# Jisu-Linnea-Han/ClimateMachine.jl

Hardware: AMD Instinct MI355X
Metric: DG RHS DOF-updates/sec (higher is better)
Workload: dtype f64; 1 GPU; Held-Suarez dry GCM (BASELINE configs[2]), stacked cubed sphere 6x30x30x8 elements, N=4, LSRK54 explicit, hyperdiffusion (DryBiharmonic, horizontal), Rusanov, fp64; elements=43200, nodes_per_element=125, states=5, parallelism=element partition (Hilbert, whole columns), 1 rank(s), RCCL p2p halo

## Files before the change

### climatemachine.jl_amd/_lib.py

```python
import ctypes as C
import os

_HERE = os.path.dirname(os.path.abspath(__file__))
LIB_PATH = os.environ.get("CMDG_LIB", os.path.join(_HERE, "libcmdg.so"))

CMDG_K = dict(GRADIENTS=0, DIVGRAD=1, GRADLAP=2, TENDENCY=3, PACK=4, UNPACK=5, UPDATE_AUX=6,
              FILTER=7, STACK_INTEGRAL=8, TRANSPORT=9, HALO_EXPOSED=10, GRADIENTS_EXT=11,
              DIVGRAD_EXT=12, GRADLAP_EXT=13, TENDENCY_EXT=14, FV_GRADIENTS=15, FV_TENDENCY=16,
              ESDG_TENDENCY=17)
STACK_MAXOUT = 8
OPT_KEEP_GRADFLUX = 1
OPT_STACK_HEIGHT = 2
OPT_REFERENCE_HALO = 3
OPT_HALO_PIPELINE = 4
OPT_STEP_GRAPH = 5
OPT_STREAM_PRIORITY = 6
OPT_TENDENCY_PAIRS = 7
OPT_ASYNC_RUN = 8
OPT_TENDENCY_FOUR_WAVES = 9
OPT_GRADARG_HANDOFF = 10
CMDG_Q = dict(GRADFLUX_LIVE=1, LAW_NEEDS_GRADFLUX=2, NDERIVED=3, NUPDATED_AUX=4, FUSED_UPDATE_AUX=5,
              DIRECT_SEND=6, DIRECT_RECV=7, TENDENCY_ELEMS_PER_GROUP=8, HALO_PIPELINE=9, HOST_POST_NS=10, HOST_POST_COUNT=11, GRAPH_STEPS=12, TENDENCY_PAIRS=13,
              GRADARG_HANDOFF=14, GRADARG_REFRESHES=15,
              STATE_READ=16, AUX_READ=20)


class CmdgStackIntegralDesc(C.Structure):
    _fields_ = [
        ("nout", C.c_int32),
        ("src_is_state", C.c_int32 * STACK_MAXOUT), ("src_col", C.c_int32 * STACK_MAXOUT),
        ("scale", C.c_double * STACK_MAXOUT), ("dst_col", C.c_int32 * STACK_MAXOUT),
        ("rsrc_col", C.c_int32 * STACK_MAXOUT), ("rdst_col", C.c_int32 * STACK_MAXOUT),
    ]


class CmdgDesc(C.Structure):
    _fields_ = [
        ("dim", C.c_int32), ("N", C.c_int32 * 3),
        ("nreal", C.c_int64), ("nghost", C.c_int64),
        ("nvgeo", C.c_int32), ("physics_id", C.c_int32),
        ("iparam", C.c_int32 * 16), ("dparam", C.c_double * 64),
        ("nf_first", C.c_int32), ("direction", C.c_int32),
        ("diffusion_direction", C.c_int32), ("stacked", C.c_int32),
        ("vgeo", C.c_void_p), ("sgeo", C.c_void_p),
        ("vmapM", C.c_void_p), ("vmapP", C.c_void_p), ("elemtobndy", C.c_void_p),
        ("interiorelems", C.c_void_p), ("ninterior", C.c_int64),
        ("exteriorelems", C.c_void_p), ("nexterior", C.c_int64),
        ("activedofs", C.c_void_p), ("D", C.c_void_p),
        ("vmapsend", C.c_void_p), ("nvmapsend", C.c_int64),
        ("vmaprecv", C.c_void_p), ("nvmaprecv", C.c_int64),
        ("nnabr", C.c_int32), ("nabrtorank", C.c_void_p),
        ("nabrtovmapsend", C.c_void_p), ("nabrtovmaprecv", C.c_void_p),
        ("state_auxiliary", C.c_void_p), ("state_gradient_flux", C.c_void_p),
        ("Qhypervisc_grad", C.c_void_p), ("Qhypervisc_div", C.c_void_p),
        ("Dv", C.c_void_p),
    ]


MAX_HOOK_OPS = 4


class CmdgRhsHooks(C.Structure):
    _fields_ = [
        ("npre", C.c_int32), ("pre_filter", C.c_void_p * MAX_HOOK_OPS),
        ("ncopy", C.c_int32),
        ("copy_gf_col", C.c_int32 * MAX_HOOK_OPS), ("copy_aux_col", C.c_int32 * MAX_HOOK_OPS),
        ("copy_scale", C.c_double * MAX_HOOK_OPS),
        ("has_integral", C.c_int32), ("has_reverse_integral", C.c_int32),
        ("integral", CmdgStackIntegralDesc), ("reverse_integral", CmdgStackIntegralDesc),
        ("nsurf", C.c_int32),
        ("surf_src_col", C.c_int32 * MAX_HOOK_OPS), ("surf_dst_col", C.c_int32 * MAX_HOOK_OPS),
        ("nvertelem", C.c_int32), ("Imat", C.c_void_p),
        ("has_flow_deviation", C.c_int32), ("flow_u_col", C.c_int32), ("flow_ud_col", C.c_int32),
        ("flow_H", C.c_double),
        ("ops_before_gradients", C.c_int32), ("pre_rhs_handle", C.c_void_p),
        ("pre_rhs_src_col", C.c_int32), ("pre_rhs_dst_aux_col", C.c_int32),
    ]


class CmdgOcean01Desc(C.Structure):
    _fields_ = [("nvertelem", C.c_int32), ("H", C.c_double), ("Imat", C.c_void_p),
                ("add_fast_substeps", C.c_int32), ("nstages_fast", C.c_int32),
                ("rka_fast", C.c_void_p), ("rkb_fast", C.c_void_p), ("rkc_fast", C.c_void_p)]


class CmdgOceanCouplingDesc(C.Structure):
    _fields_ = [
        ("nvertelem", C.c_int32), ("H", C.c_double), ("Imat", C.c_void_p),
        ("slow_u_col", C.c_int32), ("slow_eta_col", C.c_int32), ("slow_dGu_col", C.c_int32),
        ("fast_eta_col", C.c_int32), ("fast_U_col", C.c_int32),
        ("fast_GU_col", C.c_int32), ("fast_du_col", C.c_int32),
    ]


MRI_MAXR, MRI_MAXGAMMA = 6, 4
MRIGARK_EXPLICIT, MRIGARK_DECOUPLED_IMPLICIT = 0, 1


class CmdgMrigarkDesc(C.Structure):
    _fields_ = [("kind", C.c_int32), ("nstages", C.c_int32), ("ngamma", C.c_int32),
                ("gamma", C.c_void_p), ("dc", C.c_void_p), ("fast_nstages", C.c_int32),
                ("fast_rka", C.c_void_p), ("fast_rkb", C.c_void_p), ("fast_rkc", C.c_void_p),
                ("fast_dt", C.c_double), ("lu_adjustable", C.c_int32)]


GMRES_MAX_M = 64


class CmdgGmresInfo(C.Structure):
    _fields_ = [("iterations", C.c_int64), ("converged", C.c_int32), ("residual_norm", C.c_double),
                ("threshold", C.c_double)]


RED_WEIGHTEDSUM, RED_SUM, RED_DOT, RED_DISTANCE, RED_NORM, RED_MAX, RED_MIN = range(7)


class CmdgReduceDesc(C.Structure):
    _fields_ = [("op", C.c_int32), ("p", C.c_double), ("weighted", C.c_int32),
                ("per_state", C.c_int32), ("nstate", C.c_int32), ("states", C.c_void_p),
                ("nstates", C.c_int32)]


class CmdgFvDesc(C.Structure):
    _fields_ = [("reconstruction", C.c_int32), ("width", C.c_int32), ("limiter", C.c_int32),
                ("nvertelem", C.c_int32), ("periodicstack", C.c_int32)]


FV_CONSTANT, FV_LINEAR = 0, 1


class CmdgEsdgDesc(C.Structure):
    _fields_ = [("volume_flux", C.c_int32), ("surface_flux", C.c_int32), ("Mcut", C.c_double),
                ("low_mach", C.c_int32), ("kinetic_energy_preserving", C.c_int32)]


(ESDG_FLUX_NONE, ESDG_FLUX_ENTROPY_CONSERVATIVE, ESDG_FLUX_CENTRAL, ESDG_FLUX_KG, ESDG_FLUX_RUSANOV,
 ESDG_FLUX_ENTROPY_CONSERVATIVE_PENALTY, ESDG_FLUX_MATRIX) = range(7)
FV_VANLEER, FV_NOLIMITER = 0, 1


_vp, _i32, _i64, _d = C.c_void_p, C.c_int32, C.c_int64, C.c_double
SYMBOLS = [
    ("cmdg_version", C.c_char_p, []),
    ("cmdg_status_string", C.c_char_p, [C.c_int]),
    ("cmdg_physics_counts", C.c_int, [_i32, _vp, _vp]),
    ("cmdg_atmos_host_constants", C.c_int, [_vp, _vp, _vp]),
    ("cmdg_create", C.c_int, [C.POINTER(CmdgDesc), C.POINTER(_vp)]),
    ("cmdg_create_dgfv", C.c_int, [C.POINTER(CmdgDesc), C.POINTER(CmdgFvDesc), C.POINTER(_vp)]),
    ("cmdg_create_esdg", C.c_int, [C.POINTER(CmdgDesc), C.POINTER(CmdgEsdgDesc), C.POINTER(_vp)]),
    ("cmdg_esdg_entropy", C.c_int, [_vp, _vp, _vp, _vp]),
    ("cmdg_destroy", C.c_int, [_vp]),
    ("cmdg_last_error", C.c_char_p, [_vp]),
    ("cmdg_rhs", C.c_int, [_vp, _vp, _vp, _d, _d, _d]),
    ("cmdg_rhs_async", C.c_int, [_vp, _vp, _vp, _d, _d, _d]),
    ("cmdg_lsrk_step", C.c_int, [_vp, _vp, _vp, _d, _d, _i32, _vp, _vp, _vp]),
    ("cmdg_lsrk_run", C.c_int, [_vp, _vp, _vp, _d, _d, _i64, _i32, _vp, _vp, _vp]),
    ("cmdg_synchronize", C.c_int, [_vp]),
    ("cmdg_set_option", C.c_int, [_vp, _i32, _i32]),
    ("cmdg_query", C.c_int, [_vp, _i32, _vp]),
    ("cmdg_export_hypervisc_grad", C.c_int, [_vp, _vp]),
    ("cmdg_export_gradient_flux", C.c_int, [_vp, _vp]),
    ("cmdg_halo_begin", C.c_int, [_vp, _vp, _i32]),
    ("cmdg_halo_end", C.c_int, [_vp, _vp, _i32]),
    ("cmdg_fillsendbuf", C.c_int, [_vp, _vp, _vp, _i64, _i32, _i32]),
    ("cmdg_transferrecvbuf", C.c_int, [_vp, _vp, _vp, _i64, _i32, _i32]),
    ("cmdg_comm_unique_id", C.c_int, [_vp]),
    ("cmdg_comm_init_rccl", C.c_int, [_vp, _vp, _i32, _i32]),
    ("cmdg_comm_selftest", C.c_int, [_vp, _i64]),
    ("cmdg_comm_connect_local", C.c_int, [_vp, _i32]),
    ("cmdg_group_rhs", C.c_int, [_vp, _i32, _vp, _vp, _d, _d, _d]),
    ("cmdg_group_halo", C.c_int, [_vp, _i32, _vp, _i32]),
    ("cmdg_group_lsrk_run", C.c_int, [_vp, _i32, _vp, _vp, _d, _d, _i64, _i32, _vp, _vp, _vp]),
    ("cmdg_norm2_local", C.c_int, [_vp, _vp, _i32, _i32, _vp]),
    ("cmdg_distance2_local", C.c_int, [_vp, _vp, _vp, _i32, _vp]),
    ("cmdg_reduce_local", C.c_int, [_vp, _vp, _vp, _vp, _vp]),
    ("cmdg_reduce_combine", C.c_int, [_vp, _vp, _i32, _vp]),
    ("cmdg_reduce", C.c_int, [_vp, _vp, _vp, _vp, _vp]),
    ("cmdg_group_reduce", C.c_int, [_vp, _i32, _vp, _vp, _vp, _vp]),
    ("cmdg_courant", C.c_int, [_vp, _i32, _vp, _d, _d, _i32, _vp]),
    ("cmdg_min_node_distance", C.c_int, [_vp, _i32, _vp]),
    ("cmdg_indefinite_stack_integral", C.c_int, [_vp, _vp, _i32, _vp, _i32, _i32, _vp, _vp]),
    ("cmdg_reverse_indefinite_stack_integral", C.c_int, [_vp, _vp, _i32, _i32, _vp]),
    ("cmdg_filter_create", C.c_int, [_vp, _vp, C.POINTER(_vp)]),
    ("cmdg_filter_destroy", C.c_int, [_vp, _vp]),
    ("cmdg_filter_apply", C.c_int, [_vp, _vp, _vp, _i32]),
    ("cmdg_set_filters", C.c_int, [_vp, _vp, _vp, _vp]),
    ("cmdg_set_rhs_hooks", C.c_int, [_vp, _vp]),
    ("cmdg_ocean_initialize_states", C.c_int, [_vp, _vp, _vp]),
    ("cmdg_ocean_tendency_from_slow_to_fast", C.c_int, [_vp, _vp, _vp, _vp]),
    ("cmdg_ocean_reconcile_from_fast_to_slow", C.c_int, [_vp, _vp, _vp, _vp, _vp]),
    ("cmdg_split_explicit01_step", C.c_int,
     [_vp, _vp, _vp, _vp, _vp, _vp, _vp, _vp, _d, _d, _d, _i32, _vp, _vp, _vp]),
    ("cmdg_group_split_explicit01_step", C.c_int,
     [_vp, _vp, _i32, _vp, _vp, _vp, _vp, _vp, _vp, _d, _d, _d, _i32, _vp, _vp, _vp]),
    ("cmdg_load_plugin", C.c_int, [C.c_char_p]),
    ("cmdg_lsrk_update", C.c_int, [_vp, _vp, _vp, _d, _d]),
    ("cmdg_ls3n_step", C.c_int, [_vp, _vp, _vp, _vp, _d, _d, _i32, _vp, _vp, _vp]),
    ("cmdg_ssprk_step", C.c_int, [_vp, _vp, _vp, _vp, _d, _d, _i32, _vp, _vp, _vp]),
    ("cmdg_group_split_explicit_step", C.c_int,
     [_vp, _vp, _i32, _vp, _i32, _vp, _vp, _vp, _vp, _vp, _d, _d, _d, _i32, _vp, _vp, _vp]),
    ("cmdg_split_explicit_step", C.c_int,
     [_vp, _vp, _vp, _i32, _vp, _vp, _vp, _vp, _vp, _d, _d, _d, _i32, _vp, _vp, _vp]),
    ("cmdg_profile_enable", C.c_int, [_vp, _i32]),
    ("cmdg_profile_get", C.c_int, [_vp, _i32, _vp, _vp]),
    ("cmdg_profile_reset", C.c_int, [_vp]),
    ("cmdg_columnlu_create", C.c_int, [_vp, _i32, _d, C.POINTER(_vp)]),
    ("cmdg_columnlu_update", C.c_int, [_vp, _d]),
    ("cmdg_columnlu_assemble", C.c_int, [_vp, _d]),
    ("cmdg_columnlu_solve", C.c_int, [_vp, _vp, _vp]),
    ("cmdg_columnlu_info", C.c_int, [_vp, _vp]),
    ("cmdg_columnlu_alpha", C.c_int, [_vp, _vp]),
    ("cmdg_columnlu_export_band", C.c_int, [_vp, _i64, _vp]),
    ("cmdg_columnlu_destroy", C.c_int, [_vp]),
    ("cmdg_ark_step", C.c_int, [_vp, _vp, _vp, _vp, _d, _d, _i32, _vp, _vp, _vp, _vp, _i32]),
    ("cmdg_mri_lsrk_update", C.c_int, [_vp, _vp, _vp, _d, _d, _i32, _vp, _vp]),
    ("cmdg_mri_qhat", C.c_int, [_vp, _vp, _vp, _i32, _vp, _vp]),
    ("cmdg_mrigark_step", C.c_int, [_vp, _vp, _vp, _vp, _vp, _vp, _vp, _vp, _d, _d]),
    ("cmdg_gmres_create", C.c_int, [_vp, _i32, _d, _d, C.POINTER(_vp)]),
    ("cmdg_gmres_fits", C.c_int, [_vp, _i32, _i64, _vp]),
    ("cmdg_gmres_prepare", C.c_int, [_vp, _d]),
    ("cmdg_gmres_solve", C.c_int, [_vp, _d, _vp, _vp, _d, _i64, C.POINTER(CmdgGmresInfo)]),
    ("cmdg_gmres_step_info", C.c_int, [_vp, _i32, _vp, _vp]),
    ("cmdg_gmres_destroy", C.c_int, [_vp]),
    ("cmdg_ark_step_gmres", C.c_int, [_vp, _vp, _vp, _vp, _d, _d, _i32, _vp, _vp, _vp, _vp, _i32]),
    ("cmdg_mrigark_step_gmres", C.c_int, [_vp, _vp, _vp, _vp, _vp, _vp, _vp, _vp, _d, _d]),
    ("cmdg_interp_create", C.c_int, [_vp, _vp, C.POINTER(_vp)]),
    ("cmdg_interp_destroy", C.c_int, [_vp, _vp]),
    ("cmdg_interp_apply", C.c_int, [_vp, _vp, _vp, _i32, _i64, _vp]),
    ("cmdg_interp_project", C.c_int, [_vp, _vp, _vp, _i32, _vp]),
    ("cmdg_interp_scatter", C.c_int, [_vp, _vp, _i32, _vp, _i32, _vp]),
    ("cmdg_dss_create", C.c_int, [_vp, _vp, C.POINTER(_vp)]),
    ("cmdg_dss_destroy", C.c_int, [_vp, _vp]),
    ("cmdg_dss_info", C.c_int, [_vp, _vp]),
    ("cmdg_dss_apply", C.c_int, [_vp, _vp, _vp, _i32]),
    ("cmdg_dss", C.c_int, [_vp, _vp, _vp, _i32]),
    ("cmdg_group_dss", C.c_int, [_vp, _i32, _vp, _vp, _i32]),
]

_LIB = None


class CmdgError(RuntimeError):
    pass


def lib():
    global _LIB
    if _LIB is None:
        if not os.path.exists(LIB_PATH):
            raise CmdgError(
                "libcmdg.so is not built (%s); run `python -c 'import __graft_entry__ as g; "
                "g.build()'` -- there is no CPU fallback" % LIB_PATH)
        try:
            import torch
            rccl = os.path.join(os.path.dirname(torch.__file__), "lib", "librccl.so")
            if os.path.exists(rccl):
                os.environ.setdefault("CMDG_RCCL_LIB", rccl)
        except Exception:
            pass
        L = C.CDLL(LIB_PATH)
        for name, res, args in SYMBOLS:
            f = getattr(L, name)
            f.restype = res
            f.argtypes = args
        _LIB = L
    return _LIB


def check(status, handle=None):
    if status != 0:
        L = lib()
        msg = L.cmdg_last_error(handle).decode()
        raise CmdgError("libcmdg: %s (%d): %s" % (
            L.cmdg_status_string(status).decode(), status, msg))
```

### climatemachine.jl_amd/csrc/cmdg.hip

```cpp
#include <dlfcn.h>

#include <algorithm>
#include <new>
#include <tuple>

#include "rccl.h"
#include "stepping.h"

namespace cmdg {

namespace {
typedef int (*roctx_push_t)(const char *);
typedef int (*roctx_pop_t)();
roctx_push_t g_roctx_push = nullptr;
roctx_pop_t g_roctx_pop = nullptr;
int g_roctx_state = 0;
void roctx_resolve()
{
    g_roctx_state = -1;
    const char *names[] = {"librocprofiler-sdk-roctx.so.1", "librocprofiler-sdk-roctx.so", "libroctx64.so.4",
                           "libroctx64.so", nullptr};
    const char *want = getenv("CMDG_ROCTX");
    void *lib = nullptr;
    for (int i = 0; names[i] && !lib; ++i) lib = dlopen(names[i], RTLD_NOW | RTLD_NOLOAD);
    if (!lib && want && *want && *want != '0')
        for (int i = 0; names[i] && !lib; ++i) lib = dlopen(names[i], RTLD_NOW | RTLD_GLOBAL);
    if (!lib) return;
    g_roctx_push = (roctx_push_t)dlsym(lib, "roctxRangePushA");
    g_roctx_pop = (roctx_pop_t)dlsym(lib, "roctxRangePop");
    if (g_roctx_push && g_roctx_pop) g_roctx_state = 1;
}
}
void roctx_push(const char *name)
{
    if (g_roctx_state == 0) roctx_resolve();
    if (g_roctx_state == 1) g_roctx_push(name);
}
void roctx_pop()
{
    if (g_roctx_state == 1) g_roctx_pop();
}

int dbg_sync()
{
    static const int v = [] {
        const char *p = getenv("CMDG_DBG_SYNC");
        return p ? atoi(p) : 0;
    }();
    return v;
}

hipError_t ev_record(hipEvent_t e, hipStream_t s) { return hipEventRecord(e, s); }

int EngineBase::launch_status(const char *what)
{
    hipError_t e = hipGetLastError();
    if (e != hipSuccess) return fail(CMDG_ERR_HIP, std::string(what) + ": " + hipGetErrorString(e));
    return CMDG_OK;
}

int EngineBase::order(hipStream_t earlier, hipStream_t later)
{
    if (earlier == later) return CMDG_OK;
    if (dbg_sync() & 1) (void)hipStreamSynchronize(earlier);
    if (ev_record(ev_comp, earlier) != hipSuccess || hipStreamWaitEvent(later, ev_comp, 0) != hipSuccess)
        return fail(CMDG_ERR_HIP, "stream ordering failed");
    return CMDG_OK;
}

int EngineBase::ensure_Imat(const double *host)
{
    if (d_Imat) return CMDG_OK;
    if (!host) return fail(CMDG_ERR_INVALID, "Imat is NULL");
    if (d_Imat.alloc(NQ * NQ) != hipSuccess ||
        hipMemcpy(d_Imat, host, sizeof(double) * NQ * NQ, hipMemcpyHostToDevice) != hipSuccess)
        return fail(CMDG_ERR_HIP, "Imat upload failed");
    return CMDG_OK;
}

int set_err(cmdg_handle h, int code)
{
    if (h && h->eng && code != CMDG_OK) h->err = h->eng->err;
    return code;
}

GroupCall::GroupCall(cmdg_handle *h, cmdg_handle *h2, int n, bool pairs)
{
    if (!h || (pairs && !h2) || n < 1) return;
    for (int i = 0; i < n; ++i)
        if (!h[i] || (pairs && !h2[i])) return;
    for (int i = 0; i < n; ++i) {
        const std::string r = std::to_string(i);
        members.push_back({h[i], pairs ? "pair " + r + " (slow): " : "rank " + r + ": "});
        if (pairs) members.push_back({h2[i], "pair " + r + " (fast): "});
    }
    for (auto &m : members) {
        if (m.first->eng->worker) m.first->eng->worker->wait_idle();
        m.first->eng->err.clear();
    }
    dev.emplace(h[0]->eng);
}

GroupCall::GroupCall(const std::vector<std::pair<cmdg_handle, std::string>> &named)
{
    if (named.empty()) return;
    for (auto &m : named)
        if (!m.first) return;
    for (auto &m : named) {
        bool merged = false;
        for (auto &have : members)
            if (have.first == m.first) {
                have.second = have.second.substr(0, have.second.size() - 2) + " / " + m.second + ": ";
                merged = true;
            }
        if (!merged) members.push_back({m.first, m.second + ": "});
    }
    for (auto &m : members) {
        if (m.first->eng->worker) m.first->eng->worker->wait_idle();
        m.first->eng->err.clear();
    }
    dev.emplace(named[0].first->eng);
}

int GroupCall::finish(int rc)
{
    if (rc == CMDG_OK) return rc;
    std::string msg = cmdg_status_string(rc);
    for (auto &m : members)
        if (!m.first->eng->err.empty()) {
            msg = m.second + m.first->eng->err;
            break;
        }
    for (auto &m : members) m.first->err = msg;
    return rc;
}

EngineBase::~EngineBase()
{
    delete worker;
    worker = nullptr;
    if (s_comp) hipStreamSynchronize(s_comp);
    if (s_comm) hipStreamSynchronize(s_comm);
    prof_collect();
    if (graph_exec) hipGraphExecDestroy(graph_exec);
    if (nccl_comm && rccl::CommDestroy) rccl::CommDestroy(nccl_comm);
}

static __global__ void k_face_digest(const double *__restrict__ vgeo, int nvgeo,
                                     const double *__restrict__ sgeo,
                                     const int64_t *__restrict__ vmapM,
                                     const int64_t *__restrict__ vmapP,
                                     const int64_t *__restrict__ elemtobndy, int NQ, int NQV,
                                     int64_t nreal, int32_t *__restrict__ faceP,
                                     double *__restrict__ faceG, double *__restrict__ faceW,
                                     int32_t *__restrict__ facePr, int *__restrict__ bad)
{
    const int Np = NQ * NQ * NQV, Nfph = NQ * NQV, Nfpv = NQ * NQ;
    const int Nfp = Nfph > Nfpv ? Nfph : Nfpv, NFT = 4 * Nfph + 2 * Nfpv;
    const int64_t I = (int64_t)blockIdx.x * blockDim.x + threadIdx.x;
    if (I >= nreal * NFT) return;
    const int64_t e = I / NFT;
    const int t = (int)(I % NFT);
    int f, n;
    if (t < 4 * Nfph) {
        f = t / Nfph;
        n = t % Nfph;
    } else {
        f = 4 + (t - 4 * Nfph) / Nfpv;
        n = (t - 4 * Nfph) % Nfpv;
    }
    const int64_t o = n + (int64_t)Nfp * (f + 6 * e);
    const int a = n % NQ, b = n / NQ;
    int vid;
    switch (f) {
    case 0: vid = NQ * (a + NQ * b); break;
    case 1: vid = (NQ - 1) + NQ * (a + NQ * b); break;
    case 2: vid = a + NQ * NQ * b; break;
    case 3: vid = a + NQ * ((NQ - 1) + NQ * b); break;
    case 4: vid = n; break;
    default: vid = n + NQ * NQ * (NQV - 1); break;
    }
    int flags = 0;
    const int64_t idM = vmapM[o] - 1;
    if (idM != e * Np + vid) flags |= 1;
    int64_t idP = vmapP[o] - 1;
    if (elemtobndy[f + 6 * e] != 0) idP = e * Np + vid;
    if (idP < 0 || idP > 2147483647LL) flags |= 4;
    faceP[I] = (int32_t)idP;
    const int64_t eP = idP >= 0 ? idP / Np : 0;
    facePr[I] = (int32_t)(eP * Np + ring_slot_of(NQ, NQV, (int)(idP - eP * Np)));
    const double *sg = sgeo + 5 * o;
#pragma unroll
    for (int c = 0; c < 4; ++c) faceG[((int64_t)4 * e + c) * NFT + t] = sg[c];
    const double mi = vgeo[vid + (int64_t)Np * (VMI + (int64_t)nvgeo * e)];
    if (!(sg[SVMI] == mi)) flags |= 2;
    faceW[I] = mi * sg[SSM];
    if (flags) atomicOr(bad, flags);
}

int EngineBase::init(const cmdg_desc *d)
{
    Np = NQ * NQ * NQV;
    Nfp = NQ * (NQ > NQV ? NQ : NQV);
    if (d->N[0] != d->N[1] || d->N[0] != NQ - 1 || d->N[2] != NQV - 1)
        return fail(CMDG_ERR_INVALID, "cmdg_create: polynomial orders do not match the engine");
    if (NQV != NQ && !d->Dv)
        return fail(CMDG_ERR_INVALID, "cmdg_create: Dv is required when the vertical order differs");
    nreal = d->nreal;
    nghost = d->nghost;
    nelem = nreal + nghost;
    nf_first = d->nf_first;
    direction = d->direction;
    diffusion_direction = d->diffusion_direction;
    stacked = d->stacked;
    if (!d->vgeo || !d->sgeo || !d->vmapM || !d->vmapP || !d->elemtobndy || !d->D ||
        !d->state_auxiliary)
        return fail(CMDG_ERR_INVALID, "cmdg_create: a required grid/state pointer is NULL");
    if (d->nvgeo < 11) return fail(CMDG_ERR_INVALID, "cmdg_create: vgeo needs >= 11 columns");
    if (d->ninterior + d->nexterior != nreal)
        return fail(CMDG_ERR_INVALID, "cmdg_create: interior + exterior != nreal");
    if ((d->ninterior > 0 && !d->interiorelems) || (d->nexterior > 0 && !d->exteriorelems))
        return fail(CMDG_ERR_INVALID, "cmdg_create: element list pointer is NULL");
    if (direction < 0 || direction > 2 || diffusion_direction < 0 || diffusion_direction > 2)
        return fail(CMDG_ERR_INVALID, "cmdg_create: bad direction");
    g.vgeo = d->vgeo;
    g.sgeo = d->sgeo;
    g.vmapM = d->vmapM;
    g.vmapP = d->vmapP;
    g.elemtobndy = d->elemtobndy;
    g.nvgeo = d->nvgeo;
    d_interior = d_interior_user = d->interiorelems;
    ninterior = d->ninterior;
    d_exterior = d_exterior_user = d->exteriorelems;
    nexterior = d->nexterior;
    d_activedofs = d->activedofs;
    d_vmapsend = d->vmapsend;
    nvmapsend = d->nvmapsend;
    d_vmaprecv = d->vmaprecv;
    nvmaprecv = d->nvmaprecv;
    if (d->nnabr > 0) {
        if (!d->nabrtorank || !d->nabrtovmapsend || !d->nabrtovmaprecv || !d->vmapsend ||
            !d->vmaprecv)
            return fail(CMDG_ERR_INVALID, "cmdg_create: halo tables missing");
        nabrtorank.assign(d->nabrtorank, d->nabrtorank + d->nnabr);
        nabrsend.assign(d->nabrtovmapsend, d->nabrtovmapsend + 2 * d->nnabr);
        nabrrecv.assign(d->nabrtovmaprecv, d->nabrtovmaprecv + 2 * d->nnabr);
    }
    HIPCHK(hipGetDevice(&dev));
    HIPCHK(s_comp.create(hipStreamNonBlocking));
    {
        int lo = 0, hi = 0;
        const char *pv = getenv("CMDG_HALO_PRIORITY");
        if (communicate() && pv && *pv == '1' && hipDeviceGetStreamPriorityRange(&lo, &hi) == hipSuccess && hi < lo)
            HIPCHK(s_comm.create(hipStreamNonBlocking, hi));
        else
            HIPCHK(s_comm.create(hipStreamNonBlocking));
    }
    for (int i = 0; i < 2; ++i) {
        HIPCHK(ev_int[i].create(hipEventDisableTiming));
        HIPCHK(ev_ext[i].create(hipEventDisableTiming));
    }
    HIPCHK(gev_fork.create(hipEventDisableTiming));
    if (const char *v = getenv("CMDG_STEP_GRAPH")) step_graph = *v && *v != '0';
    HIPCHK(ev_comp.create(hipEventDisableTiming));
    HIPCHK(d_D.alloc(NQ * NQ));
    HIPCHK(hipMemcpy(d_D, d->D, sizeof(double) * NQ * NQ, hipMemcpyHostToDevice));
    g.D = d_D;
    g.Dv = d_D;
    if (NQV != NQ) {
        HIPCHK(d_Dv.alloc(NQV * NQV));
        HIPCHK(hipMemcpy(d_Dv, d->Dv, sizeof(double) * NQV * NQV, hipMemcpyHostToDevice));
        g.Dv = d_Dv;
    }
    {
        const int NFT = 4 * NQ * NQV + 2 * NQ * NQ;
        const int64_t nt = std::max<int64_t>(nreal, 1) * NFT;
        DevBuf<int> d_bad;
        int bad = 0;
        HIPCHK(d_faceP.alloc(nt));
        HIPCHK(d_faceG.alloc(4 * nt));
        HIPCHK(d_faceW.alloc(nt));
        HIPCHK(d_facePr.alloc(nt));
        HIPCHK(d_bad.alloc_zeroed(1, s_comp));
        if (nreal > 0)
            hipLaunchKernelGGL(k_face_digest, dim3((unsigned)((nreal * NFT + 255) / 256)), dim3(256), 0,
                               s_comp, g.vgeo, g.nvgeo, g.sgeo, g.vmapM, g.vmapP, g.elemtobndy, NQ,
                               NQV, nreal, d_faceP.get(), d_faceG.get(), d_faceW.get(), d_facePr.get(),
                               d_bad.get());
        hipError_t le = hipGetLastError();
        hipError_t ce = hipMemcpyAsync(&bad, d_bad, sizeof(int), hipMemcpyDeviceToHost, s_comp);
        hipError_t se = hipStreamSynchronize(s_comp);
        d_bad.reset();
        if (le != hipSuccess || ce != hipSuccess || se != hipSuccess)
            return fail(CMDG_ERR_HIP, "cmdg_create: digest of the face tables failed");
        if (bad & 1)
            return fail(CMDG_ERR_INVALID, "cmdg_create: vmapM is not the face numbering of Grids.jl:586-594");
        if (bad & 2)
            return fail(CMDG_ERR_INVALID, "cmdg_create: sgeo's vMI differs from vgeo's MI at the face nodes (Grids.jl:1097-1101)");
        if (bad & 4)
            return fail(CMDG_ERR_INVALID, "cmdg_create: too many elements for 32-bit face indices");
        g.faceP = d_faceP;
        g.faceG = d_faceG;
        g.faceW = d_faceW;
        g.facePr = d_facePr;
    }
    aux = d->state_auxiliary;
    const size_t nd = (size_t)Np * nelem;
    gf = gf_node_major() ? nullptr : d->state_gradient_flux;
    gf_user = gf_node_major() ? d->state_gradient_flux : nullptr;
    if (!gf) {
        HIPCHK(gf_own.alloc_zeroed(std::max<size_t>(nd * ngf, 1), s_comp));
        gf = gf_own;
    }
    hypgrad_user = ngl > 0 ? d->Qhypervisc_grad : nullptr;
    HIPCHK(hypgrad.alloc_zeroed(std::max<size_t>(nd * 3 * ngl, 1), s_comp));
    hypdiv = d->Qhypervisc_div;
    if (!hypdiv) {
        HIPCHK(hd_own.alloc_zeroed(std::max<size_t>(nd * nhyp, 1), s_comp));
        hypdiv = hd_own;
    }
    slot_nvar_max = std::max(std::max(ns, ngf), std::max(3 * ngl, nhyp));
    if (communicate()) {
        for (auto &s : slot) {
            HIPCHK(s.sendbuf.alloc(slot_nvar_max * std::max<int64_t>(nvmapsend, 1)));
            HIPCHK(s.recvbuf.alloc(slot_nvar_max * std::max<int64_t>(nvmaprecv, 1)));
            HIPCHK(s.ev_packed.create(hipEventDisableTiming));
            HIPCHK(s.ev_done.create(hipEventDisableTiming));
            HIPCHK(s.ev_pulled.create(hipEventDisableTiming));
        }
    }
    HIPCHK(d_partial.alloc(1024));
    if (communicate())
        if (int r = init_halo_tables()) return r;
    if (const char *v = getenv("CMDG_REFERENCE_HALO")) reference_halo = *v && *v != '0';
    if (const char *v = getenv("CMDG_HALO_PIPELINE")) no_pipeline = *v == '0';
    if (const char *v = getenv("CMDG_FUSED_COLUMNS")) fused_columns = atoi(v);
    if (int r = init_derived()) return r;
    HIPCHK(hipStreamSynchronize(s_comp));
    return CMDG_OK;
}

int EngineBase::ensure_work()
{
    for (int i = 0; i < 2; ++i)
        if (!W[i]) {
            const size_t n = (size_t)Np * ns * nelem;
            HIPCHK(W[i].alloc_zeroed(n, s_comp));
            HIPCHK(hipStreamSynchronize(s_comp));
        }
    return CMDG_OK;
}

int EngineBase::ensure_garg()
{
    if (!garg) {
        const size_t n = std::max<size_t>((size_t)Np * ngl * nelem, 1);
        HIPCHK(garg.alloc_zeroed(n, s_comp));
        HIPCHK(lapr.alloc_zeroed(n, s_comp));
        HIPCHK(hipStreamSynchronize(s_comp));
    }
    return CMDG_OK;
}

int EngineBase::synchronize()
{
    HIPCHK(hipStreamSynchronize(s_comp));
    HIPCHK(hipStreamSynchronize(s_comm));
    return CMDG_OK;
}

ProfRec &EngineBase::prof_pair(int kernel, bool clamp, Event e1)
{
    ProfRec r{kernel, Event(), std::move(e1), clamp};
    r.e0.create();
    if (!r.e1) r.e1.create();
    prof.push_back(std::move(r));
    return prof.back();
}
void EngineBase::prof_begin(int kernel, hipStream_t st)
{
    if (!profiling) return;
    hipEventRecord(prof_pair(kernel, false).e0, st);
}
void EngineBase::prof_end(hipStream_t st)
{
    if (!profiling) return;
    hipEventRecord(prof.back().e1, st);
}
static __global__ void k_export_node_major(double *__restrict__ dst, const double *__restrict__ src, int Np,
                                           int ncol, int64_t nelem)
{
    const int64_t I = (int64_t)blockIdx.x * blockDim.x + threadIdx.x;
    if (I >= (int64_t)Np * ncol * nelem) return;
    const int64_t e = I / ((int64_t)Np * ncol);
    const int r = (int)(I - e * Np * ncol), s = r / Np, n = r - s * Np;
    dst[I] = src[s + (int64_t)ncol * (n + (int64_t)Np * e)];
}
static __global__ void k_import_node_major(double *__restrict__ dst, const double *__restrict__ src, int Np,
                                           int ncol, int64_t nelem)
{
    const int64_t I = (int64_t)blockIdx.x * blockDim.x + threadIdx.x;
    if (I >= (int64_t)Np * ncol * nelem) return;
    const int64_t e = I / ((int64_t)Np * ncol);
    const int r = (int)(I - e * Np * ncol), n = r / ncol, s = r - n * ncol;
    dst[I] = src[n + (int64_t)Np * (s + (int64_t)ncol * e)];
}

int EngineBase::export_hypgrad(double *dst)
{
    if (!dst) dst = hypgrad_user;
    if (ngl == 0) return CMDG_OK;
    if (!dst) return fail(CMDG_ERR_INVALID, "cmdg_export_hypervisc_grad: no destination (cmdg_desc.Qhypervisc_grad was NULL)");
    const int64_t n = (int64_t)Np * 3 * ngl * nelem;
    hipLaunchKernelGGL(k_export_node_major, dim3((unsigned)((n + 255) / 256)), dim3(256), 0, s_comp, dst, hypgrad, Np,
                       3 * ngl, nelem);
    HIPCHK(hipStreamSynchronize(s_comp));
    return CMDG_OK;
}
int EngineBase::export_gradflux(double *dst)
{
    if (!dst) dst = gf_node_major() ? gf_user : gf;
    if (ngf == 0) return CMDG_OK;
    if (!dst) return fail(CMDG_ERR_INVALID, "cmdg_export_gradient_flux: no destination (cmdg_desc.state_gradient_flux was NULL)");
    const int64_t n = (int64_t)Np * ngf * nelem;
    if (gf_node_major()) {
        hipLaunchKernelGGL(k_export_node_major, dim3((unsigned)((n + 255) / 256)), dim3(256), 0, s_comp, dst, gf, Np,
                           ngf, nelem);
    } else if (dst != gf) {
        HIPCHK(hipMemcpyAsync(dst, gf, sizeof(double) * n, hipMemcpyDeviceToDevice, s_comp));
    }
    HIPCHK(hipStreamSynchronize(s_comp));
    return CMDG_OK;
}
void EngineBase::prof_collect()
{
    for (auto &r : prof) {
        hipEventSynchronize(r.e1);
        float ms = 0;
        if (hipEventElapsedTime(&ms, r.e0, r.e1) == hipSuccess) {
            prof_ms[r.kernel] += r.clamp && ms < 0 ? 0.0f : ms;
            prof_n[r.kernel] += 1;
        }
    }
    prof.clear();
}

int EngineBase::set_stack_height(int nv)
{
    constexpr int TILE_C = 32, TILE_L = 4, MIN_HEIGHT = 17;
    if (nv < 0 || (nv > 0 && (!stacked || nreal % nv != 0)))
        return fail(CMDG_ERR_INVALID, "stack height: not a stacked topology or nreal is not a multiple of it");
    if (fv) return CMDG_OK;
    HIPCHK(hipStreamSynchronize(s_comp));
    d_interior = d_interior_user;
    d_exterior = d_exterior_user;
    if (nv < MIN_HEIGHT) return CMDG_OK;
    for (int which = 0; which < 2; ++which) {
        const int64_t n = which ? nexterior : ninterior;
        if (n == 0) continue;
        std::vector<int64_t> h((size_t)n);
        HIPCHK(hipMemcpy(h.data(), which ? d_exterior_user : d_interior_user, sizeof(int64_t) * n,
                         hipMemcpyDeviceToHost));
        auto key = [&](int64_t e1) {
            const int64_t e = e1 - 1, col = e / nv, lev = e % nv;
            return std::make_tuple(col / TILE_C, lev / TILE_L, col % TILE_C, lev % TILE_L);
        };
        std::stable_sort(h.begin(), h.end(), [&](int64_t x, int64_t y) { return key(x) < key(y); });
        DevBuf<int64_t> &own = which ? d_exterior_tiled : d_interior_tiled;
        if (!own) HIPCHK(own.alloc(n));
        HIPCHK(hipMemcpy(own, h.data(), sizeof(int64_t) * n, hipMemcpyHostToDevice));
        (which ? d_exterior : d_interior) = own;
    }
    return CMDG_OK;
}

int EngineBase::set_stream_priority(int level)
{
    int lo = 0, hi = 0;
    HIPCHK(hipDeviceGetStreamPriorityRange(&lo, &hi));
    if (level < -1 || level > 1) return fail(CMDG_ERR_INVALID, "stream priority: 0 (default), 1 (highest) or -1 (lowest)");
    if (int r = synchronize()) return r;
    drop_graph();
    Stream nc, nm;
    const int prio = level > 0 ? hi : (level < 0 ? lo : 0);
    HIPCHK(nc.create(hipStreamNonBlocking, prio));
    HIPCHK(nm.create(hipStreamNonBlocking, prio));
    s_comp = std::move(nc);
    s_comm = std::move(nm);
    stream_priority = level;
    return CMDG_OK;
}

int EngineBase::rhs_segment(int seg, const RhsCtx &c)
{
    const bool comm = exchanges();
    const bool gfl = gf_live();
    const bool grad = gfl || nhyp > 0;
    const bool hyper = nhyp > 0;
    const bool dsend = comm && direct_send(), unpack = !(comm && direct_recv());
    const bool pipe = pipelined() && !has_hooks;
    hipStream_t s_ext = pipe ? s_comm : s_comp;
    const int nhd = ngl;
    int r;
#define TRY(x) \
    if ((r = (x)) != CMDG_OK) return r
    const Event *const EI = capturing ? gev_int : ev_int, *const EE = capturing ? gev_ext : ev_ext;
    auto evi = [&](int64_t q) { return capturing ? (int)((cap_pass + (q - pass_seq)) % NGEV) : (int)(q & 1); };
    auto interior_begin = [&]() -> int {
        ++pass_seq;
        if (capturing) ++cap_pass;
        if (!pipe) return CMDG_OK;
        if (capturing && cap_interior++ == 0) return CMDG_OK;
        if (profiling && prof_ext_done) {
            hipEventRecord(prof_pair(CMDG_K_HALO_EXPOSED, true, std::move(prof_ext_done)).e0, s_comp);
        }
        if (dbg_sync() & 64) HIPCHK(hipStreamSynchronize(s_comm));
        HIPCHK(hipStreamWaitEvent(s_comp, EE[evi(pass_seq - 1)], 0));
        return CMDG_OK;
    };
    auto interior_end = [&]() -> int {
        if (pipe) HIPCHK(ev_record(EI[evi(pass_seq)], s_comp));
        return CMDG_OK;
    };
    auto exterior_begin = [&]() -> int {
        if (pipe && !(capturing && cap_exterior++ == 0)) {
            if (dbg_sync() & 64) HIPCHK(hipStreamSynchronize(s_comp));
            HIPCHK(hipStreamWaitEvent(s_comm, EI[evi(pass_seq - 1)], 0));
        }
        return CMDG_OK;
    };
    auto exterior_end = [&]() -> int {
        if (pipe) HIPCHK(ev_record(EE[evi(pass_seq)], s_comm));
        if (pipe && profiling) {
            prof_ext_done.create();
            hipEventRecord(prof_ext_done, s_comm);
        }
        return CMDG_OK;
    };
    switch (seg) {
    case 0:
        if (has_hooks) {
            if (!c.pre_done) TRY(run_pre_hooks(c));
            slot[SLOT_Q].fresh_for = nullptr;
        }
        if (!(grad && fused_update_aux())) launch_update_aux(c, 0, nreal);
        if (comm) TRY(halo_begin(SLOT_Q, c.Qin, ns, 0, pipe));
        if (grad) {
            TRY(interior_begin());
            launch_gradients(c, d_interior, ninterior, false, s_comp);
            TRY(interior_end());
        }
        break;
    case 1:
        if (!grad) break;
        if (comm) {
            TRY(halo_end(SLOT_Q, c.Qin, ns, unpack, pipe));
            if (unpack) launch_update_aux(c, nreal, nelem);
            if (has_hooks && hooks.has_flow_deviation)
                TRY(flow_deviation(c.Qin, nreal / hooks.nvertelem, nghost / hooks.nvertelem));
            if (has_hooks && hooks.ops_before_gradients) TRY(run_column_ops(c, nreal, nelem));
        }
        if (dsend && gfl) TRY(before_direct_send(SLOT_GF, s_ext));
        if (dsend && hyper) TRY(before_direct_send(SLOT_HG, s_ext));
        TRY(exterior_begin());
        launch_gradients(c, d_exterior, nexterior, comm, s_ext);
        TRY(exterior_end());
        if (dsend && gfl && !gradient_filter) mark_fresh(SLOT_GF, gf, ngf);
        if (dsend && hyper) mark_fresh(SLOT_HG, hypgrad, 3 * ngl);
        if (gradient_filter && gfl) {
            if (gf_node_major()) {
                const int64_t n = (int64_t)Np * ngf * nelem;
                const unsigned nb = (unsigned)((n + 255) / 256);
                if (!gf_scratch) HIPCHK(gf_scratch.alloc(n));
                hipLaunchKernelGGL(k_export_node_major, dim3(nb), dim3(256), 0, s_comp, gf_scratch, gf, Np, ngf, nelem);
                TRY(filter_apply(gradient_filter, gf_scratch, ngf));
                hipLaunchKernelGGL(k_import_node_major, dim3(nb), dim3(256), 0, s_comp, gf, gf_scratch, Np, ngf, nelem);
            } else {
                TRY(filter_apply(gradient_filter, gf, ngf));
            }
        }
        if (comm) {
            int slots[2], ns_ = 0;
            if (gfl) {
                TRY(halo_pack(SLOT_GF, gf, ngf, 0, pipe));
                slots[ns_++] = SLOT_GF;
            }
            if (hyper) {
                TRY(halo_pack(SLOT_HG, hypgrad, 3 * ngl, 0, pipe));
                slots[ns_++] = SLOT_HG;
            }
            if (ns_) TRY(halo_post(slots, ns_));
        }
        if (has_hooks && gfl) TRY(run_gradient_hooks(c, 0, nreal));
        if (hyper) {
            TRY(interior_begin());
            launch_divgrad(c, d_interior, ninterior, false, s_comp);
            TRY(interior_end());
        }
        break;
    case 2:
        if (!hyper) break;
        if (comm) TRY(halo_end(SLOT_HG, hypgrad, 3 * ngl, unpack, pipe));
        if (dsend) TRY(before_direct_send(SLOT_HD, s_ext));
        TRY(exterior_begin());
        launch_divgrad(c, d_exterior, nexterior, comm, s_ext);
        TRY(exterior_end());
        if (dsend) mark_fresh(SLOT_HD, hypdiv, nhd);
        if (comm) TRY(halo_begin(SLOT_HD, hypdiv, nhd, nhyp, pipe));
        TRY(interior_begin());
        launch_gradlap(c, d_interior, ninterior, false, s_comp);
        TRY(interior_end());
        break;
    case 3:
        if (hyper) {
            if (comm) TRY(halo_end(SLOT_HD, hypdiv, nhd, unpack, pipe));
            if (dsend) TRY(before_direct_send(SLOT_HG, s_ext));
            TRY(exterior_begin());
            launch_gradlap(c, d_exterior, nexterior, comm, s_ext);
            TRY(exterior_end());
            if (dsend) mark_fresh(SLOT_HG, hypgrad, 3 * ngl);
            if (comm) TRY(halo_begin(SLOT_HG, hypgrad, 3 * ngl, 0, pipe));
        }
        TRY(interior_begin());
        launch_tendency(c, d_interior, ninterior, false, s_comp);
        TRY(interior_end());
        break;
    case 4:
        if (comm) {
            if (grad) {
                if (gfl) {
                    TRY(halo_end(SLOT_GF, gf, ngf, unpack, pipe));
                    if (has_hooks) TRY(run_gradient_hooks(c, nreal, nelem));
                }
                if (hyper) TRY(halo_end(SLOT_HG, hypgrad, 3 * ngl, unpack, pipe));
            } else {
                TRY(halo_end(SLOT_Q, c.Qin, ns, unpack, pipe));
                if (unpack) launch_update_aux(c, nreal, nelem);
            }
        }
        break;
    case 5:
        if (dsend && c.lsrk) TRY(before_direct_send(SLOT_Q, s_ext));
        TRY(exterior_begin());
        launch_tendency(c, d_exterior, nexterior, comm, s_ext);
        TRY(exterior_end());
        if (dsend && c.lsrk) mark_fresh(SLOT_Q, c.Qout, ns);
        if (pipe && (dbg_sync() & 128)) HIPCHK(hipStreamSynchronize(s_comm));
        if (pipe) HIPCHK(hipStreamWaitEvent(s_comp, EE[evi(pass_seq)], 0));
        if (tendency_filter) TRY(filter_apply(tendency_filter, c.tendency, ns));
        if (c.update_after) {
            const int64_t n = (int64_t)Np * ns * nreal;
            lsrk_update(s_comp, c.tendency, c.Qin, c.rka_next, c.rkb_dt, n);
        }
        break;
    default: break;
    }
#undef TRY
    if (dbg_sync() & 512) HIPCHK(hipDeviceSynchronize());
    return launch_status("kernel launch");
}

int EngineBase::rhs_async(const RhsCtx &c)
{
    if (transport == TRANSPORT_LOCAL && communicate())
        return fail(CMDG_ERR_INVALID, "handles connected locally must be driven by the cmdg_group_* calls");
    invalidate_sends();
    for (int s = 0; s < NSEG; ++s)
        if (int r = rhs_segment(s, c)) {
            abort_exchanges();
            return r;
        }
    return CMDG_OK;
}

int group_rhs(std::vector<EngineBase *> &g, std::vector<RhsCtx> &c, bool keep_fresh)
{
    if (!keep_fresh)
        for (auto *e : g) e->invalidate_sends();
    for (auto &x : c) x.pre_done = false;
    if (dbg_sync() & 256) (void)hipDeviceSynchronize();
    bool nested = false;
    for (auto *e : g) nested = nested || (e->has_hooks && e->hooks.pre_rhs_handle);
    if (nested && g.size() > 1) {
        std::vector<EngineBase *> ch;
        std::vector<RhsCtx> cc(g.size());
        for (size_t i = 0; i < g.size(); ++i) {
            if (!(g[i]->has_hooks && g[i]->hooks.pre_rhs_handle))
                return g[i]->fail(CMDG_ERR_INVALID, "local group: every rank needs the nested operator");
            if (int r = g[i]->run_pre_hooks_a(c[i], cc[i])) return r;
            ch.push_back(g[i]->hooks.pre_rhs_handle->eng);
        }
        for (auto *e : ch) e->err.clear();
        if (int r = group_rhs(ch, cc)) {
            for (size_t i = 0; i < ch.size(); ++i)
                if (!ch[i]->err.empty()) return g[i]->fail(r, "nested operator: " + ch[i]->err);
            return r;
        }
        for (size_t i = 0; i < g.size(); ++i) {
            if (int r = g[i]->run_pre_hooks_b(c[i])) return r;
            c[i].pre_done = true;
        }
    }
    for (int s = 0; s < EngineBase::NSEG; ++s)
        for (size_t i = 0; i < g.size(); ++i)
            if (int r = g[i]->rhs_segment(s, c[i])) {
                for (auto *e : g) e->abort_exchanges();
                return r;
            }
    return CMDG_OK;
}

static __global__ void k_extremum(const double *__restrict__ v, int64_t n, int is_min,
                                  double *__restrict__ out)
{
    __shared__ double s[1024];
    double a = is_min ? INFINITY : -INFINITY;
    for (int64_t i = threadIdx.x; i < n; i += blockDim.x) a = is_min ? fmin(a, v[i]) : fmax(a, v[i]);
    s[threadIdx.x] = a;
    __syncthreads();
    for (int h = blockDim.x / 2; h > 0; h >>= 1) {
        if ((int)threadIdx.x < h)
            s[threadIdx.x] = is_min ? fmin(s[threadIdx.x], s[threadIdx.x + h])
                                    : fmax(s[threadIdx.x], s[threadIdx.x + h]);
        __syncthreads();
    }
    if (threadIdx.x == 0) out[0] = s[0];
}

int EngineBase::courant(int mode, int kind, const double *Q, double dt, double t, int dir,
                        double *out)
{
    if (dir < 0 || dir > 2 || kind < 0 || kind > 3) return fail(CMDG_ERR_INVALID, "courant: bad argument");
    if (g.nvgeo < 15) return fail(CMDG_ERR_INVALID, "courant: vgeo lacks the coordinate columns");
    if (nreal == 0) {
        *out = mode == 0 ? INFINITY : -INFINITY;
        return CMDG_OK;
    }
    if (!d_elemred) HIPCHK(d_elemred.alloc(nreal + 1));
    if (int r = launch_courant(mode, kind, Q, dt, t, dir, d_elemred)) return r;
    hipLaunchKernelGGL(k_extremum, dim3(1), dim3(1024), 0, s_comp, d_elemred, nreal, mode == 0,
                       d_elemred + nreal);
    HIPCHK(hipMemcpyAsync(out, d_elemred + nreal, sizeof(double), hipMemcpyDeviceToHost, s_comp));
    HIPCHK(hipStreamSynchronize(s_comp));
    return CMDG_OK;
}

static __global__ void k_wsum2(const double *__restrict__ A, const double *__restrict__ B,
                        const double *__restrict__ vgeo, int nvgeo, int Np, int nvar,
                        int64_t nreal, int weighted, double *__restrict__ partial)
{
    __shared__ double sh[256];
    const int64_t total = (int64_t)Np * nvar * nreal;
    double acc = 0.0;
    for (int64_t I = (int64_t)blockIdx.x * blockDim.x + threadIdx.x; I < total;
         I += (int64_t)gridDim.x * blockDim.x) {
        const int64_t e = I / ((int64_t)Np * nvar);
        const int n = (int)(I % Np);
        double d = A[I];
        if (B) d -= B[I];
        const double w = weighted ? vgeo[n + (int64_t)Np * (VM + (int64_t)nvgeo * e)] : 1.0;
        acc += w * d * d;
    }
    sh[threadIdx.x] = acc;
    __syncthreads();
    for (int s = 128; s > 0; s >>= 1) {
        if ((int)threadIdx.x < s) sh[threadIdx.x] += sh[threadIdx.x + s];
        __syncthreads();
    }
    if (threadIdx.x == 0) partial[blockIdx.x] = sh[0];
}

int EngineBase::wsum2(const double *A, const double *B, int nvar, int weighted, double *out)
{
    const int nb = 512;
    hipLaunchKernelGGL(k_wsum2, dim3(nb), dim3(256), 0, s_comp, A, B, g.vgeo, g.nvgeo, Np, nvar,
                       nreal, weighted, d_partial);
    double h[nb];
    HIPCHK(hipMemcpyAsync(h, d_partial, sizeof(double) * nb, hipMemcpyDeviceToHost, s_comp));
    HIPCHK(hipStreamSynchronize(s_comp));
    double acc = 0;
    for (int i = 0; i < nb; ++i) acc += h[i];
    *out = acc;
    return CMDG_OK;
}

}

using namespace cmdg;

extern "C" {

const char *cmdg_version(void) { return "cmdg 0.1 (gfx950)"; }

const char *cmdg_status_string(int status)
{
    switch (status) {
    case CMDG_OK: return "ok";
    case CMDG_ERR_INVALID: return "invalid argument";
    case CMDG_ERR_HIP: return "HIP runtime error";
    case CMDG_ERR_NO_DEVICE: return "no gfx950 device";
    case CMDG_ERR_COMM: return "communication error";
    case CMDG_ERR_UNSUPPORTED: return "unsupported physics / polynomial order";
    default: return "unknown status";
    }
}

int cmdg_esdg_entropy(cmdg_handle h, const double *Q, double *beta, double *eta)
{
    if (!h || !Q) return CMDG_ERR_INVALID;
    DevGuard guard_(h->eng);
    return set_err(h, h->eng->launch_entropy(Q, beta, eta));
}

int cmdg_rhs_async(cmdg_handle h, double *tendency, double *Q, double t, double alpha, double beta)
{
    if (!h || !tendency || !Q) return CMDG_ERR_INVALID;
    DevGuard guard_(h->eng);
    RhsCtx c;
    c.tendency = tendency;
    c.Qin = Q;
    c.t = t;
    c.alpha = alpha;
    c.beta = beta;
    return set_err(h, h->eng->rhs_async(c));
}

int cmdg_rhs(cmdg_handle h, double *tendency, double *Q, double t, double alpha, double beta)
{
    int r = cmdg_rhs_async(h, tendency, Q, t, alpha, beta);
    if (r) return r;
    DevGuard guard_(h->eng);
    return set_err(h, h->eng->synchronize());
}

int cmdg_synchronize(cmdg_handle h)
{
    if (!h) return CMDG_ERR_INVALID;
    DevGuard guard_(h->eng);
    if (h->eng->worker) {
        std::lock_guard<std::mutex> lk(h->eng->worker->m);
        if (const int r = h->eng->worker->deferred_rc) {
            h->eng->err = h->eng->worker->deferred_err;
            h->eng->worker->deferred_rc = 0;
            h->eng->worker->deferred_err.clear();
            return set_err(h, r);
        }
    }
    return set_err(h, h->eng->synchronize());
}

int cmdg_set_option(cmdg_handle h, int32_t option, int32_t value)
{
    if (!h) return CMDG_ERR_INVALID;
    DevGuard guard_(h->eng);
    EngineBase *e = h->eng;
    switch (option) {
    case CMDG_OPT_KEEP_GRADFLUX:
        e->drop_graph();
        e->keep_gradflux = value != 0;
        return CMDG_OK;
    case CMDG_OPT_STACK_HEIGHT:
        e->drop_graph();
        return set_err(h, e->set_stack_height(value));
    case CMDG_OPT_REFERENCE_HALO:
        if (int r = e->synchronize()) return set_err(h, r);
        e->drop_graph();
        e->reference_halo = value != 0 || e->fv || e->esdg;
        e->invalidate_sends();
        return CMDG_OK;
    case CMDG_OPT_STEP_GRAPH:
        if (int r = e->synchronize()) return set_err(h, r);
        e->drop_graph();
        e->step_graph = value != 0;
        e->graph_failed = false;
        return CMDG_OK;
    case CMDG_OPT_STREAM_PRIORITY: return set_err(h, e->set_stream_priority(value));
    case CMDG_OPT_ASYNC_RUN:
        if (value && !e->worker) {
            e->worker = new (std::nothrow) RunWorker();
            if (!e->worker) return set_err(h, e->fail(CMDG_ERR_INVALID, "async run: out of memory"));
            e->worker->start();
        } else if (!value && e->worker) {
            delete e->worker;
            e->worker = nullptr;
        }
        return CMDG_OK;
    case CMDG_OPT_TENDENCY_PAIRS:
    case CMDG_OPT_TENDENCY_FOUR_WAVES: return CMDG_OK;
    case CMDG_OPT_GRADARG_HANDOFF: e->gradarg_handoff = value != 0; return CMDG_OK;
    case CMDG_OPT_HALO_PIPELINE:
        if (int r = e->synchronize()) return set_err(h, r);
        e->drop_graph();
        e->no_pipeline = value == 0;
        e->invalidate_sends();
        return CMDG_OK;
    default: return set_err(h, e->fail(CMDG_ERR_INVALID, "cmdg_set_option: unknown option"));
    }
}

int cmdg_query(cmdg_handle h, int32_t what, int64_t *out)
{
    if (!h || !out) return CMDG_ERR_INVALID;
    const EngineBase *e = h->eng;
    switch (what) {
    case CMDG_Q_GRADFLUX_LIVE: *out = e->gf_live(); return CMDG_OK;
    case CMDG_Q_LAW_NEEDS_GRADFLUX: *out = e->law_needs_gradflux(); return CMDG_OK;
    case CMDG_Q_NDERIVED: *out = e->law_nder(); return CMDG_OK;
    case CMDG_Q_NUPDATED_AUX: *out = e->has_update_aux() ? e->law_nupd() : 0; return CMDG_OK;
    case CMDG_Q_FUSED_UPDATE_AUX: *out = e->has_update_aux() && e->fused_update_aux(); return CMDG_OK;
    case CMDG_Q_DIRECT_SEND: *out = e->communicate() && e->direct_send(); return CMDG_OK;
    case CMDG_Q_DIRECT_RECV: *out = e->communicate() && e->direct_recv(); return CMDG_OK;
    case CMDG_Q_TENDENCY_ELEMS_PER_GROUP: *out = e->tendency_epb(); return CMDG_OK;
    case CMDG_Q_GRAPH_STEPS: *out = e->graph_steps; return CMDG_OK;
    case CMDG_Q_TENDENCY_PAIRS: *out = -1; return CMDG_OK;
    case CMDG_Q_GRADARG_HANDOFF: *out = e->handoff_used; return CMDG_OK;
    case CMDG_Q_GRADARG_REFRESHES: *out = e->handoff_refreshes; return CMDG_OK;
    case CMDG_Q_HOST_POST_NS: *out = e->host_post_ns; return CMDG_OK;
    case CMDG_Q_HOST_POST_COUNT: *out = e->host_post_n; return CMDG_OK;
    case CMDG_Q_HALO_PIPELINE: *out = e->pipelined() && !e->has_hooks; return CMDG_OK;
    default:
        if (what >= CMDG_Q_STATE_READ && what < CMDG_Q_STATE_READ + 4) {
            *out = e->law_state_read(what - CMDG_Q_STATE_READ);
            return CMDG_OK;
        }
        if (what >= CMDG_Q_AUX_READ && what < CMDG_Q_AUX_READ + 4) {
            *out = e->law_aux_read(what - CMDG_Q_AUX_READ);
            return CMDG_OK;
        }
        return set_err(h, h->eng->fail(CMDG_ERR_INVALID, "cmdg_query: unknown item"));
    }
}

int cmdg_export_hypervisc_grad(cmdg_handle h, double *dst)
{
    if (!h) return CMDG_ERR_INVALID;
    DevGuard guard_(h->eng);
    return set_err(h, h->eng->export_hypgrad(dst));
}

int cmdg_export_gradient_flux(cmdg_handle h, double *dst)
{
    if (!h) return CMDG_ERR_INVALID;
    DevGuard guard_(h->eng);
    return set_err(h, h->eng->export_gradflux(dst));
}

int cmdg_group_rhs(cmdg_handle *handles, int32_t n, double **tendency, double **Q, double t,
                   double alpha, double beta)
{
    if (!tendency || !Q) return CMDG_ERR_INVALID;
    for (int i = 0; i < n; ++i)
        if (!tendency[i] || !Q[i]) return CMDG_ERR_INVALID;
    GroupCall gc(handles, n);
    if (!gc.ok()) return CMDG_ERR_INVALID;
    std::vector<EngineBase *> g;
    std::vector<RhsCtx> c(n);
    for (int i = 0; i < n; ++i) {
        g.push_back(handles[i]->eng);
        c[i].tendency = tendency[i];
        c[i].Qin = Q[i];
        c[i].t = t;
        c[i].alpha = alpha;
        c[i].beta = beta;
    }
    return gc.finish(group_rhs(g, c));
}

int cmdg_norm2_local(cmdg_handle h, const double *A, int32_t nstate, int32_t weighted,
                     double *out_host)
{
    if (!h || !A || !out_host) return CMDG_ERR_INVALID;
    DevGuard guard_(h->eng);
    return set_err(h, h->eng->wsum2(A, nullptr, nstate, weighted, out_host));
}
int cmdg_distance2_local(cmdg_handle h, const double *A, const double *B, int32_t nstate,
                         double *out_host)
{
    if (!h || !A || !B || !out_host) return CMDG_ERR_INVALID;
    DevGuard guard_(h->eng);
    return set_err(h, h->eng->wsum2(A, B, nstate, 1, out_host));
}

int cmdg_courant(cmdg_handle h, int32_t kind, const double *Q, double dt, double simtime,
                 int32_t direction, double *out_host)
{
    if (!h || !Q || !out_host) return CMDG_ERR_INVALID;
    DevGuard guard_(h->eng);
    if (h->eng->fv)
        return set_err(h, h->eng->fail(CMDG_ERR_UNSUPPORTED, "courant: the device Courant number is not defined "
                                                             "for a finite-volume vertical (DGFVModel handle)"));
    return set_err(h, h->eng->courant(1, kind, Q, dt, simtime, direction, out_host));
}

int cmdg_min_node_distance(cmdg_handle h, int32_t direction, double *out_host)
{
    if (!h || !out_host) return CMDG_ERR_INVALID;
    DevGuard guard_(h->eng);
    if (h->eng->fv)
        return set_err(h, h->eng->fail(CMDG_ERR_UNSUPPORTED, "min_node_distance: on a DGFVModel handle the vertical "
                                                             "distance is the cell height 2 JcV; use the host grid's"));
    return set_err(h, h->eng->courant(0, 0, nullptr, 0.0, 0.0, direction, out_host));
}

int cmdg_profile_enable(cmdg_handle h, int32_t on)
{
    if (!h) return CMDG_ERR_INVALID;
    DevGuard guard_(h->eng);
    h->eng->drop_graph();
    h->eng->profiling = on != 0;
    return CMDG_OK;
}
int cmdg_profile_get(cmdg_handle h, int32_t kernel, double *total_ms, int64_t *launches)
{
    if (!h || kernel < 0 || kernel >= CMDG_K_COUNT) return CMDG_ERR_INVALID;
    DevGuard guard_(h->eng);
    h->eng->synchronize();
    h->eng->prof_collect();
    if (total_ms) *total_ms = h->eng->prof_ms[kernel];
    if (launches) *launches = h->eng->prof_n[kernel];
    return CMDG_OK;
}
int cmdg_profile_reset(cmdg_handle h)
{
    if (!h) return CMDG_ERR_INVALID;
    DevGuard guard_(h->eng);
    h->eng->synchronize();
    h->eng->prof_collect();
    for (int i = 0; i < CMDG_K_COUNT; ++i) {
        h->eng->prof_ms[i] = 0;
        h->eng->prof_n[i] = 0;
    }
    return CMDG_OK;
}

}
```

### climatemachine.jl_amd/csrc/engine.h

```cpp
#pragma once
#include "engine_base.h"
#include "kernels.h"

namespace cmdg {

template <class P, int NQ_, int NQV_ = NQ_>
struct EngineT : EngineBase {
    typename P::Params prm;
    PassArgs<P> make_args(const RhsCtx &c, const int64_t *elems, int64_t n, int dir, bool exterior, double *send0,
                          double *send1) const
    {
        PassArgs<P> a;
        a.prm = prm;
        a.g = g;
        a.elems = elems;
        a.nelems = n;
        a.Q = c.Qin;
        a.aux = aux;
        a.aux_rw = aux;
        a.derived = derived;
        a.gf = gf;
        a.hypgrad = hypgrad;
        a.hypdiv = hypdiv;
        a.tendency = c.tendency;
        a.Qout = c.Qout;
        a.garg = garg;
        a.lapr = lapr;
        a.hypdiv_out = c.hypdiv_out;
        a.t = c.t;
        a.tptr = c.tptr;
        a.alpha = c.alpha;
        a.beta = c.beta;
        a.rkb_dt = c.rkb_dt;
        a.rka_next = c.rka_next;
        a.direction = dir;
        a.model_dir = direction;
        a.nf_first = nf_first;
        a.h = halo_dev(exterior, send0, send1);
        return a;
    }
    using Kernel = void (*)(PassArgs<P>);
    static constexpr bool HO = GradArgHandoff<P, NQ_, NQV_>::value;
    static constexpr bool ELIDE = GradArgHandoff<P, NQ_, NQV_>::elide_refresh;
    struct Pass {
        const char *range, *range_ext;
        int prof, prof_ext;
    };
    static constexpr Pass GRADIENTS{"cmdg:gradients", "cmdg:gradients:exterior", CMDG_K_GRADIENTS, CMDG_K_GRADIENTS_EXT};
    static constexpr Pass DIVGRAD{"cmdg:divgrad", "cmdg:divgrad:exterior", CMDG_K_DIVGRAD, CMDG_K_DIVGRAD_EXT};
    static constexpr Pass GRADLAP{"cmdg:gradlap", "cmdg:gradlap:exterior", CMDG_K_GRADLAP, CMDG_K_GRADLAP_EXT};
    static constexpr Pass TENDENCY{"cmdg:tendency", "cmdg:tendency:exterior", CMDG_K_TENDENCY, CMDG_K_TENDENCY_EXT};
    template <class Enqueue>
    void in_pass(const Pass &p, int64_t n, bool exterior, hipStream_t st, Enqueue enqueue)
    {
        if (n <= 0) return;
        Range range_(exterior ? p.range_ext : p.range);
        prof_begin(exterior ? p.prof_ext : p.prof, st);
        enqueue();
        prof_end(st);
    }
    static Kernel pick_gradients(bool gf_live, bool garg_in)
    {
        if constexpr (HO)
            if (garg_in) return k_gradients<P, NQ_, NQV_, false, true>;
        return gf_live ? k_gradients<P, NQ_, NQV_, true> : k_gradients<P, NQ_, NQV_, false>;
    }
    template <bool LSRK, bool GF>
    static Kernel tendency_recv(bool recv)
    {
        return recv ? k_tendency<P, NQ_, NQV_, LSRK, GF, true> : k_tendency<P, NQ_, NQV_, LSRK, GF, false>;
    }
    static Kernel pick_tendency(bool lsrk, bool gf, bool recv, GargOut out)
    {
        if constexpr (HO)
            if (out != GargOut::none) {
                if constexpr (ELIDE)
                    if (out == GargOut::records) return k_tendency<P, NQ_, NQV_, true, false, false, true, false>;
                return k_tendency<P, NQ_, NQV_, true, false, false, true>;
            }
        if (lsrk) return gf ? tendency_recv<true, true>(recv) : tendency_recv<true, false>(recv);
        return gf ? tendency_recv<false, true>(recv) : tendency_recv<false, false>(recv);
    }
    static Kernel pick_divgrad(bool ring)
    {
        if constexpr (HO)
            if (ring) return k_divgrad<P, NQ_, NQV_, true>;
        return k_divgrad<P, NQ_, NQV_>;
    }
    static Kernel pick_gradlap(bool ring)
    {
        if constexpr (HO)
            if (ring) return k_gradlap<P, NQ_, NQV_, true>;
        return k_gradlap<P, NQ_, NQV_>;
    }
    void launch_gradients(const RhsCtx &c, const int64_t *elems, int64_t n, bool exterior, hipStream_t st) override
    {
        in_pass(GRADIENTS, n, exterior, st, [&] {
            const PassArgs<P> args = make_args(c, elems, n, diffusion_direction, exterior,
                                               gf_live() ? slot[SLOT_GF].sendbuf : nullptr,
                                               ngl > 0 ? slot[SLOT_HG].sendbuf : nullptr);
            hipLaunchKernelGGL(pick_gradients(gf_live(), c.garg_in), dim3((unsigned)n), dim3(KDims<NQ_, NQV_>::NT), 0,
                               st, args);
        });
    }
    void launch_divgrad(const RhsCtx &c, const int64_t *elems, int64_t n, bool exterior, hipStream_t st) override
    {
        in_pass(DIVGRAD, n, exterior, st, [&] {
            const PassArgs<P> args = make_args(c, elems, n, diffusion_direction, exterior, slot[SLOT_HD].sendbuf, nullptr);
            hipLaunchKernelGGL(pick_divgrad(c.garg_in), dim3((unsigned)n), dim3(KDims<NQ_, NQV_>::NT), 0, st, args);
        });
    }
    void launch_gradlap(const RhsCtx &c, const int64_t *elems, int64_t n, bool exterior, hipStream_t st) override
    {
        in_pass(GRADLAP, n, exterior, st, [&] {
            PassArgs<P> args = make_args(c, elems, n, diffusion_direction, exterior, slot[SLOT_HG].sendbuf, nullptr);
            if (c.garg_in) args.g.faceP = g.facePr;
            hipLaunchKernelGGL(pick_gradlap(c.garg_in), dim3((unsigned)n), dim3(KDims<NQ_, NQV_>::NT), 0, st, args);
        });
    }
    void launch_tendency(const RhsCtx &c, const int64_t *elems, int64_t n, bool exterior, hipStream_t st) override
    {
        in_pass(TENDENCY, n, exterior, st, [&] {
            using SH = TendencyShape<P, NQ_, NQV_>;
            PassArgs<P> args = make_args(c, elems, n, direction, exterior, c.lsrk ? slot[SLOT_Q].sendbuf : nullptr, nullptr);
            const bool recv = args.h.ghostslot != nullptr && exterior;
            if (!recv) args.h.ghostslot = nullptr;
            hipLaunchKernelGGL(pick_tendency(c.lsrk, P::needs_gradflux(prm), recv, c.garg_out),
                               dim3((unsigned)SH::blocks(n)), dim3(SH::NT), 0, st, args);
        });
    }
    void launch_update_aux(const RhsCtx &c, int64_t e0, int64_t e1) override
    {
        if constexpr (P::HAS_UPDATE_AUX) {
            if (e1 <= e0 || !P::update_aux_active(prm)) return;
            const int64_t n = (e1 - e0) * KDims<NQ_, NQV_>::Np;
            prof_begin(CMDG_K_UPDATE_AUX, s_comp);
            hipLaunchKernelGGL((k_update_aux<P, NQ_, NQV_>), dim3((unsigned)((n + 255) / 256)), dim3(256),
                               0, s_comp, prm, c.Qin, aux, d_activedofs, c.t, e0, e1);
            prof_end(s_comp);
        }
    }
    int launch_courant(int mode, int kind, const double *Q, double dt, double t, int dir,
                       double *out_elem) override
    {
        constexpr int NT = KDims<NQ_, NQV_>::Np <= 128 ? 128 : 256;
        if (mode == 1 && !P::HAS_COURANT)
            return fail(CMDG_ERR_UNSUPPORTED, "this balance law defines no local Courant number");
        if (mode == 0)
            hipLaunchKernelGGL((k_courant<P, NQ_, NQV_, 0>), dim3((unsigned)nreal), dim3(NT), 0, s_comp, prm,
                               g.vgeo, g.nvgeo, Q, aux, gf, kind, dt, t, dir, out_elem);
        else
            hipLaunchKernelGGL((k_courant<P, NQ_, NQV_, 1>), dim3((unsigned)nreal), dim3(NT), 0, s_comp, prm,
                               g.vgeo, g.nvgeo, Q, aux, gf, kind, dt, t, dir, out_elem);
        return CMDG_OK;
    }
    bool has_update_aux() const override { return P::HAS_UPDATE_AUX && P::update_aux_active(prm); }
    bool law_needs_gradflux() const override { return P::needs_gradflux(prm); }
    bool gf_node_major() const override { return cmdg::gf_node_major<P>::value; }
    bool fused_update_aux() const override { return P::HAS_UPDATE_AUX && P::FUSE_UPDATE_AUX; }
    bool garg_capable() const override { return HO && !P::needs_gradflux(prm); }
    bool refresh_elidable() const override { return ELIDE; }
    int law_nder() const override { return P::HAS_SOURCE ? P::NDER : 0; }
    int law_nupd() const override { return P::HAS_UPDATE_AUX ? P::NUPD : 0; }
    int tendency_epb() const override { return TendencyShape<P, NQ_, NQV_>::EPB; }
    int law_state_read(int pass) const override { return law_reads<P>::state(pass); }
    int law_aux_read(int pass) const override { return law_reads<P>::aux(pass); }
    int init_derived() override
    {
        if constexpr (P::NDER > 0) {
            const int64_t n = nelem * KDims<NQ_, NQV_>::Np;
            if (derived.alloc((size_t)n * P::NDER) != hipSuccess)
                return fail(CMDG_ERR_HIP, "hipMalloc(derived) failed");
            hipLaunchKernelGGL((k_init_derived<P, NQ_, NQV_>), dim3((unsigned)((n + 255) / 256)), dim3(256),
                               0, s_comp, prm, aux, derived, nelem);
            if (hipStreamSynchronize(s_comp) != hipSuccess)
                return fail(CMDG_ERR_HIP, "k_init_derived failed");
        }
        return CMDG_OK;
    }
};

template <class P, int NQ_, int NQV_ = NQ_>
EngineBase *make_engine(const cmdg_desc *d)
{
    auto *e = new EngineT<P, NQ_, NQV_>();
    e->NQ = NQ_;
    e->NQV = NQV_;
    e->ns = P::NS;
    e->naux = P::NAUX;
    e->ngrad = P::NGRAD;
    e->ngf = P::NGF;
    e->ngl = P::NGL;
    e->nhyp = P::NHYP;
    P::make_params(e->prm, d->iparam, d->dparam);
    return e;
}


}
```

### climatemachine.jl_amd/csrc/engine_base.h

```cpp
#pragma once
#include <hip/hip_runtime.h>
#include <stdint.h>

#include <algorithm>
#include <condition_variable>
#include <deque>
#include <functional>
#include <mutex>
#include <optional>
#include <string>
#include <thread>
#include <vector>

#include "../../include/cmdg.h"
#include "cmdg_common.h"
#include "owned.h"

namespace cmdg {

enum { SLOT_Q = 0, SLOT_GF = 1, SLOT_HG = 2, SLOT_HD = 3, NSLOT = 4 };
enum { TRANSPORT_NONE = 0, TRANSPORT_LOCAL = 1, TRANSPORT_RCCL = 2 };

struct HaloSlot {
    DevBuf<double> sendbuf, recvbuf;
    Event ev_packed, ev_done, ev_pulled;
    bool active = false;
    int nvar = 0;
    int ncol = 0;
    double *array = nullptr;
    const double *fresh_for = nullptr;
    int fresh_nvar = 0;
};

struct StepInRun {
    bool first_step, last_step;
};

enum class GargOut { none, records, records_refresh };

struct RhsCtx {
    double *tendency = nullptr;
    double *Qin = nullptr;
    double *Qout = nullptr;
    double t = 0, alpha = 1, beta = 0;
    const double *tptr = nullptr;
    bool lsrk = false;
    bool update_after = false;
    bool garg_in = false;
    bool hypdiv_out = true;
    GargOut garg_out = GargOut::none;
    double rkb_dt = 0, rka_next = 0;
    bool pre_done = false;
};

struct FilterObj {
    int kind = 0, target = 0, direction = 0;
    int nindices = 0;
    int indices[CMDG_MAX_FILTER_STATES] = {0};
    int aux_ref_rho = 0, aux_ref_rhoe = 0;
    DevBuf<double> d_Fh, d_Fv;
};

void roctx_push(const char *name);
void roctx_pop();
int dbg_sync();
hipError_t ev_record(hipEvent_t e, hipStream_t s);
inline unsigned nblocks(int64_t n) { return (unsigned)std::min<int64_t>((n + 255) / 256, 65535); }
struct Range {
    explicit Range(const char *name) { roctx_push(name); }
    ~Range() { roctx_pop(); }
    Range(const Range &) = delete;
    Range &operator=(const Range &) = delete;
};

struct ProfRec {
    int kernel;
    Event e0, e1;
    bool clamp;
};

struct RunWorker {
    std::thread th;
    std::mutex m;
    std::condition_variable cv;
    std::deque<std::function<int()>> jobs;
    bool stop = false, busy = false;
    int deferred_rc = 0;
    std::string deferred_err;
    std::thread::id tid;
    void start()
    {
        th = std::thread([this] {
            std::unique_lock<std::mutex> lk(m);
            for (;;) {
                cv.wait(lk, [this] { return stop || !jobs.empty(); });
                if (jobs.empty()) return;
                auto job = std::move(jobs.front());
                jobs.pop_front();
                busy = true;
                lk.unlock();
                const int r = job();
                lk.lock();
                busy = false;
                if (r && !deferred_rc) deferred_rc = r;
                cv.notify_all();
            }
        });
        tid = th.get_id();
    }
    void submit(std::function<int()> f)
    {
        {
            std::lock_guard<std::mutex> lk(m);
            jobs.push_back(std::move(f));
        }
        cv.notify_all();
    }
    void wait_idle()
    {
        if (std::this_thread::get_id() == tid) return;
        std::unique_lock<std::mutex> lk(m);
        cv.wait(lk, [this] { return jobs.empty() && !busy; });
    }
    ~RunWorker()
    {
        if (th.joinable()) {
            {
                std::lock_guard<std::mutex> lk(m);
                stop = true;
            }
            cv.notify_all();
            th.join();
        }
    }
};

#define HIPCHK(call)                                                                     \
    do {                                                                                 \
        hipError_t e_ = (call);                                                          \
        if (e_ != hipSuccess)                                                            \
            return fail(CMDG_ERR_HIP, std::string(#call) + ": " + hipGetErrorString(e_)); \
    } while (0)

struct EngineBase {
    Stream s_comp, s_comm;
    RunWorker *worker = nullptr;
    int NQ = 0, NQV = 0, Np = 0, Nfp = 0;
    int64_t nreal = 0, nghost = 0, nelem = 0;
    int ns = 0, naux = 0, ngrad = 0, ngf = 0, ngl = 0, nhyp = 0;
    int nf_first = 0, direction = 0, diffusion_direction = 0, stacked = 0;
    GridDev g{};
    const int64_t *d_interior = nullptr, *d_exterior = nullptr;
    const int64_t *d_interior_user = nullptr, *d_exterior_user = nullptr;
    DevBuf<int64_t> d_interior_tiled, d_exterior_tiled;
    int set_stack_height(int nv);
    int set_stream_priority(int level);
    int stream_priority = 0;
    int64_t ninterior = 0, nexterior = 0;
    const uint8_t *d_activedofs = nullptr;
    DevBuf<double> d_D;
    DevBuf<int32_t> d_faceP;
    DevBuf<double> d_faceG;
    DevBuf<double> d_faceW;
    DevBuf<int32_t> d_facePr;
    const int64_t *d_vmapsend = nullptr, *d_vmaprecv = nullptr;
    int64_t nvmapsend = 0, nvmaprecv = 0;
    std::vector<int> nabrtorank;
    std::vector<int64_t> nabrsend, nabrrecv;
    double *aux = nullptr, *gf = nullptr, *hypdiv = nullptr;
    DevBuf<double> hypgrad;
    DevBuf<double> derived;
    DevBuf<double> gf_own, hd_own;
    double *hypgrad_user = nullptr, *gf_user = nullptr;
    DevBuf<double> gf_scratch;
    bool node_major(const double *array) const
    {
        return array == hypgrad || (array == gf && gf_node_major());
    }
    int dev = 0;
    Event ev_comp;
    HaloSlot slot[NSLOT];
    int slot_nvar_max = 0;
    DevBuf<double> W[2];
    DevBuf<double> garg;
    DevBuf<double> lapr;
    bool gradarg_handoff = true;
    bool handoff_used = false;
    int64_t handoff_refreshes = 0;
    virtual bool garg_capable() const = 0;
    virtual bool refresh_elidable() const = 0;
    bool handoff_eligible() const
    {
        return gradarg_handoff && garg_capable() && !gf_live() && ngl > 0 && has_update_aux() &&
               fused_update_aux() && !has_hooks && !step_filter && !tendency_filter && !gradient_filter &&
               !step_graph && nghost == 0 && !communicate();
    }
    int ensure_garg();
    DevBuf<double> d_partial;
    int transport = TRANSPORT_NONE;
    int rank = 0, nranks = 1;
    std::vector<EngineBase *> group;
    void *nccl_comm = nullptr;
    const FilterObj *gradient_filter = nullptr, *tendency_filter = nullptr,
                    *step_filter = nullptr;
    bool profiling = false;
    std::vector<ProfRec> prof;
    double prof_ms[CMDG_K_COUNT] = {0};
    int64_t prof_n[CMDG_K_COUNT] = {0};
    std::string err;

    virtual ~EngineBase();
    int init(const cmdg_desc *d);
    int fail(int code, const std::string &msg)
    {
        err = msg;
        return code;
    }
    int launch_status(const char *what);
    int order(hipStream_t earlier, hipStream_t later);
    bool communicate() const { return !nabrtorank.empty(); }
    bool fv = false;
    int fv_nvert = 0;
    bool esdg = false;
    bool fused_lsrk() const { return tendency_filter == nullptr && !fv && !esdg; }
    int init_fv();
    bool column_orders() const { return NQ >= 2 && NQ <= 8 && NQV == NQ; }
    bool exchanges() const { return communicate() && !(stacked && direction == DIR_VERTICAL); }

    virtual void launch_gradients(const RhsCtx &c, const int64_t *elems, int64_t n, bool exterior, hipStream_t st) = 0;
    virtual void launch_divgrad(const RhsCtx &c, const int64_t *elems, int64_t n, bool exterior, hipStream_t st) = 0;
    virtual void launch_gradlap(const RhsCtx &c, const int64_t *elems, int64_t n, bool exterior, hipStream_t st) = 0;
    virtual void launch_tendency(const RhsCtx &c, const int64_t *elems, int64_t n, bool exterior, hipStream_t st) = 0;
    virtual void launch_update_aux(const RhsCtx &c, int64_t e0, int64_t e1) = 0;
    virtual bool has_update_aux() const = 0;
    virtual bool law_needs_gradflux() const = 0;
    virtual bool gf_node_major() const = 0;
    bool keep_gradflux = false;
    bool gf_live() const
    {
        return ngf > 0 && (keep_gradflux || law_needs_gradflux() || has_hooks || gradient_filter);
    }
    virtual bool fused_update_aux() const = 0;
    virtual int law_nder() const = 0;
    virtual int law_nupd() const = 0;
    virtual int tendency_epb() const = 0;
    virtual int law_state_read(int pass) const = 0;
    virtual int law_aux_read(int pass) const = 0;
    virtual int init_derived() = 0;
    virtual int launch_courant(int mode, int kind, const double *Q, double dt, double t, int dir,
                               double *out_elem) = 0;
    virtual int launch_entropy(const double *, double *, double *)
    {
        return fail(CMDG_ERR_UNSUPPORTED, "cmdg_esdg_entropy: not an ESDGModel handle (cmdg_create_esdg)");
    }

    DevBuf<int32_t> d_sendoff, d_ghostslot;
    DevBuf<SendEnt> d_sendent;
    bool direct_send_ok = false, direct_recv_ok = false;
    bool reference_halo = false;
    int init_halo_tables();
    bool direct_send() const { return direct_send_ok && !reference_halo; }
    bool direct_recv() const
    {
        return direct_recv_ok && !reference_halo && !has_hooks && !(has_update_aux() && !fused_update_aux());
    }
    HaloDev halo_dev(bool exterior, double *send0, double *send1) const
    {
        HaloDev h{};
        h.nreal = nreal;
        if (!communicate()) return h;
        if (exterior && direct_send()) {
            h.sendoff = d_sendoff;
            h.sendent = d_sendent;
            h.send[0] = send0;
            h.send[1] = send1;
        }
        if (direct_recv()) {
            h.ghostslot = d_ghostslot;
            h.recvQ = slot[SLOT_Q].recvbuf;
            h.recvGF = slot[SLOT_GF].recvbuf;
            h.recvHG = slot[SLOT_HG].recvbuf;
            h.recvHD = slot[SLOT_HD].recvbuf;
        }
        return h;
    }
    int before_direct_send(int s, hipStream_t st);
    Event ev_int[2], ev_ext[2];
    int64_t pass_seq = 0;
    int64_t host_post_ns = 0, host_post_n = 0;
    Event prof_ext_done;
    bool no_pipeline = false;
    bool pipelined() const
    {
        return exchanges() && !no_pipeline && direct_send() && direct_recv() && !gradient_filter &&
               !tendency_filter && (!has_update_aux() || fused_update_aux());
    }
    void invalidate_sends()
    {
        for (auto &h : slot) h.fresh_for = nullptr;
    }
    void mark_fresh(int s, const double *array, int nvar)
    {
        slot[s].fresh_for = array;
        slot[s].fresh_nvar = nvar;
    }

    bool step_graph = false;
    bool capturing = false;
    int cap_interior = 0, cap_exterior = 0;
    static constexpr int NGEV = 64;
    Event gev_int[NGEV], gev_ext[NGEV], gev_fork;
    int cap_pass = 0;
    hipGraphExec_t graph_exec = nullptr;
    struct GraphKey {
        const double *Q = nullptr, *dQ = nullptr;
        double dt = 0;
        int nstages = 0;
        double coef[48] = {0};
        bool pipe = false, comm = false;
        bool operator==(const GraphKey &o) const
        {
            if (Q != o.Q || dQ != o.dQ || dt != o.dt || nstages != o.nstages || pipe != o.pipe || comm != o.comm)
                return false;
            for (int i = 0; i < 48; ++i)
                if (coef[i] != o.coef[i]) return false;
            return true;
        }
    } graph_key;
    DevBuf<double> d_gtime;
    int64_t graph_steps = 0;
    bool graph_failed = false;
    bool graph_eligible() const;
    void drop_graph()
    {
        if (graph_exec) {
            hipStreamSynchronize(s_comp);
            hipGraphExecDestroy(graph_exec);
            graph_exec = nullptr;
        }
    }
    int capture_step(double *Q, double *dQ, double dt, int nstages, const double *rka,
                     const double *rkb, const double *rkc);
    int run_steps(double *Q, double *dQ, double t, double dt, int64_t nsteps, int nstages,
                  const double *rka, const double *rkb, const double *rkc);

    static constexpr int NSEG = 6;
    int rhs_segment(int seg, const RhsCtx &c);
    int rhs_async(const RhsCtx &c);
    int lsrk_step(double *Q, double *dQ, double t, double dt, int nstages, const double *rka,
                  const double *rkb, const double *rkc, bool continued = false,
                  const StepInRun *handoff = nullptr);
    int export_hypgrad(double *dst);
    int export_gradflux(double *dst);
    int halo_begin(int s, double *array, int nvar, int ncol = 0, bool on_halo_stream = false);
    int halo_pack(int s, double *array, int nvar, int ncol = 0, bool on_halo_stream = false);
    int halo_post(const int *slots, int nslots);
    int halo_end(int s, double *array, int nvar, bool unpack = true, bool on_halo_stream = false);
    void abort_exchanges();
    int ensure_work();
    int synchronize();
    int wsum2(const double *A, const double *B, int nvar, int weighted, double *out);
    int courant(int mode, int kind, const double *Q, double dt, double t, int dir, double *out);
    DevBuf<double> d_elemred;
    int stack_integral(bool reverse, const double *Q, int nstate, double *aux_arr, int naux_arr,
                       int nvert, const double *Imat_host, const cmdg_stack_integral_desc *d,
                       int64_t h0 = 0, int64_t nh = -1);
    bool has_hooks = false;
    bool hooks_orphaned = false;
    cmdg_rhs_hooks hooks{};
    std::vector<EngineBase *> nested_in;
    int set_hooks(const cmdg_rhs_hooks *hk);
    int run_pre_hooks(const RhsCtx &c);
    int run_pre_hooks_a(const RhsCtx &c, RhsCtx &nested);
    int run_pre_hooks_b(const RhsCtx &c);
    int integrate_velocity(const double *X, int nstate, int col, int nvert, int64_t h0 = 0,
                           int64_t nh = -1);
    int flow_deviation(double *Q, int64_t h0, int64_t nh);
    DevBuf<double> d_flowint;
    DevBuf<double> d_preT;
    int run_column_ops(const RhsCtx &c, int64_t e0, int64_t e1);
    int fused_columns = 2;
    bool column_chain(const RhsCtx &c, int64_t e0, int64_t e1, bool with_copies);
    bool filter_pair(double *Q);
    int run_gradient_hooks(const RhsCtx &c, int64_t e0, int64_t e1);
    DevBuf<double> d_Imat;
    int ensure_Imat(const double *host);
    DevBuf<double> d_Dv;
    int filter_create(const cmdg_filter_desc *d, FilterObj **out);
    int filter_apply(const FilterObj *f, double *Q, int nstate);

    ProfRec &prof_pair(int kernel, bool clamp, Event e1 = Event());
    void prof_begin(int kernel, hipStream_t st);
    void prof_end(hipStream_t st);
    void prof_collect();
};

}

struct cmdg_context {
    cmdg::EngineBase *eng = nullptr;
    std::string err;
};

namespace cmdg {
struct DevGuard {
    int prev = -1;
    bool changed = false;
    explicit DevGuard(const EngineBase *e)
    {
        if (e->worker) e->worker->wait_idle();
        if (hipGetDevice(&prev) == hipSuccess && prev != e->dev)
            changed = hipSetDevice(e->dev) == hipSuccess;
    }
    ~DevGuard()
    {
        if (changed) (void)hipSetDevice(prev);
    }
    DevGuard(const DevGuard &) = delete;
    DevGuard &operator=(const DevGuard &) = delete;
};

struct GroupCall {
    GroupCall(cmdg_handle *handles, int n) : GroupCall(handles, nullptr, n, false) {}
    GroupCall(cmdg_handle *slow, cmdg_handle *fast, int n) : GroupCall(slow, fast, n, true) {}
    explicit GroupCall(const std::vector<std::pair<cmdg_handle, std::string>> &named);
    bool ok() const { return !members.empty(); }
    int finish(int rc);

  private:
    GroupCall(cmdg_handle *h, cmdg_handle *h2, int n, bool pairs);
    std::vector<std::pair<cmdg_handle, std::string>> members;
    std::optional<DevGuard> dev;
};

int set_err(cmdg_handle h, int code);
void set_create_err(const std::string &msg);

struct ObjectDevice {
    int prev = -1;
    bool changed = false;
    explicit ObjectDevice(int dev)
    {
        if (hipGetDevice(&prev) == hipSuccess && prev != dev) changed = hipSetDevice(dev) == hipSuccess;
    }
    ~ObjectDevice()
    {
        if (changed) (void)hipSetDevice(prev);
    }
    ObjectDevice(const ObjectDevice &) = delete;
    ObjectDevice &operator=(const ObjectDevice &) = delete;
};
inline int object_call_done(cmdg_handle h, int r, const std::string &err)
{
    if (r == CMDG_OK) return r;
    if (h) return set_err(h, h->eng->fail(r, err));
    set_create_err(err);
    return r;
}

inline unsigned long engine_abi_stamp()
{
    return (unsigned long)sizeof(EngineBase) * 1000003ul + (unsigned long)sizeof(cmdg_desc) * 10007ul +
           (unsigned long)sizeof(RhsCtx) * 101ul + (unsigned long)sizeof(cmdg_rhs_hooks);
}

}
```

### climatemachine.jl_amd/csrc/kernels.h

```cpp
#pragma once
#include <type_traits>

#include "cmdg_common.h"

#ifndef CMDG_TEND_MINW
#define CMDG_TEND_MINW 1
#endif
#ifndef CMDG_TEND_EPB_LARGE
#define CMDG_TEND_EPB_LARGE 2
#endif
#ifndef CMDG_TEND_EPB_SMALL
#define CMDG_TEND_EPB_SMALL 1
#endif
#ifndef CMDG_GRAD_MINW
#define CMDG_GRAD_MINW 4
#endif
#ifndef CMDG_GRAD_BOUND_LARGE
#define CMDG_GRAD_BOUND_LARGE 1024
#endif
#ifndef CMDG_LAP_MINW
#define CMDG_LAP_MINW 1
#endif

namespace cmdg {

template <class P>
struct PassArgs {
    typename P::Params prm;
    GridDev g;
    const int64_t *elems;
    int64_t nelems;
    const double *Q;
    const double *aux;
    double *aux_rw;
    const double *derived;
    double *gf;
    double *hypgrad;
    double *hypdiv;
    double *tendency;
    double *Qout;
    double *garg;
    double *lapr;
    int hypdiv_out;
    double t, alpha, beta;
    const double *tptr;
    double rkb_dt, rka_next;
    int direction;
    int model_dir;
    int nf_first;
    HaloDev h;
};

struct FacePt {
    double n[3], sM, vMI;
    double w;
    int64_t eP;
    int vidM, vidP, bctag;
};

template <int NQ, int NQV = NQ>
__host__ __device__ __forceinline__ constexpr int face_vid(int f, int n)
{
    const int a = n % NQ, b = n / NQ;
    switch (f) {
    case 0: return NQ * (a + NQ * b);
    case 1: return (NQ - 1) + NQ * (a + NQ * b);
    case 2: return a + NQ * NQ * b;
    case 3: return a + NQ * ((NQ - 1) + NQ * b);
    case 4: return n;
    default: return n + NQ * NQ * (NQV - 1);
    }
}

template <int NQ, int NQV = NQ>
__device__ __forceinline__ void face_index(const GridDev &g, int64_t e, int t, int f, int32_t &idP,
                                           int &bctag)
{
    idP = g.faceP[(int64_t)KDims<NQ, NQV>::NFT * e + t];
    bctag = (int)g.elemtobndy[f + 6 * e];
}
template <int NQ, int NQV = NQ, bool LIFTW = false>
__device__ __forceinline__ void face_geometry(const GridDev &g, int64_t e, int t, int f, int n,
                                              int32_t idP, int bctag, FacePt &fp)
{
    constexpr int Np = KDims<NQ, NQV>::Np, NFT = KDims<NQ, NQV>::NFT;
    const double *sg = g.faceG + (int64_t)4 * NFT * e + t;
    fp.n[0] = sg[0];
    fp.n[1] = sg[NFT];
    fp.n[2] = sg[2 * NFT];
    fp.vidM = face_vid<NQ, NQV>(f, n);
    if constexpr (LIFTW) {
        fp.w = g.faceW[(int64_t)NFT * e + t];
    } else {
        fp.sM = sg[3 * NFT];
        fp.vMI = g.vgeo[fp.vidM + (int64_t)Np * (VMI + (int64_t)g.nvgeo * e)];
    }
    fp.bctag = bctag;
    fp.eP = idP / Np;
    fp.vidP = idP - (int)fp.eP * Np;
}
template <int NQ, int NQV = NQ, bool LIFTW = false>
__device__ __forceinline__ void face_setup(const GridDev &g, int64_t e, int t, int f, int n,
                                           FacePt &fp)
{
    int32_t idP;
    int bctag;
    face_index<NQ, NQV>(g, e, t, f, idP, bctag);
    face_geometry<NQ, NQV, LIFTW>(g, e, t, f, n, idP, bctag, fp);
}

template <class P, class = void>
struct has_flux_wavespeed : std::false_type {
};
template <class P>
struct has_flux_wavespeed<P, std::void_t<decltype(P::HAS_FLUX_WAVESPEED)>> : std::true_type {
};

template <class P, class = void>
struct gf_node_major : std::false_type {
};
template <class P>
struct gf_node_major<P, std::void_t<decltype(P::GF_NODE_MAJOR)>>
    : std::integral_constant<bool, P::GF_NODE_MAJOR && (P::NGF > 0)> {
};
template <class P, int Np>
__device__ __forceinline__ int64_t gf_at(int n, int s, int64_t e)
{
    return col_at<gf_node_major<P>::value, P::NGF, Np>(n, s, e);
}
template <class P, int Np>
__device__ __forceinline__ void load_gf(Vec<P::NGF> &dst, const double *__restrict__ arr, int n, int64_t e)
{
#pragma unroll
    for (int s = 0; s < P::NGF; ++s) dst[s] = arr[gf_at<P, Np>(n, s, e)];
}
template <class P, int Np>
__device__ __forceinline__ void load_plus_gf(Vec<P::NGF> &dst, const double *__restrict__ arr,
                                             const double *__restrict__ recv, int gslot, int vidP, int64_t eP)
{
    if (gslot >= 0) {
#pragma unroll
        for (int s = 0; s < P::NGF; ++s) dst[s] = recv[s + (int64_t)P::NGF * gslot];
    } else {
        load_gf<P, Np>(dst, arr, vidP, eP);
    }
}

template <class P, class = void>
struct node_cache_size : std::integral_constant<int, 0> {
};
template <class P>
struct node_cache_size<P, std::void_t<decltype(P::NCACHE)>> : std::integral_constant<int, P::NCACHE> {
};

template <class P, class = void>
struct law_reads {
    static constexpr int state(int) { return P::NS; }
    static constexpr int aux(int) { return P::NAUX; }
};
template <class P>
struct law_reads<P, std::void_t<decltype(P::aux_read(0))>> {
    static constexpr int state(int pass) { return P::state_read(pass); }
    static constexpr int aux(int pass) { return P::aux_read(pass); }
};

template <class P, class = void>
struct has_law_nf : std::false_type {
};
template <class P>
struct has_law_nf<P, std::void_t<decltype(P::LAW_NF)>> : std::integral_constant<bool, P::LAW_NF> {
};

template <class P>
__device__ __forceinline__ void nf_first_order(const typename P::Params &prm, int nf,
                                               Vec<P::NS> &fluxn, const double *n,
                                               const double *QM, const double *auxM,
                                               const double *QP, const double *auxP, double t,
                                               int facedir, const double *cacheM = nullptr)
{
    constexpr int NS = P::NS;
    if constexpr (has_law_nf<P>::value) {
        if (nf >= NF_ROE) {
            P::numerical_flux_law(prm, nf, fluxn, n, QM, auxM, QP, auxP, t, facedir);
            return;
        }
    }
    Vec<3 * NS> FM, FP;
    Vec<NS> wM, wP;
    FM.negzero();
    FP.negzero();
    if constexpr (has_flux_wavespeed<P>::value) {
        if (nf == NF_RUSANOV) {
            if constexpr (node_cache_size<P>::value > 0) {
                if (cacheM)
                    P::flux_wavespeed_cached(prm, FM, wM, n, QM, auxM, cacheM);
                else
                    P::flux_wavespeed(prm, FM, wM, n, QM, auxM, t, facedir);
            } else {
                P::flux_wavespeed(prm, FM, wM, n, QM, auxM, t, facedir);
            }
            P::flux_wavespeed(prm, FP, wP, n, QP, auxP, t, facedir);
        } else {
            P::flux_first_order(prm, FM, QM, auxM, t, facedir);
            P::flux_first_order(prm, FP, QP, auxP, t, facedir);
        }
    } else {
        P::flux_first_order(prm, FM, QM, auxM, t, facedir);
        P::flux_first_order(prm, FP, QP, auxP, t, facedir);
    }
    const double nh0 = n[0] / 2, nh1 = n[1] / 2, nh2 = n[2] / 2;
#pragma unroll
    for (int s = 0; s < NS; ++s)
        fluxn[s] += (FM[3 * s] + FP[3 * s]) * nh0 + (FM[3 * s + 1] + FP[3 * s + 1]) * nh1 +
                    (FM[3 * s + 2] + FP[3 * s + 2]) * nh2;
    if (nf == NF_RUSANOV) {
        if constexpr (!has_flux_wavespeed<P>::value) {
            P::wavespeed(prm, wM, n, QM, auxM, t, facedir);
            P::wavespeed(prm, wP, n, QP, auxP, t, facedir);
        }
        Vec<NS> pen;
#pragma unroll
        for (int s = 0; s < NS; ++s) {
            const double mw = wM[s] > wP[s] ? wM[s] : wP[s];
            pen[s] = mw * (QM[s] - QP[s]);
        }
        if constexpr (P::HAS_PENALTY) P::update_penalty(prm, pen, n, QM, QP);
#pragma unroll
        for (int s = 0; s < NS; ++s) fluxn[s] += pen[s] / 2;
    }
}

template <int NQ, int NQV = NQ>
__device__ __forceinline__ int surf_index(int ijk)
{
    constexpr int NI = NQ - 2, NIV = NQV > 2 ? NQV - 2 : 0;
    const int i = ijk % NQ, j = (ijk / NQ) % NQ, k = ijk / (NQ * NQ);
    const bool ii = i >= 1 && i <= NI, jj = j >= 1 && j <= NI, kk = k >= 1 && k <= NIV;
    if (ii && jj && kk) return -1;
    auto clampi = [](int v, int hi) { return v < 0 ? 0 : (v > hi ? hi : v); };
    int before = NI * NI * clampi(k - 1, NIV);
    if (kk) {
        before += NI * clampi(j - 1, NI);
        if (jj) before += clampi(i - 1, NI);
    }
    return ijk - before;
}
template <int NQ, int NQV = NQ>
struct SurfDims {
    static constexpr int NSURF =
        NQ * NQ * NQV - (NQ - 2) * (NQ - 2) * (NQV > 2 ? NQV - 2 : 0);
};

template <class P, class = void>
struct has_gradient_flux_g : std::false_type {
};
template <class P>
struct has_gradient_flux_g<P, std::void_t<decltype(&P::gradient_flux_g)>> : std::true_type {
};
template <class P>
__device__ __forceinline__ void law_gradient_flux(const typename P::Params &prm, double *gf,
                                                  const double *g, const double *Q, const double *aux,
                                                  double t, const double *G)
{
    if constexpr (has_gradient_flux_g<P>::value)
        P::gradient_flux_g(prm, gf, g, Q, aux, t, G);
    else
        P::gradient_flux(prm, gf, g, Q, aux, t);
}

template <class P, class = void>
struct grad_min_waves : std::integral_constant<int, CMDG_GRAD_MINW> {
};
template <class P>
struct grad_min_waves<P, std::void_t<decltype(P::GRAD_MIN_WAVES)>> : std::integral_constant<int, P::GRAD_MIN_WAVES> {
};

template <class P, int NQ, int NQV>
struct TendencyShape {
    using KD = KDims<NQ, NQV>;
    static constexpr int EPB =
        node_cache_size<P>::value != 0 ? 1 : (KD::Np > 125 ? CMDG_TEND_EPB_LARGE : CMDG_TEND_EPB_SMALL);
    static constexpr bool STAGE_M = EPB == 1;
    static constexpr int NTE = EPB == 1 ? KD::NT : (KD::Np > KD::NFT ? KD::Np : KD::NFT);
    static constexpr int NT = EPB == 1 ? KD::NT : ((EPB * NTE + 63) / 64) * 64;
    static int64_t blocks(int64_t nelems) { return (nelems + EPB - 1) / EPB; }
};

template <class P, class = void>
struct law_gradarg_handoff : std::false_type {
};
template <class P>
struct law_gradarg_handoff<P, std::void_t<decltype(P::GRADARG_HANDOFF)>>
    : std::integral_constant<bool, P::GRADARG_HANDOFF && (P::NGL > 0) && P::HAS_UPDATE_AUX && P::FUSE_UPDATE_AUX> {
};
template <class P, class = void>
struct law_refresh_unread : std::false_type {
};
template <class P>
struct law_refresh_unread<P, std::void_t<decltype(P::GRADARG_REFRESH_UNREAD)>>
    : std::integral_constant<bool, P::GRADARG_REFRESH_UNREAD && law_gradarg_handoff<P>::value> {
};
template <class P, int NQ, int NQV>
struct GradArgHandoff {
    static constexpr bool value = law_gradarg_handoff<P>::value && TendencyShape<P, NQ, NQV>::EPB == 1;
    static constexpr bool elide_refresh = value && law_refresh_unread<P>::value;
};
template <int NGL, int Np>
__device__ __forceinline__ int64_t garg_at(int n, int64_t e)
{
    return (int64_t)NGL * (n + (int64_t)Np * e);
}

template <class P, int NQ, int NQV, bool LSRK, bool USE_GF, bool RECV = false, bool GARG_OUT = false,
          bool GARG_REFRESH = true>
__device__ __forceinline__ void tendency_body(const PassArgs<P> &a)
{
    static_assert(!GARG_OUT || (LSRK && !USE_GF && !RECV && TendencyShape<P, NQ, NQV>::EPB == 1),
                  "the hand-off rides in the fused update of single-rank handles");
    static_assert(GARG_REFRESH || (GARG_OUT && GradArgHandoff<P, NQ, NQV>::elide_refresh),
                  "only a hand-off launch of a law that opts in may leave the refresh out");
    using KD = KDims<NQ, NQV>;
    const double a_t = a.tptr ? *a.tptr : a.t;
    using SH = TendencyShape<P, NQ, NQV>;
    constexpr int EPB = SH::EPB;
    constexpr bool STAGE_M = SH::STAGE_M;
    constexpr int Np = KD::Np, NS = P::NS, NAUX = P::NAUX, NGF = P::NGF,
                  NHYP = P::NHYP, NHG = 3 * P::NGL, NFA = P::NFAUX,
                  NSURF = SurfDims<NQ, NQV>::NSURF, NGFS = USE_GF ? NGF : 0,
                  NCA = node_cache_size<P>::value,
                  NMF = (STAGE_M ? NFA + NGFS + NHYP : 0) + NCA, OCA = NMF - NCA;
    __shared__ double aD[NQ * NQ + (NQV == NQ ? 0 : NQV * NQV)], aF[EPB * 3 * NS * Np],
        aM[EPB * (NMF > 0 ? NMF : 1) * (NMF > 0 ? NSURF : 1)], aQ[EPB * NS * Np];
    double *sD = aD, *sF_ = aF, *sM_ = aM, *sQ_ = aQ;
    const double *const sDv = sD + (NQV == NQ ? 0 : NQ * NQ);
    const int sub = EPB == 1 ? 0 : (int)threadIdx.x / SH::NTE;
    const int tid = EPB == 1 ? (int)threadIdx.x : (int)threadIdx.x - sub * SH::NTE;
    const int64_t li = (int64_t)EPB * xcd_remap(blockIdx.x, gridDim.x) + sub;
    const bool live = EPB == 1 || (sub < EPB && li < a.nelems);
    const int64_t e = live ? a.elems[li] - 1 : 0;
    const int lsub = live ? sub : 0;
    double *const sF = sF_ + lsub * (3 * NS * Np);
    double *const sM = sM_ + lsub * ((NMF > 0 ? NMF : 1) * (NMF > 0 ? NSURF : 1));
    double *const sQ = sQ_ + lsub * (NS * Np);
    double *const sT = sF;
    if (threadIdx.x < NQ * NQ) sD[threadIdx.x] = a.g.D[threadIdx.x];
    if constexpr (NQV != NQ) {
        if (threadIdx.x < NQV * NQV) sD[NQ * NQ + threadIdx.x] = a.g.Dv[threadIdx.x];
    }
    const bool hz = a.direction != DIR_VERTICAL, vt = a.direction != DIR_HORIZONTAL;
    constexpr bool use_gf = NGF > 0 && USE_GF;
    constexpr bool HS_SHAPE = NHYP > 0 && !use_gf && Np <= 125 && NS >= 5;
    int32_t f_idP = 0;
    int f_bctag = 0, f_f = 0, f_n = 0;
    KD::face_task(tid, f_f, f_n);
    const bool face_on = live && tid < KD::NFT && (f_f < 4 ? hz : vt);
    if (face_on) face_index<NQ, NQV>(a.g, e, tid, f_f, f_idP, f_bctag);
    Vec<NS> S;
    double MI = 0;
    if (live && tid < Np) {
        const double *vg = a.g.vgeo + (int64_t)Np * a.g.nvgeo * e + tid;
        const double M = vg[VM * Np];
        MI = vg[VMI * Np];
        Vec<NS> lQ;
        Vec<NAUX> laux;
        Vec<NGF> lgf;
        Vec<NHYP> lhyp;
        double x11 = 0, x12 = 0, x13 = 0, x21 = 0, x22 = 0, x23 = 0, x31 = 0, x32 = 0, x33 = 0;
        constexpr bool METRICS_FIRST = !HS_SHAPE;
        if constexpr (METRICS_FIRST) {
            if (hz) {
                x11 = vg[XI1X1 * Np], x12 = vg[XI1X2 * Np], x13 = vg[XI1X3 * Np];
                x21 = vg[XI2X1 * Np], x22 = vg[XI2X2 * Np], x23 = vg[XI2X3 * Np];
            }
            if (vt) x31 = vg[XI3X1 * Np], x32 = vg[XI3X2 * Np], x33 = vg[XI3X3 * Np];
        }
        load_state<NS, Np>(lQ, a.Q, tid, e);
        load_state<NAUX, Np>(laux, a.aux, tid, e);
#pragma unroll
        for (int s = 0; s < NGF; ++s) lgf[s] = 0.0;
        if (use_gf) load_gf<P, Np>(lgf, a.gf, tid, e);
#pragma unroll
        for (int s = 0; s < NHYP; ++s)
            lhyp[s] = a.hypgrad[hg_at<NHG, Np>(tid, s, e)];
        if constexpr (METRICS_FIRST) __builtin_amdgcn_sched_barrier(0);
        const int sidx = surf_index<NQ, NQV>(tid);
#pragma unroll
        for (int s = 0; s < NS; ++s) sQ[s * Np + tid] = lQ[s];
        if (STAGE_M && sidx >= 0) {
#pragma unroll
            for (int s = 0; s < NFA; ++s) sM[s * NSURF + sidx] = laux[P::face_aux(s)];
            if (use_gf) {
#pragma unroll
                for (int s = 0; s < NGF; ++s) sM[(NFA + s) * NSURF + sidx] = lgf[s];
            }
#pragma unroll
            for (int s = 0; s < NHYP; ++s) sM[(NFA + NGFS + s) * NSURF + sidx] = lhyp[s];
        }
        Vec<3 * NS> F, F2;
        F.negzero();
        if constexpr (NCA > 0) {
            Vec<NCA> lc;
            P::node_cache(a.prm, lc, lQ, laux);
            P::flux_first_order_cached(a.prm, F, lQ, laux, lc);
            if (sidx >= 0) {
#pragma unroll
                for (int s = 0; s < NCA; ++s)
                    sM[(OCA + s) * NSURF + sidx] = lc[s];
            }
        } else {
            P::flux_first_order(a.prm, F, lQ, laux, a_t, a.model_dir);
        }
        F2.negzero();
        P::flux_second_order(a.prm, F2, lQ, lgf, lhyp, laux, a_t);
#pragma unroll
        for (int q = 0; q < 3 * NS; ++q) F[q] += F2[q];
        if (hz) {
            if constexpr (!METRICS_FIRST) {
                x11 = vg[XI1X1 * Np], x12 = vg[XI1X2 * Np], x13 = vg[XI1X3 * Np];
                x21 = vg[XI2X1 * Np], x22 = vg[XI2X2 * Np], x23 = vg[XI2X3 * Np];
            }
#pragma unroll
            for (int s = 0; s < NS; ++s) {
                const double F1 = F[3 * s], F2_ = F[3 * s + 1], F3 = F[3 * s + 2];
                sF[(0 * NS + s) * Np + tid] = M * (x11 * F1 + x12 * F2_ + x13 * F3);
                sF[(1 * NS + s) * Np + tid] = M * (x21 * F1 + x22 * F2_ + x23 * F3);
            }
        }
        if (vt) {
            if constexpr (!METRICS_FIRST) x31 = vg[XI3X1 * Np], x32 = vg[XI3X2 * Np], x33 = vg[XI3X3 * Np];
#pragma unroll
            for (int s = 0; s < NS; ++s) {
                const double F1 = F[3 * s], F2_ = F[3 * s + 1], F3 = F[3 * s + 2];
                sF[(2 * NS + s) * Np + tid] = M * (x31 * F1 + x32 * F2_ + x33 * F3);
            }
        }
        S.negzero();
        if constexpr (P::HAS_SOURCE) {
            Vec<P::NDER> lder;
            load_state<P::NDER, Np>(lder, a.derived, tid, e);
            P::source(a.prm, S, lQ, lgf, laux, lder, a_t, a.model_dir);
        }
    }
    __syncthreads();
    Vec<NS> Tv;
    if (live && tid < Np) {
        const int i = tid % NQ, j = (tid / NQ) % NQ, k = tid / (NQ * NQ);
        Vec<NS> Tprev;
#pragma unroll
        for (int s = 0; s < NS; ++s) Tprev[s] = 0.0;
        if (a.beta != 0) {
#pragma unroll
            for (int s = 0; s < NS; ++s) Tprev[s] = a.tendency[tid + (int64_t)Np * (s + (int64_t)NS * e)];
        }
        double mDi[NQ], mDj[NQ], mDk[NQV];
#pragma unroll
        for (int n = 0; n < NQ; ++n) mDi[n] = mDj[n] = 0.0;
#pragma unroll
        for (int kk = 0; kk < NQV; ++kk) mDk[kk] = 0.0;
        if constexpr (HS_SHAPE) {
            if (hz) {
#pragma unroll
                for (int n = 0; n < NQ; ++n) {
                    mDi[n] = MI * sD[n + NQ * i];
                    mDj[n] = MI * sD[n + NQ * j];
                }
            }
            if (vt) {
#pragma unroll
                for (int kk = 0; kk < NQV; ++kk) mDk[kk] = MI * sDv[kk + NQV * k];
            }
        }
#pragma unroll
        for (int s = 0; s < NS; ++s) {
            double T = 0.0;
            const double Told = Tprev[s];
            if (hz) {
                double lt = 0.0;
                if (a.direction == DIR_HORIZONTAL && P::HAS_SOURCE) lt += S[s];
#pragma unroll
                for (int n = 0; n < NQ; ++n) {
                    lt += (HS_SHAPE ? mDi[n] : MI * sD[n + NQ * i]) * sF[(0 * NS + s) * Np + n + NQ * (j + NQ * k)];
                    lt += (HS_SHAPE ? mDj[n] : MI * sD[n + NQ * j]) * sF[(1 * NS + s) * Np + i + NQ * (n + NQ * k)];
                }
                T = a.beta != 0 ? a.alpha * lt + a.beta * Told : a.alpha * lt;
            }
            if (vt) {
                double lt = 0.0;
#pragma unroll
                for (int kk = 0; kk < NQV; ++kk) {
                    lt += (HS_SHAPE ? mDk[kk] : MI * sDv[kk + NQV * k]) * sF[(2 * NS + s) * Np + i + NQ * (j + NQ * kk)];
                    if (kk == k && P::HAS_SOURCE) lt += S[s];
                }
                if (hz)
                    T = a.alpha * lt + T;
                else
                    T = a.beta != 0 ? a.alpha * lt + a.beta * Told : a.alpha * lt;
            }
            Tv[s] = T;
        }
    }
    __syncthreads();
    if (live && tid < Np) {
#pragma unroll
        for (int s = 0; s < NS; ++s) sT[s * Np + tid] = Tv[s];
    }
    Vec<NS> lift;
    int vidM = 0, fpair = -1;
    if (tid < KD::NFT) {
        int f, n;
        KD::face_task(tid, f, n);
        if (face_on) {
            const int facedir = f < 4 ? DIR_HORIZONTAL : DIR_VERTICAL;
            FacePt fp;
            face_geometry<NQ, NQV>(a.g, e, tid, f, n, f_idP, f_bctag, fp);
            Vec<NS> QM, QPn, QPd, flux;
            Vec<NAUX> auxM, auxPn, auxPd;
            Vec<NGF> gfM, gfP;
            Vec<NHYP> hypM, hypP;
            const int sidx = surf_index<NQ, NQV>(fp.vidM);
#pragma unroll
            for (int s = 0; s < NAUX; ++s) auxM[s] = 0;
#pragma unroll
            for (int s = 0; s < NS; ++s) QM[s] = sQ[s * Np + fp.vidM];
            Vec<NCA> cM;
#pragma unroll
            for (int s = 0; s < NCA; ++s) cM[s] = sM[(OCA + s) * NSURF + sidx];
#pragma unroll
            for (int s = 0; s < NFA; ++s)
                auxM[P::face_aux(s)] =
                    STAGE_M ? sM[s * NSURF + sidx]
                            : a.aux[fp.vidM + (int64_t)Np * (P::face_aux(s) + (int64_t)NAUX * e)];
#pragma unroll
            for (int s = 0; s < NGF; ++s) gfM[s] = gfP[s] = 0.0;
            const int gslot = RECV ? ghost_slot<Np>(a.h, fp.eP, fp.vidP) : -1;
            if (use_gf) {
                if constexpr (STAGE_M) {
#pragma unroll
                    for (int s = 0; s < NGF; ++s) gfM[s] = sM[(NFA + s) * NSURF + sidx];
                } else {
                    load_gf<P, Np>(gfM, a.gf, fp.vidM, e);
                }
            }
#pragma unroll
            for (int s = 0; s < NHYP; ++s)
                hypM[s] = STAGE_M ? sM[(NFA + NGFS + s) * NSURF + sidx]
                                  : a.hypgrad[hg_at<NHG, Np>(fp.vidM, s, e)];
#pragma unroll
            for (int s = 0; s < NAUX; ++s) auxPn[s] = 0;
            if (use_gf) load_plus_gf<P, Np>(gfP, a.gf, a.h.recvGF, gslot, fp.vidP, fp.eP);
            load_plus<NS, Np, NS>(QPn, a.Q, a.h.recvQ, gslot, fp.vidP, fp.eP);
#pragma unroll
            for (int s = 0; s < NFA; ++s)
                auxPn[P::face_aux(s)] = a.aux[fp.vidP + (int64_t)Np * (P::face_aux(s) + (int64_t)NAUX * fp.eP)];
            load_plus_hg<NHG, Np, NHYP>(hypP, a.hypgrad, a.h.recvHG, gslot, fp.vidP, fp.eP);
#pragma unroll
            for (int s = 0; s < NS; ++s) QPd[s] = QPn[s];
#pragma unroll
            for (int s = 0; s < NAUX; ++s) auxPd[s] = auxPn[s];
            flux.negzero();
            if (fp.bctag == 0) {
                nf_first_order<P>(a.prm, a.nf_first, flux, fp.n, QM, auxM, QPn, auxPn, a_t,
                                  facedir, NCA > 0 ? (const double *)cM : nullptr);
                Vec<3 * NS> FM, FP;
                FM.negzero();
                P::flux_second_order(a.prm, FM, QM, gfM, hypM, auxM, a_t);
                FP.negzero();
                P::flux_second_order(a.prm, FP, QPd, gfP, hypP, auxPd, a_t);
                const double nh0 = fp.n[0] / 2, nh1 = fp.n[1] / 2, nh2 = fp.n[2] / 2;
#pragma unroll
                for (int s = 0; s < NS; ++s)
                    flux[s] += (FM[3 * s] + FP[3 * s]) * nh0 +
                               (FM[3 * s + 1] + FP[3 * s + 1]) * nh1 +
                               (FM[3 * s + 2] + FP[3 * s + 2]) * nh2;
            } else {
                load_state<NAUX, Np>(auxM, a.aux, fp.vidM, e);
#pragma unroll
                for (int s = 0; s < NAUX; ++s) auxPn[s] = auxPd[s] = auxM[s];
                Vec<NS> Q1;
                Vec<NAUX> aux1;
                Vec<NGF> gf1;
                for (int s = 0; s < NS; ++s) Q1[s] = 0;
                for (int s = 0; s < NAUX; ++s) aux1[s] = 0;
                for (int s = 0; s < NGF; ++s) gf1[s] = 0;
                if (f == 4) {
                    load_state<NS, Np>(Q1, a.Q, n + NQ * NQ, e);
                    load_state<NAUX, Np>(aux1, a.aux, n + NQ * NQ, e);
                    if (use_gf) load_gf<P, Np>(gf1, a.gf, n + NQ * NQ, e);
                }
                P::boundary_state(a.prm, BS_FIRST, fp.bctag, QPn, auxPn, fp.n, QM, auxM, a_t, Q1,
                                  aux1);
                nf_first_order<P>(a.prm, a.nf_first, flux, fp.n, QM, auxM, QPn, auxPn, a_t,
                                  facedir, NCA > 0 ? (const double *)cM : nullptr);
                Vec<3 * NS> FP;
                FP.negzero();
                P::boundary_flux_second_order(a.prm, fp.bctag, FP, QPd, gfP, hypP, auxPd, fp.n, QM,
                                              gfM, hypM, auxM, a_t, Q1, gf1, aux1);
#pragma unroll
                for (int s = 0; s < NS; ++s)
                    flux[s] +=
                        FP[3 * s] * fp.n[0] + FP[3 * s + 1] * fp.n[1] + FP[3 * s + 2] * fp.n[2];
            }
#pragma unroll
            for (int s = 0; s < NS; ++s) lift[s] = a.alpha * fp.vMI * fp.sM * flux[s];
            vidM = fp.vidM;
            fpair = f / 2;
        }
    }
    Vec<NAUX> gaux;
    if constexpr (GARG_OUT) {
        if (live && tid < Np) load_state<NAUX, Np>(gaux, a.aux, tid, e);
    }
    __syncthreads();
#pragma unroll
    for (int p = 0; p < 3; ++p) {
        if (fpair == p) {
#pragma unroll
            for (int s = 0; s < NS; ++s) sT[s * Np + vidM] -= lift[s];
        }
        __syncthreads();
    }
    if (live && tid < Np) {
        Vec<NS> Qn;
#pragma unroll
        for (int s = 0; s < NS; ++s) {
            const int64_t o = tid + (int64_t)Np * (s + (int64_t)NS * e);
            const double T = sT[s * Np + tid];
            if constexpr (LSRK) {
                Qn[s] = sQ[s * Np + tid] + a.rkb_dt * T;
                a.Qout[o] = Qn[s];
                a.tendency[o] = T * a.rka_next;
            } else {
                a.tendency[o] = T;
            }
        }
        if constexpr (GARG_OUT) {
            Vec<P::NGRAD> G;
            G.negzero();
            P::gradient_argument(a.prm, G, Qn, gaux, a_t);
            double *rec = a.garg + garg_at<P::NGL, Np>(tid, e);
#pragma unroll
            for (int s = 0; s < P::NGL; ++s) rec[s] = G[P::hv_indexmap(s)];
            if constexpr (GARG_REFRESH) {
                P::update_aux(a.prm, Qn, gaux, a_t);
#pragma unroll
                for (int s = 0; s < P::NUPD; ++s)
                    a.aux_rw[tid + (int64_t)Np * (P::upd_aux(s) + (int64_t)NAUX * e)] = gaux[P::upd_aux(s)];
            }
        }
    }
    if constexpr (LSRK) {
        if (live)
            send_nodes<NS, NS>(a.h, 0, e, tid, EPB == 1 ? (int)SH::NT : (int)SH::NTE, [&](int s, int n) {
                return sQ[s * Np + n] + a.rkb_dt * sT[s * Np + n];
            });
    }
}
template <class P, int NQ, int NQV, bool LSRK, bool USE_GF, bool RECV = false, bool GARG_OUT = false,
          bool GARG_REFRESH = true>
__global__ void __launch_bounds__((TendencyShape<P, NQ, NQV>::NT), CMDG_TEND_MINW) k_tendency(const PassArgs<P> a)
{
    tendency_body<P, NQ, NQV, LSRK, USE_GF, RECV, GARG_OUT, GARG_REFRESH>(a);
}

template <class P, bool USE_GF>
__host__ __device__ constexpr unsigned gradient_argument_mask()
{
    if (USE_GF) return ~0u;
    unsigned m = 0;
    for (int s = 0; s < P::NGL; ++s) m |= 1u << P::hv_indexmap(s);
    return m;
}

template <class P, int NQ, int NQV = NQ, bool USE_GF = true, bool GARG_IN = false>
__global__ void __launch_bounds__((KDims<NQ, NQV>::Np > 125 ? CMDG_GRAD_BOUND_LARGE : KDims<NQ, NQV>::NT),
                                   (NQ == 5 && NQV == 5 ? grad_min_waves<P>::value : 1)) k_gradients(const PassArgs<P> a)
{
    using KD = KDims<NQ, NQV>;
    const double a_t = a.tptr ? *a.tptr : a.t;
    constexpr int Np = KD::Np, NS = P::NS, NAUX = P::NAUX, NGRAD = P::NGRAD,
                  NGF = USE_GF ? P::NGF : 0, NGL = P::NGL, NHG = 3 * NGL, NACC = NGF + NHG;
    constexpr unsigned GMASK = gradient_argument_mask<P, USE_GF>();
    static_assert(!GARG_IN || (!USE_GF && NGL > 0), "the hand-off feeds the USE_GF = false pass");
    __shared__ double sD[NQ * NQ + (NQV == NQ ? 0 : NQV * NQV)];
    const double *const sDv = sD + (NQV == NQ ? 0 : NQ * NQ);
    __shared__ double sG[(NGRAD > 0 ? NGRAD : 1) * Np];
    __shared__ double sA[(NACC > 0 ? NACC : 1) * Np];
    const int tid = threadIdx.x;
    const int64_t e = a.elems[xcd_remap(blockIdx.x, gridDim.x)] - 1;
    if (tid < NQ * NQ) sD[tid] = a.g.D[tid];
    if constexpr (NQV != NQ) {
        if (tid < NQV * NQV) sD[NQ * NQ + tid] = a.g.Dv[tid];
    }
    const bool hz = a.direction != DIR_VERTICAL, vt = a.direction != DIR_HORIZONTAL;
    Vec<NS> lQ;
    Vec<NAUX> laux;
    if constexpr (GARG_IN) {
        if (tid < Np) {
            const double *rec = a.garg + garg_at<NGL, Np>(tid, e);
#pragma unroll
            for (int s = 0; s < NGL; ++s) sG[P::hv_indexmap(s) * Np + tid] = rec[s];
        }
    } else if (tid < Np) {
        load_state<NS, Np>(lQ, a.Q, tid, e);
        load_state<NAUX, Np>(laux, a.aux, tid, e);
        if constexpr (P::HAS_UPDATE_AUX && P::FUSE_UPDATE_AUX) {
            P::update_aux(a.prm, lQ, laux, a_t);
#pragma unroll
            for (int s = 0; s < P::NUPD; ++s)
                a.aux_rw[tid + (int64_t)Np * (P::upd_aux(s) + (int64_t)NAUX * e)] =
                    laux[P::upd_aux(s)];
        }
        Vec<NGRAD> G;
        G.negzero();
        P::gradient_argument(a.prm, G, lQ, laux, a_t);
#pragma unroll
        for (int s = 0; s < NGRAD; ++s)
            if (GMASK >> s & 1) sG[s * Np + tid] = G[s];
    }
    __syncthreads();
    if (tid < Np) {
        const int i = tid % NQ, j = (tid / NQ) % NQ, k = tid / (NQ * NQ);
        const double *vg = a.g.vgeo + (int64_t)Np * a.g.nvgeo * e + tid;
        Vec<3 * NGRAD> gh, gv;
        gh.negzero();
        gv.negzero();
        if (hz) {
            const double x11 = vg[XI1X1 * Np], x12 = vg[XI1X2 * Np], x13 = vg[XI1X3 * Np];
            const double x21 = vg[XI2X1 * Np], x22 = vg[XI2X2 * Np], x23 = vg[XI2X3 * Np];
#pragma unroll
            for (int s = 0; s < NGRAD; ++s) {
                if (!(GMASK >> s & 1)) continue;
                double G1 = 0.0, G2 = 0.0;
#pragma unroll
                for (int n = 0; n < NQ; ++n) {
                    G1 += sD[i + NQ * n] * sG[s * Np + n + NQ * (j + NQ * k)];
                    G2 += sD[j + NQ * n] * sG[s * Np + i + NQ * (n + NQ * k)];
                }
                gh[3 * s + 0] += x11 * G1;
                gh[3 * s + 1] += x12 * G1;
                gh[3 * s + 2] += x13 * G1;
                gh[3 * s + 0] += x21 * G2;
                gh[3 * s + 1] += x22 * G2;
                gh[3 * s + 2] += x23 * G2;
            }
        }
        if (vt) {
            const double x31 = vg[XI3X1 * Np], x32 = vg[XI3X2 * Np], x33 = vg[XI3X3 * Np];
#pragma unroll
            for (int s = 0; s < NGRAD; ++s) {
                if (!(GMASK >> s & 1)) continue;
                double G3 = -0.0;
#pragma unroll
                for (int n = 0; n < NQV; ++n)
                    G3 += sDv[k + NQV * n] * sG[s * Np + i + NQ * (j + NQ * n)];
                gv[3 * s + 0] += x31 * G3;
                gv[3 * s + 1] += x32 * G3;
                gv[3 * s + 2] += x33 * G3;
            }
        }
#pragma unroll
        for (int s = 0; s < NGL; ++s)
#pragma unroll
            for (int d = 0; d < 3; ++d) {
                const int q = d + 3 * P::hv_indexmap(s);
                sA[(NGF + 3 * s + d) * Np + tid] = hz ? (vt ? gh[q] + gv[q] : gh[q]) : gv[q];
            }
        if constexpr (NGF > 0) {
            Vec<NGF> o1, o2;
            o1.negzero();
            o2.negzero();
            Vec<NGRAD> Gn;
#pragma unroll
            for (int s = 0; s < NGRAD; ++s) Gn[s] = (GMASK >> s & 1) ? sG[s * Np + tid] : 0.0;
            if (hz) law_gradient_flux<P>(a.prm, o1, gh, lQ, laux, a_t, Gn);
            if (vt) law_gradient_flux<P>(a.prm, o2, gv, lQ, laux, a_t, Gn);
#pragma unroll
            for (int s = 0; s < NGF; ++s)
                sA[s * Np + tid] = hz ? (vt ? o1[s] + o2[s] : o1[s]) : o2[s];
        }
    }
    __syncthreads();
    Vec<NACC> corr;
    int vidM = 0, fpair = -1;
    if (tid < KD::NFT) {
        int f, n;
        KD::face_task(tid, f, n);
        const bool on = f < 4 ? hz : vt;
        if (on) {
            FacePt fp;
            face_setup<NQ, NQV, true>(a.g, e, tid, f, n, fp);
            Vec<NS> QM, QP;
            Vec<NAUX> auxM, auxP;
            Vec<NGRAD> GM, GP;
            if constexpr (!GARG_IN) {
                load_state<NS, Np>(QM, a.Q, fp.vidM, e);
                load_state<NAUX, Np>(auxM, a.aux, fp.vidM, e);
            }
#pragma unroll
            for (int s = 0; s < NGRAD; ++s)
                GM[s] = (GMASK >> s & 1) ? sG[s * Np + fp.vidM] : 0.0;
            GP.negzero();
            Vec<NGF> lgf;
            lgf.negzero();
            Vec<3 * NGRAD> tg, nGM;
            if (fp.bctag == 0) {
                if constexpr (GARG_IN) {
                    const double *rec = a.garg + garg_at<NGL, Np>(fp.vidP, fp.eP);
#pragma unroll
                    for (int s = 0; s < NGL; ++s) GP[P::hv_indexmap(s)] = rec[s];
                } else {
                    load_plus<NS, Np, NS>(QP, a.Q, a.h.recvQ, ghost_slot<Np>(a.h, fp.eP, fp.vidP), fp.vidP,
                                          fp.eP);
                    load_state<NAUX, Np>(auxP, a.aux, fp.vidP, fp.eP);
                    P::gradient_argument(a.prm, GP, QP, auxP, a_t);
                }
#pragma unroll
                for (int s = 0; s < NGRAD; ++s)
#pragma unroll
                    for (int d = 0; d < 3; ++d) tg[d + 3 * s] = fp.n[d] * (GP[s] + GM[s]) / 2;
            } else {
                if constexpr (GARG_IN) {
                    load_state<NS, Np>(QM, a.Q, fp.vidM, e);
                    load_state<NAUX, Np>(auxM, a.aux, fp.vidM, e);
                }
#pragma unroll
                for (int s = 0; s < NS; ++s) QP[s] = QM[s];
#pragma unroll
                for (int s = 0; s < NAUX; ++s) auxP[s] = auxM[s];
                Vec<NS> Q1;
                Vec<NAUX> aux1;
                for (int s = 0; s < NS; ++s) Q1[s] = 0;
                for (int s = 0; s < NAUX; ++s) aux1[s] = 0;
                if (f == 4) {
                    load_state<NS, Np>(Q1, a.Q, n + NQ * NQ, e);
                    load_state<NAUX, Np>(aux1, a.aux, n + NQ * NQ, e);
                }
                P::boundary_state(a.prm, BS_GRADIENT, fp.bctag, QP, auxP, fp.n, QM, auxM, a_t, Q1,
                                  aux1);
                P::gradient_argument(a.prm, GP, QP, auxP, a_t);
#pragma unroll
                for (int s = 0; s < NGRAD; ++s)
#pragma unroll
                    for (int d = 0; d < 3; ++d) tg[d + 3 * s] = fp.n[d] * GP[s];
            }
            if constexpr (NGF > 0) law_gradient_flux<P>(a.prm, lgf, tg, QM, auxM, a_t, GM);
#pragma unroll
            for (int s = 0; s < NGRAD; ++s)
#pragma unroll
                for (int d = 0; d < 3; ++d) nGM[d + 3 * s] = fp.n[d] * GM[s];
#pragma unroll
            for (int s = 0; s < NGL; ++s)
#pragma unroll
                for (int d = 0; d < 3; ++d) {
                    const int q = d + 3 * P::hv_indexmap(s);
                    corr[NGF + 3 * s + d] = fp.w * (tg[q] - nGM[q]);
                }
            if constexpr (NGF > 0) {
                Vec<NGF> visc;
                for (int s = 0; s < NGF; ++s) visc[s] = 0;
                law_gradient_flux<P>(a.prm, visc, nGM, QM, auxM, a_t, GM);
#pragma unroll
                for (int s = 0; s < NGF; ++s) corr[s] = fp.w * (lgf[s] - visc[s]);
            }
            vidM = fp.vidM;
            fpair = f / 2;
        }
    }
#pragma unroll
    for (int p = 0; p < 3; ++p) {
        if (fpair == p) {
#pragma unroll
            for (int s = 0; s < NACC; ++s) sA[s * Np + vidM] += corr[s];
        }
        __syncthreads();
    }
    if (tid < Np) {
        if constexpr (!gf_node_major<P>::value) {
#pragma unroll
            for (int s = 0; s < NGF; ++s)
                a.gf[tid + (int64_t)Np * (s + (int64_t)P::NGF * e)] = sA[s * Np + tid];
        }
    }
    if constexpr (gf_node_major<P>::value && NGF > 0)
        store_node_major<P::NGF, Np, NGF>(a.gf, e, tid, (int)blockDim.x, sA);
    if constexpr (NHG > 0)
        store_node_major<NHG, Np, NHG>(a.hypgrad, e, tid, (int)blockDim.x, sA + NGF * Np);
    if constexpr (NGF > 0)
        send_nodes<P::NGF, NGF>(a.h, 0, e, tid, (int)blockDim.x, [&](int s, int n) { return sA[s * Np + n]; });
    if constexpr (NHG > 0)
        send_nodes<NHG, NHG>(a.h, 1, e, tid, (int)blockDim.x,
                             [&](int s, int n) { return sA[(NGF + s) * Np + n]; });
}

template <class P, int NQ, int NQV = NQ, bool RING = false>
__global__ void __launch_bounds__((KDims<NQ, NQV>::NT)) k_divgrad(const PassArgs<P> a)
{
    using KD = KDims<NQ, NQV>;
    const double a_t = a.tptr ? *a.tptr : a.t;
    constexpr int Np = KD::Np, NAUX = P::NAUX, NGL = P::NGL, NHG = 3 * NGL,
                  NHYP = P::NHYP, NG = NGL > 0 ? NGL : 1;
    __shared__ double sD[NQ * NQ + (NQV == NQ ? 0 : NQV * NQV)];
    const double *const sDv = sD + (NQV == NQ ? 0 : NQ * NQ);
    __shared__ double sC[3 * NG * Np];
    __shared__ double sA[NG * Np];
    constexpr int NSURF = SurfDims<NQ, NQV>::NSURF;
    __shared__ double sM[(NHG > 0 ? NHG : 1) * NSURF];
    const int tid = threadIdx.x;
    const int64_t e = a.elems[xcd_remap(blockIdx.x, gridDim.x)] - 1;
    if (tid < NQ * NQ) sD[tid] = a.g.D[tid];
    if constexpr (NQV != NQ) {
        if (tid < NQV * NQV) sD[NQ * NQ + tid] = a.g.Dv[tid];
    }
    const bool hz = a.direction != DIR_VERTICAL, vt = a.direction != DIR_HORIZONTAL;
    double MI = 0;
    if (tid < Np) {
        const double *vg = a.g.vgeo + (int64_t)Np * a.g.nvgeo * e + tid;
        const double M = vg[VM * Np];
        MI = vg[VMI * Np];
        double x11 = 0, x12 = 0, x13 = 0, x21 = 0, x22 = 0, x23 = 0, x31 = 0, x32 = 0, x33 = 0;
        if (hz) {
            x11 = vg[XI1X1 * Np], x12 = vg[XI1X2 * Np], x13 = vg[XI1X3 * Np];
            x21 = vg[XI2X1 * Np], x22 = vg[XI2X2 * Np], x23 = vg[XI2X3 * Np];
        }
        if (vt) x31 = vg[XI3X1 * Np], x32 = vg[XI3X2 * Np], x33 = vg[XI3X3 * Np];
        Vec<NHG> G;
#pragma unroll
        for (int q = 0; q < NHG; ++q) G[q] = a.hypgrad[hg_at<NHG, Np>(tid, q, e)];
#pragma unroll
        for (int s = 0; s < NGL; ++s) {
            const double G1 = G[3 * s + 0], G2 = G[3 * s + 1], G3 = G[3 * s + 2];
            if (hz) {
                sC[(0 * NG + s) * Np + tid] = M * (x11 * G1 + x12 * G2 + x13 * G3);
                sC[(1 * NG + s) * Np + tid] = M * (x21 * G1 + x22 * G2 + x23 * G3);
            }
            if (vt) sC[(2 * NG + s) * Np + tid] = M * (x31 * G1 + x32 * G2 + x33 * G3);
            const int sidx = surf_index<NQ, NQV>(tid);
            if (sidx >= 0) {
                sM[(3 * s + 0) * NSURF + sidx] = G1;
                sM[(3 * s + 1) * NSURF + sidx] = G2;
                sM[(3 * s + 2) * NSURF + sidx] = G3;
            }
        }
    }
    __syncthreads();
    if (tid < Np) {
        const int i = tid % NQ, j = (tid / NQ) % NQ, k = tid / (NQ * NQ);
#pragma unroll
        for (int s = 0; s < NGL; ++s) {
            double dh = 0.0, dv = 0.0;
            if (hz) {
#pragma unroll
                for (int n = 0; n < NQ; ++n) {
                    dh -= MI * sD[n + NQ * i] * sC[(0 * NG + s) * Np + n + NQ * (j + NQ * k)];
                    dh -= MI * sD[n + NQ * j] * sC[(1 * NG + s) * Np + i + NQ * (n + NQ * k)];
                }
            }
            if (vt) {
#pragma unroll
                for (int kk = 0; kk < NQV; ++kk)
                    dv -= MI * sDv[kk + NQV * k] * sC[(2 * NG + s) * Np + i + NQ * (j + NQ * kk)];
            }
            sA[s * Np + tid] = hz ? (vt ? dh + dv : dh) : dv;
        }
    }
    __syncthreads();
    Vec<NGL> corr;
    int vidM = 0, fpair = -1;
    if (tid < KD::NFT) {
        int f, n;
        KD::face_task(tid, f, n);
        const bool on = f < 4 ? hz : vt;
        if (on) {
            FacePt fp;
            face_setup<NQ, NQV, true>(a.g, e, tid, f, n, fp);
            Vec<NHG> gM, gP;
            const int sidx = surf_index<NQ, NQV>(fp.vidM);
#pragma unroll
            for (int q = 0; q < NHG; ++q) gM[q] = sM[q * NSURF + sidx];
            load_plus_hg<NHG, Np, NHG>(gP, a.hypgrad, a.h.recvHG, ghost_slot<Np>(a.h, fp.eP, fp.vidP),
                                    fp.vidP, fp.eP);
            if (fp.bctag != 0) {
                Vec<NAUX> auxM, auxP;
                load_state<NAUX, Np>(auxM, a.aux, fp.vidM, e);
                load_state<NAUX, Np>(auxP, a.aux, fp.vidP, fp.eP);
                P::boundary_state_divergence(a.prm, fp.bctag, gP, auxP, fp.n, gM, auxM, a_t);
            }
            const double nh0 = fp.n[0] / 2, nh1 = fp.n[1] / 2, nh2 = fp.n[2] / 2;
#pragma unroll
            for (int s = 0; s < NGL; ++s) {
                const double ldiv = (gP[3 * s] + gM[3 * s]) * nh0 +
                                    (gP[3 * s + 1] + gM[3 * s + 1]) * nh1 +
                                    (gP[3 * s + 2] + gM[3 * s + 2]) * nh2;
                corr[s] = fp.w * ldiv;
            }
            vidM = fp.vidM;
            fpair = f / 2;
        }
    }
#pragma unroll
    for (int p = 0; p < 3; ++p) {
        if (fpair == p) {
#pragma unroll
            for (int s = 0; s < NGL; ++s) sA[s * Np + vidM] += corr[s];
        }
        __syncthreads();
    }
    if constexpr (RING) store_ring_major<NG, NQ, NQV>(a.lapr, e, tid, (int)blockDim.x, sA);
    if (tid < Np) {
        if (!RING || a.hypdiv_out) {
#pragma unroll
            for (int s = 0; s < NGL; ++s)
                a.hypdiv[tid + (int64_t)Np * (s + (int64_t)NHYP * e)] = sA[s * Np + tid];
        }
    }
    if constexpr (NGL > 0)
        send_nodes<NGL, NGL>(a.h, 0, e, tid, (int)blockDim.x, [&](int s, int n) { return sA[s * Np + n]; });
}

template <class P, int NQ, int NQV = NQ, bool RING = false>
__global__ void __launch_bounds__((KDims<NQ, NQV>::NT), CMDG_LAP_MINW) k_gradlap(const PassArgs<P> a)
{
    using KD = KDims<NQ, NQV>;
    const double a_t = a.tptr ? *a.tptr : a.t;
    constexpr int Np = KD::Np, NS = P::NS, NAUX = P::NAUX, NGL = P::NGL,
                  NHG = 3 * NGL, NHYP = P::NHYP, NG = NGL > 0 ? NGL : 1,
                  NH = NHYP > 0 ? NHYP : 1;
    __shared__ double sD[NQ * NQ + (NQV == NQ ? 0 : NQV * NQV)];
    const double *const sDv = sD + (NQV == NQ ? 0 : NQ * NQ);
    __shared__ double sL[NG * Np];
    __shared__ double sA[NH * Np];
    const int tid = threadIdx.x;
    const int64_t e = a.elems[xcd_remap(blockIdx.x, gridDim.x)] - 1;
    if (tid < NQ * NQ) sD[tid] = a.g.D[tid];
    if constexpr (NQV != NQ) {
        if (tid < NQV * NQV) sD[NQ * NQ + tid] = a.g.Dv[tid];
    }
    const bool hz = a.direction != DIR_VERTICAL, vt = a.direction != DIR_HORIZONTAL;
    if (tid < Np) {
        Vec<NGL> l;
        if constexpr (RING) {
            const double *rec = a.lapr + garg_at<NG, Np>(ring_slot<NQ, NQV>(tid), e);
#pragma unroll
            for (int s = 0; s < NGL; ++s) l[s] = rec[s];
        } else {
#pragma unroll
            for (int s = 0; s < NGL; ++s) l[s] = a.hypdiv[tid + (int64_t)Np * (s + (int64_t)NHYP * e)];
        }
#pragma unroll
        for (int s = 0; s < NGL; ++s) sL[s * Np + tid] = l[s];
    }
    __syncthreads();
    if (tid < Np) {
        const int i = tid % NQ, j = (tid / NQ) % NQ, k = tid / (NQ * NQ);
        const double *vg = a.g.vgeo + (int64_t)Np * a.g.nvgeo * e + tid;
        Vec<NS> lQ;
        Vec<NAUX> laux;
        load_state<NS, Np>(lQ, a.Q, tid, e);
        load_state<NAUX, Np>(laux, a.aux, tid, e);
        Vec<NHG> lh, lv;
        lh.negzero();
        lv.negzero();
        if (hz) {
            const double x11 = vg[XI1X1 * Np], x12 = vg[XI1X2 * Np], x13 = vg[XI1X3 * Np];
            const double x21 = vg[XI2X1 * Np], x22 = vg[XI2X2 * Np], x23 = vg[XI2X3 * Np];
#pragma unroll
            for (int s = 0; s < NGL; ++s) {
                double l1 = 0.0, l2 = 0.0;
#pragma unroll
                for (int n = 0; n < NQ; ++n) {
                    l1 += sD[i + NQ * n] * sL[s * Np + n + NQ * (j + NQ * k)];
                    l2 += sD[j + NQ * n] * sL[s * Np + i + NQ * (n + NQ * k)];
                }
                lh[3 * s + 0] = x11 * l1;
                lh[3 * s + 1] = x12 * l1;
                lh[3 * s + 2] = x13 * l1;
                lh[3 * s + 0] += x21 * l2;
                lh[3 * s + 1] += x22 * l2;
                lh[3 * s + 2] += x23 * l2;
            }
        }
        if (vt) {
            const double x31 = vg[XI3X1 * Np], x32 = vg[XI3X2 * Np], x33 = vg[XI3X3 * Np];
#pragma unroll
            for (int s = 0; s < NGL; ++s) {
                double l3 = -0.0;
#pragma unroll
                for (int n = 0; n < NQV; ++n)
                    l3 += sDv[k + NQV * n] * sL[s * Np + i + NQ * (j + NQ * n)];
                lv[3 * s + 0] += x31 * l3;
                lv[3 * s + 1] += x32 * l3;
                lv[3 * s + 2] += x33 * l3;
            }
        }
        Vec<NHYP> h1, h2;
        h1.negzero();
        h2.negzero();
        if (hz) P::post_gradient_laplacian(a.prm, h1, lh, lQ, laux, a_t);
        if (vt) P::post_gradient_laplacian(a.prm, h2, lv, lQ, laux, a_t);
#pragma unroll
        for (int s = 0; s < NHYP; ++s) sA[s * Np + tid] = hz ? (vt ? h1[s] + h2[s] : h1[s]) : h2[s];
    }
    __syncthreads();
    Vec<NHYP> corr;
    int vidM = 0, fpair = -1;
    if (tid < KD::NFT) {
        int f, n;
        KD::face_task(tid, f, n);
        const bool on = f < 4 ? hz : vt;
        if (on) {
            FacePt fp;
            face_setup<NQ, NQV, true>(a.g, e, tid, f, n, fp);
            Vec<NS> QM, QP;
            Vec<NAUX> auxM, auxP;
            Vec<NGL> lapM, lapP;
            load_state<NS, Np>(QM, a.Q, fp.vidM, e);
            load_state<NAUX, Np>(auxM, a.aux, fp.vidM, e);
            if constexpr (RING) {
#pragma unroll
                for (int s = 0; s < NS; ++s) QP[s] = QM[s];
#pragma unroll
                for (int s = 0; s < NAUX; ++s) auxP[s] = auxM[s];
#pragma unroll
                for (int s = 0; s < NGL; ++s) lapM[s] = sL[s * Np + fp.vidM];
                const double *rec = a.lapr + garg_at<NG, Np>(fp.vidP, fp.eP);
#pragma unroll
                for (int s = 0; s < NGL; ++s) lapP[s] = rec[s];
            } else {
                const int gslot = ghost_slot<Np>(a.h, fp.eP, fp.vidP);
                load_plus<NS, Np, NS>(QP, a.Q, a.h.recvQ, gslot, fp.vidP, fp.eP);
                load_state<NAUX, Np>(auxP, a.aux, fp.vidP, fp.eP);
#pragma unroll
                for (int s = 0; s < NGL; ++s) lapM[s] = sL[s * Np + fp.vidM];
                load_plus<NHYP, Np, NGL, NGL>(lapP, a.hypdiv, a.h.recvHD, gslot, fp.vidP, fp.eP);
            }
            if (fp.bctag != 0)
                P::boundary_state_higher_order(a.prm, fp.bctag, QP, auxP, lapP, fp.n, QM, auxM,
                                               lapM, a_t);
            Vec<NHG> G;
#pragma unroll
            for (int s = 0; s < NGL; ++s)
#pragma unroll
                for (int d = 0; d < 3; ++d) G[d + 3 * s] = fp.n[d] * (lapP[s] - lapM[s]) / 2;
            Vec<NHYP> lh;
            for (int s = 0; s < NHYP; ++s) lh[s] = 0;
            P::post_gradient_laplacian(a.prm, lh, G, QM, auxM, a_t);
#pragma unroll
            for (int s = 0; s < NHYP; ++s) corr[s] = fp.w * lh[s];
            vidM = fp.vidM;
            fpair = f / 2;
        }
    }
#pragma unroll
    for (int p = 0; p < 3; ++p) {
        if (fpair == p) {
#pragma unroll
            for (int s = 0; s < NHYP; ++s) sA[s * Np + vidM] += corr[s];
        }
        __syncthreads();
    }
    if constexpr (NHYP > 0) store_node_major<NHG, Np, NHYP>(a.hypgrad, e, tid, (int)blockDim.x, sA);
    if constexpr (NHYP > 0)
        send_nodes<NHG, NHYP>(a.h, 0, e, tid, (int)blockDim.x, [&](int s, int n) { return sA[s * Np + n]; });
}

template <class P, int NQ, int NQV = NQ>
__global__ void k_update_aux(typename P::Params prm, const double *Q, double *aux,
                             const uint8_t *activedofs, double t, int64_t e0, int64_t e1)
{
    constexpr int Np = KDims<NQ, NQV>::Np, NS = P::NS, NAUX = P::NAUX;
    const int64_t I = (int64_t)blockIdx.x * blockDim.x + threadIdx.x;
    const int64_t e = e0 + I / Np;
    const int n = (int)(I % Np);
    if (e >= e1) return;
    if (activedofs && !activedofs[n + e * Np]) return;
    Vec<NS> lQ;
    Vec<NAUX> laux;
    load_state<NS, Np>(lQ, Q, n, e);
    load_state<NAUX, Np>(laux, aux, n, e);
    P::update_aux(prm, lQ, laux, t);
    if constexpr (P::NUPD > 0) {
#pragma unroll
        for (int s = 0; s < P::NUPD; ++s)
            aux[n + (int64_t)Np * (P::upd_aux(s) + (int64_t)NAUX * e)] = laux[P::upd_aux(s)];
    } else {
#pragma unroll
        for (int s = 0; s < NAUX; ++s) aux[n + (int64_t)Np * (s + (int64_t)NAUX * e)] = laux[s];
    }
}

template <class P, int NQ, int NQV = NQ>
__global__ void k_init_derived(typename P::Params prm, const double *aux, double *derived,
                               int64_t nelem)
{
    constexpr int Np = KDims<NQ, NQV>::Np, NAUX = P::NAUX, NDER = P::NDER;
    const int64_t I = (int64_t)blockIdx.x * blockDim.x + threadIdx.x;
    const int64_t e = I / Np;
    const int n = (int)(I % Np);
    if (e >= nelem) return;
    Vec<NAUX> laux;
    load_state<NAUX, Np>(laux, aux, n, e);
    Vec<NDER> d;
    P::init_derived(prm, d, laux);
#pragma unroll
    for (int s = 0; s < NDER; ++s) derived[n + (int64_t)Np * (s + (int64_t)NDER * e)] = d[s];
}

template <class P, int NQ, int NQV, int MODE>
__global__ __launch_bounds__((KDims<NQ, NQV>::Np <= 128 ? 128 : 256)) void k_courant(
    typename P::Params prm, const double *__restrict__ vgeo, int nvgeo,
    const double *__restrict__ Q, const double *__restrict__ aux, const double *__restrict__ gf,
    int kind, double dt, double t, int direction, double *__restrict__ out)
{
    constexpr int Np = KDims<NQ, NQV>::Np, NT = Np <= 128 ? 128 : 256;
    __shared__ double sx[3][Np], sred[NT];
    const int tid = threadIdx.x;
    const int64_t e = blockIdx.x;
    constexpr int X1 = 12;
    for (int n = tid; n < Np; n += NT)
#pragma unroll
        for (int d = 0; d < 3; ++d) sx[d][n] = vgeo[n + (int64_t)Np * (X1 + d + (int64_t)nvgeo * e)];
    __syncthreads();
    double val = MODE == 0 ? INFINITY : -INFINITY;
    for (int n = tid; n < Np; n += NT) {
        const int i = n % NQ, j = (n / NQ) % NQ, k = n / (NQ * NQ);
        double md = INFINITY;
        auto dist = [&](int m) {
            const double d0 = sx[0][n] - sx[0][m], d1 = sx[1][n] - sx[1][m], d2 = sx[2][n] - sx[2][m];
            return sqrt(d0 * d0 + d1 * d1 + d2 * d2);
        };
        if (direction != DIR_VERTICAL) {
            if (i > 0) md = fmin(md, dist(n - 1));
            if (i < NQ - 1) md = fmin(md, dist(n + 1));
            if (j > 0) md = fmin(md, dist(n - NQ));
            if (j < NQ - 1) md = fmin(md, dist(n + NQ));
        }
        if (direction != DIR_HORIZONTAL) {
            if (k > 0) md = fmin(md, dist(n - NQ * NQ));
            if (k < NQV - 1) md = fmin(md, dist(n + NQ * NQ));
        }
        if constexpr (MODE == 0) {
            val = fmin(val, md);
        } else {
            Vec<P::NS> lQ;
            Vec<P::NAUX> lA;
            Vec<P::NGF> lG;
            load_state<P::NS, Np>(lQ, Q, n, e);
            load_state<P::NAUX, Np>(lA, aux, n, e);
            if constexpr (P::NGF > 0) load_gf<P, Np>(lG, gf, n, e);
            val = fmax(val, P::courant(prm, kind, lQ, lA, lG, md, dt, t, direction));
        }
    }
    sred[tid] = val;
    __syncthreads();
    for (int h = NT / 2; h > 0; h >>= 1) {
        if (tid < h) sred[tid] = MODE == 0 ? fmin(sred[tid], sred[tid + h]) : fmax(sred[tid], sred[tid + h]);
        __syncthreads();
    }
    if (tid == 0) out[e] = sred[0];
}

}
```

### climatemachine.jl_amd/csrc/lsrk_run.hip

```cpp
#include "stepping.h"

namespace cmdg {

static __global__ void k_lsrk_update(double *__restrict__ dQ, double *__restrict__ Q, double rka,
                                     double rkb_dt, int64_t n)
{
    for (int64_t i = blockIdx.x * (int64_t)blockDim.x + threadIdx.x; i < n;
         i += (int64_t)gridDim.x * blockDim.x) {
        Q[i] += rkb_dt * dQ[i];
        dQ[i] *= rka;
    }
}
void lsrk_update(hipStream_t st, double *dQ, double *Q, double rka_next, double rkb_dt, int64_t n)
{
    hipLaunchKernelGGL(k_lsrk_update, dim3(nblocks(n)), dim3(256), 0, st, dQ, Q, rka_next, rkb_dt, n);
}
void lsrk_update(EngineBase *e, double *dQ, double *Q, double rka_next, double rkb_dt)
{
    lsrk_update(e->s_comp, dQ, Q, rka_next, rkb_dt, real_len(e));
}

static void lsrk_stage_buffers(EngineBase *e, double *Q, int s, int nstages, double **in, double **out)
{
    *in = s == 0 ? Q : e->W[(s - 1) % 2];
    *out = s == nstages - 1 && nstages > 1 ? Q : e->W[s % 2];
}

struct StageHandoff {
    bool garg_in;
    GargOut out;
    bool last_eval;
};
static StageHandoff handoff_stage(const StepInRun *run, int s, int nstages, bool refresh_elidable)
{
    if (!run) return {false, GargOut::none, true};
    const bool in = !(run->first_step && s == 0);
    if (run->last_step && s == nstages - 1) return {in, GargOut::none, true};
    const bool refresh = !refresh_elidable || nstages == 1 || (run->last_step && s == nstages - 2);
    return {in, refresh ? GargOut::records_refresh : GargOut::records, false};
}

int EngineBase::lsrk_step(double *Q, double *dQ, double t, double dt, int nstages, const double *rka,
                          const double *rkb, const double *rkc, bool continued, const StepInRun *handoff)
{
    std::vector<EngineBase *> one{this};
    double *Qs[1] = {Q}, *dQs[1] = {dQ};
    if (transport == TRANSPORT_LOCAL && communicate())
        return fail(CMDG_ERR_INVALID, "handles connected locally must be driven by the cmdg_group_* calls");
    return group_lsrk_step(one, Qs, dQs, t, dt, nstages, rka, rkb, rkc, continued, nullptr, handoff);
}

int group_lsrk_step(std::vector<EngineBase *> &g, double **Q, double **dQ, double t, double dt,
                    int nstages, const double *rka, const double *rkb, const double *rkc,
                    bool continued, const double *stage_times_dev, const StepInRun *handoff)
{
    if (nstages < 1) return g[0]->fail(CMDG_ERR_INVALID, "lsrk: nstages < 1");
    for (auto *e : g)
        if (int r = e->ensure_work()) return r;
    std::vector<RhsCtx> c(g.size());
    for (int s = 0; s < nstages; ++s) {
        for (size_t i = 0; i < g.size(); ++i) {
            RhsCtx &x = c[i];
            const bool fused = g[i]->fused_lsrk();
            if (fused) {
                lsrk_stage_buffers(g[i], Q[i], s, nstages, &x.Qin, &x.Qout);
            } else {
                x.Qin = Q[i];
                x.Qout = nullptr;
            }
            x.tendency = dQ[i];
            x.t = t + rkc[s] * dt;
            x.tptr = stage_times_dev ? stage_times_dev + s : nullptr;
            x.alpha = 1.0;
            x.beta = 1.0;
            x.lsrk = fused;
            x.update_after = !fused;
            x.rkb_dt = rkb[s] * dt;
            x.rka_next = rka[(s + 1) % nstages];
            const StageHandoff h = handoff_stage(handoff, s, nstages, g[i]->refresh_elidable());
            x.garg_in = h.garg_in;
            x.garg_out = h.out;
            x.hypdiv_out = !h.garg_in || h.last_eval;
            if (h.out == GargOut::records_refresh) g[i]->handoff_refreshes += 1;
        }
        if (int r = group_rhs(g, c, s > 0 || continued)) return r;
    }
    for (size_t i = 0; i < g.size(); ++i) {
        EngineBase *e = g[i];
        if (nstages == 1 && e->fused_lsrk())
            if (hipMemcpyAsync(Q[i], e->W[0], sizeof(double) * e->Np * e->ns * e->nreal,
                               hipMemcpyDeviceToDevice, e->s_comp) != hipSuccess)
                return e->fail(CMDG_ERR_HIP, "lsrk: copy back failed");
        if (e->step_filter) {
            if (int r = e->filter_apply(e->step_filter, Q[i], e->ns)) return r;
            e->invalidate_sends();
        }
    }
    return CMDG_OK;
}

namespace {
struct StepTimesInit {
    double t_next, dt;
    int nstages;
    double rkc[16];
};
__global__ void k_step_times_init(double *g, StepTimesInit v)
{
    g[0] = v.t_next;
    g[1] = v.dt;
    for (int s = 0; s < v.nstages; ++s) g[18 + s] = v.rkc[s];
}
__global__ void k_step_times(double *g, int nstages)
{
    const double t = g[0], dt = g[1];
    for (int s = 0; s < nstages; ++s) g[2 + s] = t + g[18 + s] * dt;
    g[0] = t + dt;
}
}

bool EngineBase::graph_eligible() const
{
    const bool comm_ok = !exchanges() || (transport == TRANSPORT_RCCL && pipelined());
    return step_graph && !fv && !esdg && !graph_failed && !profiling && !step_filter && !tendency_filter &&
           !gradient_filter && !has_hooks && (!has_update_aux() || fused_update_aux()) && comm_ok;
}

int EngineBase::capture_step(double *Q, double *dQ, double dt, int nstages, const double *rka,
                             const double *rkb, const double *rkc)
{
    const bool comm = exchanges();
    if (graph_exec) {
        hipGraphExecDestroy(graph_exec);
        graph_exec = nullptr;
    }
    if (!d_gtime) HIPCHK(d_gtime.alloc(34));
    std::vector<EngineBase *> one{this};
    double *Qs[1] = {Q}, *dQs[1] = {dQ};
    if (4 * nstages + 1 > NGEV) return fail(CMDG_ERR_UNSUPPORTED, "step graph: too many stages");
    for (int i = 0; i < NGEV; ++i) {
        if (!gev_int[i]) HIPCHK(gev_int[i].create(hipEventDisableTiming));
        if (!gev_ext[i]) HIPCHK(gev_ext[i].create(hipEventDisableTiming));
    }
    capturing = true;
    cap_interior = cap_exterior = cap_pass = 0;
    hipGraph_t graph = nullptr;
    int r = CMDG_OK;
    const hipStream_t so = comm ? s_comm : s_comp;
    if (hipStreamBeginCapture(so, hipStreamCaptureModeRelaxed) != hipSuccess) {
        capturing = false;
        return fail(CMDG_ERR_HIP, "step graph: hipStreamBeginCapture failed");
    }
    hipLaunchKernelGGL(k_step_times, dim3(1), dim3(1), 0, so, d_gtime, nstages);
    if (comm) {
        if (hipEventRecord(gev_fork, s_comm) != hipSuccess ||
            hipStreamWaitEvent(s_comp, gev_fork, 0) != hipSuccess)
            r = fail(CMDG_ERR_HIP, "step graph: fork of the compute stream failed");
    }
    if (!r) r = group_lsrk_step(one, Qs, dQs, 0.0, dt, nstages, rka, rkb, rkc, true, d_gtime + 2);
    if (comm && !r) {
        if (hipEventRecord(gev_fork, s_comp) != hipSuccess ||
            hipStreamWaitEvent(s_comm, gev_fork, 0) != hipSuccess)
            r = fail(CMDG_ERR_HIP, "step graph: join of the compute stream failed");
    }
    const hipError_t ee = hipStreamEndCapture(so, &graph);
    capturing = false;
    if (r || ee != hipSuccess || !graph) {
        if (graph) hipGraphDestroy(graph);
        abort_exchanges();
        (void)hipGetLastError();
        graph_failed = true;
        if (!r) r = fail(CMDG_ERR_HIP, std::string("step graph: hipStreamEndCapture: ") + hipGetErrorString(ee));
        return r;
    }
    const hipError_t ie = hipGraphInstantiate(&graph_exec, graph, nullptr, nullptr, 0);
    hipGraphDestroy(graph);
    if (ie != hipSuccess) {
        graph_exec = nullptr;
        graph_failed = true;
        return fail(CMDG_ERR_HIP, std::string("step graph: hipGraphInstantiate: ") + hipGetErrorString(ie));
    }
    return CMDG_OK;
}

int EngineBase::run_steps(double *Q, double *dQ, double t, double dt, int64_t nsteps, int nstages,
                          const double *rka, const double *rkb, const double *rkc)
{
    int64_t i = 0;
    handoff_used = false;
    handoff_refreshes = 0;
    if (nsteps >= 2 && nstages <= 16 && graph_eligible()) {
        if (int r = lsrk_step(Q, dQ, t, dt, nstages, rka, rkb, rkc, false)) return r;
        t += dt;
        i = 1;
        GraphKey key;
        key.Q = Q, key.dQ = dQ, key.dt = dt, key.nstages = nstages;
        key.comm = exchanges();
        key.pipe = pipelined();
        for (int s = 0; s < nstages; ++s) key.coef[s] = rka[s], key.coef[16 + s] = rkb[s], key.coef[32 + s] = rkc[s];
        if (!graph_exec || !(key == graph_key)) {
            if (capture_step(Q, dQ, dt, nstages, rka, rkb, rkc) == CMDG_OK) graph_key = key;
            else graph_failed = true;
        }
        if (graph_exec && !graph_failed) {
            StepTimesInit v{};
            v.t_next = t, v.dt = dt, v.nstages = nstages;
            for (int s = 0; s < nstages; ++s) v.rkc[s] = rkc[s];
            const hipStream_t so = key.comm ? s_comm : s_comp;
            if (key.comm) {
                HIPCHK(hipEventRecord(ev_comp, s_comp));
                HIPCHK(hipStreamWaitEvent(s_comm, ev_comp, 0));
            }
            hipLaunchKernelGGL(k_step_times_init, dim3(1), dim3(1), 0, so, d_gtime, v);
            for (; i < nsteps; ++i, t += dt) {
                HIPCHK(hipGraphLaunch(graph_exec, so));
                graph_steps += 1;
            }
            if (key.comm) {
                HIPCHK(hipEventRecord(ev_comp, s_comm));
                HIPCHK(hipStreamWaitEvent(s_comp, ev_comp, 0));
            }
            return CMDG_OK;
        }
        invalidate_sends();
        for (; i < nsteps; ++i, t += dt)
            if (int r = lsrk_step(Q, dQ, t, dt, nstages, rka, rkb, rkc, false)) return r;
        return CMDG_OK;
    }
    handoff_used = handoff_eligible() && nsteps * nstages >= 2;
    if (handoff_used)
        if (int r = ensure_garg()) return r;
    for (; i < nsteps; ++i, t += dt) {
        const StepInRun pos{i == 0, i == nsteps - 1};
        if (int r = lsrk_step(Q, dQ, t, dt, nstages, rka, rkb, rkc, i > 0, handoff_used ? &pos : nullptr)) return r;
    }
    return CMDG_OK;
}

}

using namespace cmdg;

extern "C" {

int cmdg_lsrk_step(cmdg_handle h, double *Q, double *dQ, double t, double dt, int32_t nstages,
                   const double *rka, const double *rkb, const double *rkc)
{
    if (!h || !Q || !dQ || !rka || !rkb || !rkc) return CMDG_ERR_INVALID;
    DevGuard guard_(h->eng);
    return set_err(h, h->eng->lsrk_step(Q, dQ, t, dt, nstages, rka, rkb, rkc));
}

int cmdg_lsrk_run(cmdg_handle h, double *Q, double *dQ, double t, double dt, int64_t nsteps,
                  int32_t nstages, const double *rka, const double *rkb, const double *rkc)
{
    if (!h || !Q || !dQ || !rka || !rkb || !rkc) return CMDG_ERR_INVALID;
    EngineBase *e = h->eng;
    if (e->worker && nstages >= 1 && nstages <= 16) {
        std::vector<double> a(rka, rka + nstages), b(rkb, rkb + nstages), c(rkc, rkc + nstages);
        e->worker->submit([=]() {
            DevGuard guard_(e);
            const int r = e->run_steps(Q, dQ, t, dt, nsteps, nstages, a.data(), b.data(), c.data());
            if (r) {
                std::lock_guard<std::mutex> lk(e->worker->m);
                if (e->worker->deferred_err.empty()) e->worker->deferred_err = e->err;
            }
            return r;
        });
        return CMDG_OK;
    }
    DevGuard guard_(e);
    return set_err(h, e->run_steps(Q, dQ, t, dt, nsteps, nstages, rka, rkb, rkc));
}

int cmdg_group_lsrk_run(cmdg_handle *handles, int32_t n, double **Q, double **dQ, double t,
                        double dt, int64_t nsteps, int32_t nstages, const double *rka,
                        const double *rkb, const double *rkc)
{
    if (!Q || !dQ || !rka || !rkb || !rkc) return CMDG_ERR_INVALID;
    for (int i = 0; i < n; ++i)
        if (!Q[i] || !dQ[i]) return CMDG_ERR_INVALID;
    GroupCall gc(handles, n);
    if (!gc.ok()) return CMDG_ERR_INVALID;
    std::vector<EngineBase *> g;
    for (int i = 0; i < n; ++i) g.push_back(handles[i]->eng);
    for (int64_t s = 0; s < nsteps; ++s, t += dt)
        if (int r = group_lsrk_step(g, Q, dQ, t, dt, nstages, rka, rkb, rkc, s > 0)) return gc.finish(r);
    return CMDG_OK;
}

}
```

### include/cmdg.h

```cpp
#ifndef CMDG_H
#define CMDG_H
#include <stdint.h>

#ifdef __cplusplus
extern "C" {
#endif

typedef struct cmdg_context *cmdg_handle;

typedef enum cmdg_status {
    CMDG_OK = 0,
    CMDG_ERR_INVALID = -1,
    CMDG_ERR_HIP = -2,
    CMDG_ERR_NO_DEVICE = -3,
    CMDG_ERR_COMM = -4,
    CMDG_ERR_UNSUPPORTED = -5
} cmdg_status;

enum { CMDG_EVERY_DIRECTION = 0, CMDG_HORIZONTAL_DIRECTION = 1, CMDG_VERTICAL_DIRECTION = 2 };
enum {
    CMDG_RUSANOV = 0, CMDG_CENTRAL_FIRST_ORDER = 1,
    CMDG_ROE = 2, CMDG_HLLC = 3, CMDG_LMARS = 4,
    CMDG_ROE_MOIST = 5, CMDG_ROE_MOIST_LM = 6, CMDG_ROE_MOIST_HH = 7, CMDG_ROE_MOIST_LV = 8,
    CMDG_ROE_MOIST_LVPP = 9
};
enum {
    CMDG_PHYSICS_ADVECTION_DIFFUSION = 1, CMDG_PHYSICS_DRY_ATMOS = 2,
    CMDG_PHYSICS_HYDROSTATIC_BOUSSINESQ = 3,
    CMDG_PHYSICS_PRESSURE_GRADIENT = 4,
    CMDG_PHYSICS_SHALLOW_WATER = 5,
    CMDG_PHYSICS_MOIST_ATMOS = 6,
    CMDG_PHYSICS_OCEAN_SE01 = 7, CMDG_PHYSICS_CONTINUITY3D_SE01 = 8,
    CMDG_PHYSICS_BAROTROPIC_SE01 = 9,
    CMDG_PHYSICS_ATMOS_LINEAR_AG = 10,
    CMDG_PHYSICS_MOIST_LINEAR_AG = 11,
    CMDG_PHYSICS_ESDG_DRY_ATMOS = 12,
    CMDG_PHYSICS_ATMOS_LINEAR_ACOUSTIC = 13
};

typedef struct cmdg_desc {
    int32_t dim;
    int32_t N[3];
    int64_t nreal, nghost;
    int32_t nvgeo;
    int32_t physics_id;
    int32_t iparam[16];
    double dparam[64];
    int32_t nf_first;
    int32_t direction;
    int32_t diffusion_direction;
    int32_t stacked;
    const double *vgeo, *sgeo;
    const int64_t *vmapM, *vmapP, *elemtobndy;
    const int64_t *interiorelems;
    int64_t ninterior;
    const int64_t *exteriorelems;
    int64_t nexterior;
    const uint8_t *activedofs;
    const double *D;
    const int64_t *vmapsend;
    int64_t nvmapsend;
    const int64_t *vmaprecv;
    int64_t nvmaprecv;
    int32_t nnabr;
    const int32_t *nabrtorank;
    const int64_t *nabrtovmapsend;
    const int64_t *nabrtovmaprecv;
    double *state_auxiliary;
    double *state_gradient_flux;
    double *Qhypervisc_grad;
    double *Qhypervisc_div;
    const double *Dv;
} cmdg_desc;

const char *cmdg_version(void);
const char *cmdg_status_string(int status);
int cmdg_physics_counts(int32_t physics_id, const int32_t *iparam, int32_t out[6]);
int cmdg_atmos_host_constants(const int32_t *iparam, const double *dparam, double out[7]);

int cmdg_create(const cmdg_desc *desc, cmdg_handle *out);
int cmdg_destroy(cmdg_handle h);

enum { CMDG_FV_CONSTANT = 0, CMDG_FV_LINEAR = 1 };
enum { CMDG_FV_VANLEER = 0, CMDG_FV_NOLIMITER = 1 };
typedef struct cmdg_fv_desc {
    int32_t reconstruction;
    int32_t width;
    int32_t limiter;
    int32_t nvertelem;
    int32_t periodicstack;
} cmdg_fv_desc;
int cmdg_create_dgfv(const cmdg_desc *desc, const cmdg_fv_desc *fv, cmdg_handle *out);

enum {
    CMDG_ESDG_FLUX_NONE = 0, CMDG_ESDG_FLUX_ENTROPY_CONSERVATIVE = 1, CMDG_ESDG_FLUX_CENTRAL = 2,
    CMDG_ESDG_FLUX_KG = 3, CMDG_ESDG_FLUX_RUSANOV = 4, CMDG_ESDG_FLUX_ENTROPY_CONSERVATIVE_PENALTY = 5,
    CMDG_ESDG_FLUX_MATRIX = 6
};
typedef struct cmdg_esdg_desc {
    int32_t volume_flux;
    int32_t surface_flux;
    double Mcut;
    int32_t low_mach;
    int32_t kinetic_energy_preserving;
} cmdg_esdg_desc;
int cmdg_create_esdg(const cmdg_desc *desc, const cmdg_esdg_desc *esdg, cmdg_handle *out);
int cmdg_esdg_entropy(cmdg_handle h, const double *Q, double *beta, double *eta);

int cmdg_load_plugin(const char *path);
const char *cmdg_last_error(cmdg_handle h);

int cmdg_rhs(cmdg_handle h, double *tendency, double *Q, double t, double alpha, double beta);
int cmdg_rhs_async(cmdg_handle h, double *tendency, double *Q, double t, double alpha,
                   double beta);
int cmdg_lsrk_step(cmdg_handle h, double *Q, double *dQ, double t, double dt, int32_t nstages,
                   const double *rka, const double *rkb, const double *rkc);
int cmdg_lsrk_run(cmdg_handle h, double *Q, double *dQ, double t, double dt, int64_t nsteps,
                  int32_t nstages, const double *rka, const double *rkb, const double *rkc);
int cmdg_synchronize(cmdg_handle h);

enum {
    CMDG_OPT_KEEP_GRADFLUX = 1, CMDG_OPT_STACK_HEIGHT = 2, CMDG_OPT_REFERENCE_HALO = 3,
    CMDG_OPT_HALO_PIPELINE = 4, CMDG_OPT_STEP_GRAPH = 5, CMDG_OPT_STREAM_PRIORITY = 6,
    CMDG_OPT_TENDENCY_PAIRS = 7 , CMDG_OPT_ASYNC_RUN = 8,
    CMDG_OPT_TENDENCY_FOUR_WAVES = 9 , CMDG_OPT_GRADARG_HANDOFF = 10
};
int cmdg_set_option(cmdg_handle h, int32_t option, int32_t value);

enum {
    CMDG_Q_GRADFLUX_LIVE = 1, CMDG_Q_LAW_NEEDS_GRADFLUX = 2, CMDG_Q_NDERIVED = 3,
    CMDG_Q_NUPDATED_AUX = 4, CMDG_Q_FUSED_UPDATE_AUX = 5, CMDG_Q_DIRECT_SEND = 6,
    CMDG_Q_DIRECT_RECV = 7, CMDG_Q_TENDENCY_ELEMS_PER_GROUP = 8,
    CMDG_Q_HALO_PIPELINE = 9,
    CMDG_Q_HOST_POST_NS = 10,
    CMDG_Q_HOST_POST_COUNT = 11,
    CMDG_Q_GRAPH_STEPS = 12,
    CMDG_Q_TENDENCY_PAIRS = 13,
    CMDG_Q_GRADARG_HANDOFF = 14,
    CMDG_Q_GRADARG_REFRESHES = 15,
    CMDG_Q_STATE_READ = 16, CMDG_Q_AUX_READ = 20
};
int cmdg_query(cmdg_handle h, int32_t what, int64_t *out);

int cmdg_export_hypervisc_grad(cmdg_handle h, double *dst);
int cmdg_export_gradient_flux(cmdg_handle h, double *dst);

int cmdg_halo_begin(cmdg_handle h, double *array, int32_t nstate);
int cmdg_halo_end(cmdg_handle h, double *array, int32_t nstate);
int cmdg_fillsendbuf(double *sendbuf, const double *buf, const int64_t *vmapsend, int64_t nvmap,
                     int32_t Np, int32_t nstate);
int cmdg_transferrecvbuf(double *buf, const double *recvbuf, const int64_t *vmaprecv,
                         int64_t nvmap, int32_t Np, int32_t nstate);
int cmdg_comm_unique_id(void *out128);
int cmdg_comm_init_rccl(cmdg_handle h, const void *unique_id128, int32_t rank, int32_t nranks);
int cmdg_comm_selftest(cmdg_handle h, int64_t count);
int cmdg_comm_connect_local(cmdg_handle *handles, int32_t n);

int cmdg_group_rhs(cmdg_handle *handles, int32_t n, double **tendency, double **Q, double t,
                   double alpha, double beta);
int cmdg_group_halo(cmdg_handle *handles, int32_t n, double **arrays, int32_t nstate);
int cmdg_group_lsrk_run(cmdg_handle *handles, int32_t n, double **Q, double **dQ, double t,
                        double dt, int64_t nsteps, int32_t nstages, const double *rka,
                        const double *rkb, const double *rkc);

int cmdg_norm2_local(cmdg_handle h, const double *A, int32_t nstate, int32_t weighted,
                     double *out_host);
int cmdg_distance2_local(cmdg_handle h, const double *A, const double *B, int32_t nstate,
                         double *out_host);

enum {
    CMDG_RED_WEIGHTEDSUM = 0,
    CMDG_RED_SUM = 1,
    CMDG_RED_DOT = 2,
    CMDG_RED_DISTANCE = 3,
    CMDG_RED_NORM = 4,
    CMDG_RED_MAX = 5,
    CMDG_RED_MIN = 6
};
typedef struct cmdg_reduce_desc {
    int32_t op;
    double p;
    int32_t weighted;
    int32_t per_state;
    int32_t nstate;
    const int32_t *states;
    int32_t nstates;
} cmdg_reduce_desc;

int cmdg_reduce_local(cmdg_handle h, const cmdg_reduce_desc *d, const double *A, const double *B,
                      double *partials_host);
int cmdg_reduce_combine(const cmdg_reduce_desc *d, const double *partials, int32_t nranks,
                        double *out);
int cmdg_reduce(cmdg_handle h, const cmdg_reduce_desc *d, const double *A, const double *B,
                double *out_host);
int cmdg_group_reduce(cmdg_handle *handles, int32_t n, const cmdg_reduce_desc *d,
                      const double **A, const double **B, double *out_host);

enum {
    CMDG_ADVECTIVE_COURANT = 0, CMDG_NONDIFFUSIVE_COURANT = 1, CMDG_DIFFUSIVE_COURANT = 2,
    CMDG_VISCOUS_COURANT = 3
};
int cmdg_courant(cmdg_handle h, int32_t kind, const double *Q, double dt, double simtime,
                 int32_t direction, double *out_host);
int cmdg_min_node_distance(cmdg_handle h, int32_t direction, double *out_host);

#define CMDG_STACK_MAXOUT 8
typedef struct cmdg_stack_integral_desc {
    int32_t nout;
    int32_t src_is_state[CMDG_STACK_MAXOUT], src_col[CMDG_STACK_MAXOUT];
    double scale[CMDG_STACK_MAXOUT];
    int32_t dst_col[CMDG_STACK_MAXOUT];
    int32_t rsrc_col[CMDG_STACK_MAXOUT], rdst_col[CMDG_STACK_MAXOUT];
} cmdg_stack_integral_desc;
int cmdg_indefinite_stack_integral(cmdg_handle h, const double *Q, int32_t nstate, double *aux,
                                   int32_t naux, int32_t nvertelem, const double *Imat,
                                   const cmdg_stack_integral_desc *d);
int cmdg_reverse_indefinite_stack_integral(cmdg_handle h, double *aux, int32_t naux,
                                           int32_t nvertelem, const cmdg_stack_integral_desc *d);

typedef struct cmdg_filter_s *cmdg_filter;
enum { CMDG_FILTER_SPECTRAL = 0, CMDG_FILTER_MASS_PRESERVING = 1, CMDG_FILTER_TMAR = 2 };
enum {
    CMDG_TARGET_INDICES = 0, CMDG_TARGET_ATMOS_PERTURBATIONS = 1,
    CMDG_TARGET_ATMOS_SPECIFIC_PERTURBATIONS = 2
};
#define CMDG_MAX_FILTER_STATES 32
typedef struct cmdg_filter_desc {
    int32_t kind;
    int32_t target;
    int32_t direction;
    int32_t nindices;
    int32_t indices[CMDG_MAX_FILTER_STATES];
    int32_t aux_ref_rho, aux_ref_rhoe;
    const double *filter_h;
    const double *filter_v;
} cmdg_filter_desc;
int cmdg_filter_create(cmdg_handle h, const cmdg_filter_desc *d, cmdg_filter *out);
int cmdg_filter_destroy(cmdg_handle h, cmdg_filter f);
int cmdg_filter_apply(cmdg_handle h, cmdg_filter f, double *Q, int32_t nstate);
int cmdg_set_filters(cmdg_handle h, cmdg_filter gradient_filter, cmdg_filter tendency_filter,
                     cmdg_filter step_filter);

typedef struct cmdg_interp_s *cmdg_interp;
typedef struct cmdg_interp_desc {
    int32_t Nq[3];
    int64_t nelem;
    int64_t npoints;
    const double *xi_nodes[3];
    const int64_t *offset;
    const double *xi1, *xi2, *xi3;
    const int32_t *i1, *i2, *i3;
    int64_t n1, n2, n3;
    const double *lat_grd, *long_grd;
} cmdg_interp_desc;
int cmdg_interp_create(cmdg_handle h, const cmdg_interp_desc *d, cmdg_interp *out);
int cmdg_interp_destroy(cmdg_handle h, cmdg_interp it);
int cmdg_interp_apply(cmdg_handle h, cmdg_interp it, const double *Q, int32_t nstate, int64_t nelemQ,
                      double *v);
int cmdg_interp_project(cmdg_handle h, cmdg_interp it, double *v, int32_t nstate, const int32_t uvwi[3]);
int cmdg_interp_scatter(cmdg_handle h, const cmdg_interp *its, int32_t n, const double *const *v,
                        int32_t nstate, double *fiv);

typedef struct cmdg_dss_s *cmdg_dss_t;
typedef struct cmdg_dss_desc {
    int32_t Nq[3];
    int64_t nelem;
    int64_t nreal;
    int64_t nvt;
    const int64_t *vtconn;
    const int64_t *vtconnoff;
    int64_t nedg;
    const int64_t *edgconn;
    const int64_t *edgconnoff;
    int64_t nfc;
    const int64_t *fcconn;
    const int64_t *vertmap;
    const int64_t *edgemap;
    int64_t Nemax;
    const int64_t *facemap;
    int64_t Nfmax;
} cmdg_dss_desc;
int cmdg_dss_create(cmdg_handle h, const cmdg_dss_desc *d, cmdg_dss_t *out);
int cmdg_dss_destroy(cmdg_handle h, cmdg_dss_t dss);
int cmdg_dss_info(cmdg_dss_t dss, int64_t out[4]);
int cmdg_dss_apply(cmdg_handle h, cmdg_dss_t dss, double *Q, int32_t nstate);
int cmdg_dss(cmdg_handle h, cmdg_dss_t dss, double *Q, int32_t nstate);
int cmdg_group_dss(cmdg_handle *handles, int32_t n, const cmdg_dss_t *dss, double **Q, int32_t nstate);

#define CMDG_MAX_HOOK_OPS 4
typedef struct cmdg_rhs_hooks {
    int32_t npre;
    cmdg_filter pre_filter[CMDG_MAX_HOOK_OPS];
    int32_t ncopy;
    int32_t copy_gf_col[CMDG_MAX_HOOK_OPS], copy_aux_col[CMDG_MAX_HOOK_OPS];
    double copy_scale[CMDG_MAX_HOOK_OPS];
    int32_t has_integral, has_reverse_integral;
    cmdg_stack_integral_desc integral;
    cmdg_stack_integral_desc reverse_integral;
    int32_t nsurf;
    int32_t surf_src_col[CMDG_MAX_HOOK_OPS], surf_dst_col[CMDG_MAX_HOOK_OPS];
    int32_t nvertelem;
    const double *Imat;
    int32_t has_flow_deviation, flow_u_col, flow_ud_col;
    double flow_H;
    int32_t ops_before_gradients;
    cmdg_handle pre_rhs_handle;
    int32_t pre_rhs_src_col, pre_rhs_dst_aux_col;
} cmdg_rhs_hooks;
int cmdg_set_rhs_hooks(cmdg_handle h, const cmdg_rhs_hooks *hooks);

typedef struct cmdg_ocean_coupling_desc {
    int32_t nvertelem;
    double H;
    const double *Imat;
    int32_t slow_u_col, slow_eta_col;
    int32_t slow_dGu_col;
    int32_t fast_eta_col, fast_U_col;
    int32_t fast_GU_col, fast_du_col;
} cmdg_ocean_coupling_desc;
int cmdg_ocean_initialize_states(cmdg_handle slow, cmdg_handle fast,
                                 const cmdg_ocean_coupling_desc *d);
int cmdg_ocean_tendency_from_slow_to_fast(cmdg_handle slow, cmdg_handle fast,
                                          const cmdg_ocean_coupling_desc *d,
                                          const double *dQ_slow);
int cmdg_ocean_reconcile_from_fast_to_slow(cmdg_handle slow, cmdg_handle fast,
                                           const cmdg_ocean_coupling_desc *d, double *Q_slow,
                                           const double *Q_fast);
typedef struct cmdg_ocean01_desc {
    int32_t nvertelem;
    double H;
    const double *Imat;
    int32_t add_fast_substeps;
    int32_t nstages_fast;
    const double *rka_fast, *rkb_fast, *rkc_fast;
} cmdg_ocean01_desc;
int cmdg_split_explicit01_step(cmdg_handle slow, cmdg_handle fast, const cmdg_ocean01_desc *d,
                               double *Q3, double *dQ3, double *dQ2fast, double *Q2, double *dQ2,
                               double t, double dt, double dt_fast, int32_t nstages,
                               const double *rka, const double *rkb, const double *rkc);
int cmdg_group_split_explicit01_step(cmdg_handle *slow, cmdg_handle *fast, int32_t n,
                                     const cmdg_ocean01_desc *d, double **Q3, double **dQ3,
                                     double **dQ2fast, double **Q2, double **dQ2, double t, double dt,
                                     double dt_fast, int32_t nstages, const double *rka,
                                     const double *rkb, const double *rkc);

int cmdg_lsrk_update(cmdg_handle h, double *dQ, double *Q, double rka_next, double rkb_dt);
#define CMDG_MRI_MAXR 6
int cmdg_mri_lsrk_update(cmdg_handle h, double *dQ, double *Q, double rka_next, double rkb_dt, int32_t nR,
                         const double *const *R, const double *sc);
int cmdg_mri_qhat(cmdg_handle h, double *Qhat, const double *Q, int32_t nR, const double *const *R,
                  const double *sc);
int cmdg_ssprk_step(cmdg_handle h, double *Q, double *Rstage, double *Qstage, double t, double dt,
                    int32_t nstages, const double *rka, const double *rkb, const double *rkc);

int cmdg_ls3n_step(cmdg_handle h, double *Q, double *dQ, double *dR, double t, double dt,
                   int32_t nstages, const double *rka, const double *rkb, const double *rkc);

int cmdg_split_explicit_step(cmdg_handle slow, cmdg_handle fast,
                             const cmdg_ocean_coupling_desc *d, int32_t coupled, double *Q_slow,
                             double *dQ_slow, double *dQ2fast, double *Q_fast, double *dQ_fast,
                             double t, double dt_slow, double dt_fast, int32_t nstages,
                             const double *rka, const double *rkb, const double *rkc);

int cmdg_group_split_explicit_step(cmdg_handle *slow, cmdg_handle *fast, int32_t n,
                                   const cmdg_ocean_coupling_desc *d, int32_t coupled,
                                   double **Q_slow, double **dQ_slow, double **dQ2fast,
                                   double **Q_fast, double **dQ_fast, double t, double dt_slow,
                                   double dt_fast, int32_t nstages, const double *rka,
                                   const double *rkb, const double *rkc);

enum {
    CMDG_K_GRADIENTS = 0, CMDG_K_DIVGRAD = 1, CMDG_K_GRADLAP = 2, CMDG_K_TENDENCY = 3,
    CMDG_K_PACK = 4, CMDG_K_UNPACK = 5, CMDG_K_UPDATE_AUX = 6, CMDG_K_FILTER = 7,
    CMDG_K_STACK_INTEGRAL = 8,
    CMDG_K_TRANSPORT = 9, CMDG_K_HALO_EXPOSED = 10,
    CMDG_K_GRADIENTS_EXT = 11, CMDG_K_DIVGRAD_EXT = 12, CMDG_K_GRADLAP_EXT = 13,
    CMDG_K_TENDENCY_EXT = 14,
    CMDG_K_FV_GRADIENTS = 15, CMDG_K_FV_TENDENCY = 16,
    CMDG_K_ESDG_TENDENCY = 17, CMDG_K_COUNT = 18
};
int cmdg_profile_enable(cmdg_handle h, int32_t on);
int cmdg_profile_get(cmdg_handle h, int32_t kernel, double *total_ms, int64_t *launches);
int cmdg_profile_reset(cmdg_handle h);

typedef struct cmdg_columnlu *cmdg_columnlu_handle;
int cmdg_columnlu_create(cmdg_handle linear, int32_t nvertelem, double alpha, cmdg_columnlu_handle *out);
int cmdg_columnlu_update(cmdg_columnlu_handle lu, double alpha);
int cmdg_columnlu_assemble(cmdg_columnlu_handle lu, double alpha);
int cmdg_columnlu_solve(cmdg_columnlu_handle lu, double *Q, const double *Qrhs);
int cmdg_columnlu_info(cmdg_columnlu_handle lu, int64_t *out);
int cmdg_columnlu_alpha(cmdg_columnlu_handle lu, double *alpha);
int cmdg_columnlu_export_band(cmdg_columnlu_handle lu, int64_t column, double *out);
int cmdg_columnlu_destroy(cmdg_columnlu_handle lu);
int cmdg_ark_step(cmdg_handle full, cmdg_columnlu_handle lu, double *Q, double *const *work, double t,
                  double dt, int32_t nstages, const double *rka_explicit, const double *rka_implicit,
                  const double *rkb, const double *rkc, int32_t split_explicit_implicit);

#define CMDG_GMRES_MAX_M 64
typedef struct cmdg_gmres *cmdg_gmres_handle;
typedef struct cmdg_gmres_info {
    int64_t iterations;
    int32_t converged;
    double residual_norm;
    double threshold;
} cmdg_gmres_info;
int cmdg_gmres_create(cmdg_handle linear, int32_t M, double rtol, double atol, cmdg_gmres_handle *out);
int cmdg_gmres_fits(cmdg_handle linear, int32_t M, int64_t free_bytes, int64_t *basis_bytes);
int cmdg_gmres_prepare(cmdg_gmres_handle g, double alpha);
int cmdg_gmres_solve(cmdg_gmres_handle g, double alpha, double *Q, const double *Qrhs, double t,
                     int64_t max_iters, cmdg_gmres_info *info);
int cmdg_gmres_step_info(cmdg_gmres_handle g, int32_t capacity, cmdg_gmres_info *out, int32_t *nsolves);
int cmdg_gmres_destroy(cmdg_gmres_handle g);
int cmdg_ark_step_gmres(cmdg_handle full, cmdg_gmres_handle gmres, double *Q, double *const *work, double t,
                        double dt, int32_t nstages, const double *rka_explicit, const double *rka_implicit,
                        const double *rkb, const double *rkc, int32_t split_explicit_implicit);

#define CMDG_MRIGARK_EXPLICIT 0
#define CMDG_MRIGARK_DECOUPLED_IMPLICIT 1
#define CMDG_MRI_MAXGAMMA 4
typedef struct cmdg_mrigark_desc {
    int32_t kind;
    int32_t nstages;
    int32_t ngamma;
    const double *gamma;
    const double *dc;
    int32_t fast_nstages;
    const double *fast_rka, *fast_rkb, *fast_rkc;
    double fast_dt;
    int32_t lu_adjustable;
} cmdg_mrigark_desc;
int cmdg_mrigark_step(cmdg_handle slow, cmdg_handle slow_minus, cmdg_handle fast, cmdg_handle fast_minus,
                      cmdg_columnlu_handle lu, const cmdg_mrigark_desc *d, double *Q, double *const *work,
                      double t, double dt);
int cmdg_mrigark_step_gmres(cmdg_handle slow, cmdg_handle slow_minus, cmdg_handle fast, cmdg_handle fast_minus,
                            cmdg_gmres_handle gmres, const cmdg_mrigark_desc *d, double *Q,
                            double *const *work, double t, double dt);

#ifdef __cplusplus
}
#endif
#endif
```

Measured before the change: 20.11 billion DOF-updates/s.

## Fuse hyperdiffusion gradient and Laplacian passes into one kernel using neighbour tables

Adds a k_lapfused kernel that recomputes the horizontal hyperviscous gradient, with face lifting, inside the divergence (Laplacian) pass. When the fused path is eligible (periodic lateral faces, no halo, horizontal diffusion, gradient-argument handoff active), the separate gradients launch is skipped. Precomputed per-element tables of neighbour metric terms and face indices supply what the kernel needs about each neighbour's face. The aim is to cut one kernel launch and the global write and reread of the gradient per stage. In exchange it adds redundant neighbour-side work and extra table memory, and it relies on an edge-ordering trick to keep the floating-point summation order.

Result: faster. 21.92 billion DOF-updates/s, median of 6 (+9.0%).

```diff
diff --git a/climatemachine.jl_amd/_lib.py b/climatemachine.jl_amd/_lib.py
--- a/climatemachine.jl_amd/_lib.py
+++ b/climatemachine.jl_amd/_lib.py
@@ -19,10 +19,11 @@
 OPT_ASYNC_RUN = 8
 OPT_TENDENCY_FOUR_WAVES = 9
 OPT_GRADARG_HANDOFF = 10
+OPT_FUSED_LAPLACIAN = 11
 CMDG_Q = dict(GRADFLUX_LIVE=1, LAW_NEEDS_GRADFLUX=2, NDERIVED=3, NUPDATED_AUX=4, FUSED_UPDATE_AUX=5,
               DIRECT_SEND=6, DIRECT_RECV=7, TENDENCY_ELEMS_PER_GROUP=8, HALO_PIPELINE=9, HOST_POST_NS=10, HOST_POST_COUNT=11, GRAPH_STEPS=12, TENDENCY_PAIRS=13,
               GRADARG_HANDOFF=14, GRADARG_REFRESHES=15,
-              STATE_READ=16, AUX_READ=20)
+              STATE_READ=16, AUX_READ=20, FUSED_LAPLACIAN=24)
 
 
 class CmdgStackIntegralDesc(C.Structure):
diff --git a/climatemachine.jl_amd/csrc/cmdg.hip b/climatemachine.jl_amd/csrc/cmdg.hip
--- a/climatemachine.jl_amd/csrc/cmdg.hip
+++ b/climatemachine.jl_amd/csrc/cmdg.hip
@@ -4,6 +4,7 @@
 #include <new>
 #include <tuple>
 
+#include "lapfused_tables.h"
 #include "rccl.h"
 #include "stepping.h"
 
@@ -196,6 +197,58 @@
     if (!(sg[SVMI] == mi)) flags |= 2;
     faceW[I] = mi * sg[SSM];
     if (flags) atomicOr(bad, flags);
+}
+
+static __global__ void k_lapfused_fill(const double *__restrict__ vgeo, int nvgeo, const int32_t *__restrict__ faceP,
+                                       const double *__restrict__ faceG, const double *__restrict__ faceW,
+                                       const int32_t *__restrict__ lapI, int Np, int NFT, int NL, int64_t nreal,
+                                       double *__restrict__ lapT)
+{
+    const int64_t I = (int64_t)blockIdx.x * blockDim.x + threadIdx.x;
+    if (I >= nreal * NL) return;
+    const int64_t e = I / NL;
+    const int t = (int)(I % NL);
+    const int64_t idP = faceP[NFT * e + t], N = idP / Np;
+    const int vidP = (int)(idP - N * Np), tP = lapI[(2 * e + 0) * NL + t];
+    const double *vg = vgeo + (int64_t)Np * nvgeo * N + vidP;
+    const int rows[6] = {XI1X1, XI1X2, XI1X3, XI2X1, XI2X2, XI2X3};
+    double *dst = lapT + 10 * e * NL + t;
+#pragma unroll
+    for (int c = 0; c < 6; ++c) dst[(int64_t)c * NL] = vg[(int64_t)rows[c] * Np];
+#pragma unroll
+    for (int c = 0; c < 3; ++c) dst[(int64_t)(6 + c) * NL] = faceG[((int64_t)4 * N + c) * NFT + tP];
+    dst[(int64_t)9 * NL] = faceW[NFT * N + tP];
+}
+
+int EngineBase::init_lapfused()
+{
+    if (!garg_capable() || ngl <= 0 || nhyp != 3 * ngl || diffusion_direction != DIR_HORIZONTAL || nghost != 0 ||
+        communicate() || fv || esdg || nreal < 1)
+        return CMDG_OK;
+    const int NFT = 4 * NQ * NQV + 2 * NQ * NQ, NL = 4 * NQ * NQV;
+    std::vector<int32_t> h_faceP((size_t)(nreal * NFT));
+    std::vector<int64_t> h_bndy((size_t)(6 * nreal));
+    HIPCHK(hipMemcpy(h_faceP.data(), d_faceP, sizeof(int32_t) * h_faceP.size(), hipMemcpyDeviceToHost));
+    HIPCHK(hipMemcpy(h_bndy.data(), g.elemtobndy, sizeof(int64_t) * h_bndy.size(), hipMemcpyDeviceToHost));
+    LapFusedTables tab;
+    lapfused_build(NQ, NQV, nreal, h_faceP.data(), h_bndy.data(), tab);
+    if (!tab.eligible) return CMDG_OK;
+    std::vector<int32_t> h_lapI((size_t)(2 * NL * nreal));
+    for (int64_t e = 0; e < nreal; ++e)
+        for (int t = 0; t < NL; ++t) {
+            h_lapI[(size_t)((2 * e + 0) * NL + t)] = tab.tP[(size_t)(NL * e + t)];
+            h_lapI[(size_t)((2 * e + 1) * NL + t)] = tab.tE[(size_t)(NL * e + t)];
+        }
+    HIPCHK(d_lapI.alloc(h_lapI.size()));
+    HIPCHK(d_lapT.alloc((size_t)(10 * NL * nreal)));
+    HIPCHK(hipMemcpy(d_lapI, h_lapI.data(), sizeof(int32_t) * h_lapI.size(), hipMemcpyHostToDevice));
+    hipLaunchKernelGGL(k_lapfused_fill, dim3((unsigned)((nreal * NL + 255) / 256)), dim3(256), 0, s_comp, g.vgeo,
+                       g.nvgeo, d_faceP.get(), d_faceG.get(), d_faceW.get(), d_lapI.get(), Np, NFT, NL, nreal,
+                       d_lapT.get());
+    if (hipGetLastError() != hipSuccess || hipStreamSynchronize(s_comp) != hipSuccess)
+        return fail(CMDG_ERR_HIP, "cmdg_create: the tables of the fused Laplacian pass failed");
+    lapfused_ok = true;
+    return CMDG_OK;
 }
 
 int EngineBase::init(const cmdg_desc *d)
@@ -304,6 +357,7 @@
         g.faceW = d_faceW;
         g.facePr = d_facePr;
     }
+    if (int r = init_lapfused()) return r;
     aux = d->state_auxiliary;
     const size_t nd = (size_t)Np * nelem;
     gf = gf_node_major() ? nullptr : d->state_gradient_flux;
@@ -888,6 +942,7 @@
     case CMDG_OPT_TENDENCY_PAIRS:
     case CMDG_OPT_TENDENCY_FOUR_WAVES: return CMDG_OK;
     case CMDG_OPT_GRADARG_HANDOFF: e->gradarg_handoff = value != 0; return CMDG_OK;
+    case CMDG_OPT_FUSED_LAPLACIAN: e->fused_laplacian = value != 0; return CMDG_OK;
     case CMDG_OPT_HALO_PIPELINE:
         if (int r = e->synchronize()) return set_err(h, r);
         e->drop_graph();
@@ -915,6 +970,7 @@
     case CMDG_Q_TENDENCY_PAIRS: *out = -1; return CMDG_OK;
     case CMDG_Q_GRADARG_HANDOFF: *out = e->handoff_used; return CMDG_OK;
     case CMDG_Q_GRADARG_REFRESHES: *out = e->handoff_refreshes; return CMDG_OK;
+    case CMDG_Q_FUSED_LAPLACIAN: *out = e->fused_launches; return CMDG_OK;
     case CMDG_Q_HOST_POST_NS: *out = e->host_post_ns; return CMDG_OK;
     case CMDG_Q_HOST_POST_COUNT: *out = e->host_post_n; return CMDG_OK;
     case CMDG_Q_HALO_PIPELINE: *out = e->pipelined() && !e->has_hooks; return CMDG_OK;
diff --git a/climatemachine.jl_amd/csrc/engine.h b/climatemachine.jl_amd/csrc/engine.h
--- a/climatemachine.jl_amd/csrc/engine.h
+++ b/climatemachine.jl_amd/csrc/engine.h
@@ -81,10 +81,12 @@
         if (lsrk) return gf ? tendency_recv<true, true>(recv) : tendency_recv<true, false>(recv);
         return gf ? tendency_recv<false, true>(recv) : tendency_recv<false, false>(recv);
     }
-    static Kernel pick_divgrad(bool ring)
-    {
-        if constexpr (HO)
+    static Kernel pick_divgrad(bool ring, bool fused)
+    {
+        if constexpr (HO) {
+            if (ring && fused) return k_lapfused<P, NQ_, NQV_>;
             if (ring) return k_divgrad<P, NQ_, NQV_, true>;
+        }
         return k_divgrad<P, NQ_, NQV_>;
     }
     static Kernel pick_gradlap(bool ring)
@@ -95,6 +97,7 @@
     }
     void launch_gradients(const RhsCtx &c, const int64_t *elems, int64_t n, bool exterior, hipStream_t st) override
     {
+        if (c.lap_fused) return;
         in_pass(GRADIENTS, n, exterior, st, [&] {
             const PassArgs<P> args = make_args(c, elems, n, diffusion_direction, exterior,
                                                gf_live() ? slot[SLOT_GF].sendbuf : nullptr,
@@ -106,8 +109,13 @@
     void launch_divgrad(const RhsCtx &c, const int64_t *elems, int64_t n, bool exterior, hipStream_t st) override
     {
         in_pass(DIVGRAD, n, exterior, st, [&] {
-            const PassArgs<P> args = make_args(c, elems, n, diffusion_direction, exterior, slot[SLOT_HD].sendbuf, nullptr);
-            hipLaunchKernelGGL(pick_divgrad(c.garg_in), dim3((unsigned)n), dim3(KDims<NQ_, NQV_>::NT), 0, st, args);
+            PassArgs<P> args = make_args(c, elems, n, diffusion_direction, exterior, slot[SLOT_HD].sendbuf, nullptr);
+            const bool fused = HO && c.garg_in && c.lap_fused;
+            if (fused) {
+                args.g.facePr = d_lapI;
+                args.derived = d_lapT;
+            }
+            hipLaunchKernelGGL(pick_divgrad(c.garg_in, fused), dim3((unsigned)n), dim3(KDims<NQ_, NQV_>::NT), 0, st, args);
         });
     }
     void launch_gradlap(const RhsCtx &c, const int64_t *elems, int64_t n, bool exterior, hipStream_t st) override
diff --git a/climatemachine.jl_amd/csrc/engine_base.h b/climatemachine.jl_amd/csrc/engine_base.h
--- a/climatemachine.jl_amd/csrc/engine_base.h
+++ b/climatemachine.jl_amd/csrc/engine_base.h
@@ -48,6 +48,7 @@
     bool update_after = false;
     bool garg_in = false;
     bool hypdiv_out = true;
+    bool lap_fused = false;
     GargOut garg_out = GargOut::none;
     double rkb_dt = 0, rka_next = 0;
     bool pre_done = false;
@@ -196,6 +197,13 @@
                !step_graph && nghost == 0 && !communicate();
     }
     int ensure_garg();
+    DevBuf<int32_t> d_lapI;
+    DevBuf<double> d_lapT;
+    bool fused_laplacian = true;
+    bool lapfused_ok = false;
+    int64_t fused_launches = 0;
+    int init_lapfused();
+    bool lapfused_eligible() const { return fused_laplacian && lapfused_ok; }
     DevBuf<double> d_partial;
     int transport = TRANSPORT_NONE;
     int rank = 0, nranks = 1;
diff --git a/climatemachine.jl_amd/csrc/kernels.h b/climatemachine.jl_amd/csrc/kernels.h
--- a/climatemachine.jl_amd/csrc/kernels.h
+++ b/climatemachine.jl_amd/csrc/kernels.h
@@ -20,6 +20,12 @@
 #endif
 #ifndef CMDG_LAP_MINW
 #define CMDG_LAP_MINW 1
+#endif
+#ifndef CMDG_LAPFUSED_MINW
+#define CMDG_LAPFUSED_MINW 4
+#endif
+#ifndef CMDG_LAPFUSED_STAGE
+#define CMDG_LAPFUSED_STAGE(idx, dep) asm volatile("" : "+v"(idx) : "v"(dep))
 #endif
 
 namespace cmdg {
@@ -671,6 +677,63 @@
     return m;
 }
 
+template <int NQ, class Line>
+__device__ __forceinline__ double line_derivative(const double *sD, int i, Line line)
+{
+    double G = 0.0;
+#pragma unroll
+    for (int n = 0; n < NQ; ++n) G += sD[i + NQ * n] * line(n);
+    return G;
+}
+__device__ __forceinline__ void metric_gradient(double x11, double x12, double x13, double x21, double x22,
+                                                double x23, double G1, double G2, double *gh)
+{
+    gh[0] += x11 * G1;
+    gh[1] += x12 * G1;
+    gh[2] += x13 * G1;
+    gh[0] += x21 * G2;
+    gh[1] += x22 * G2;
+    gh[2] += x23 * G2;
+}
+template <int NQ, class Line1, class Line2>
+__device__ __forceinline__ void grad_volume_h(const double *sD, int i, int j, Line1 line1, Line2 line2, double x11,
+                                              double x12, double x13, double x21, double x22, double x23,
+                                              double *gh)
+{
+    const double G1 = line_derivative<NQ>(sD, i, line1), G2 = line_derivative<NQ>(sD, j, line2);
+    metric_gradient(x11, x12, x13, x21, x22, x23, G1, G2, gh);
+}
+__device__ __forceinline__ double central_gradient_flux(double nd, double GP, double GM)
+{
+    return nd * (GP + GM) / 2;
+}
+__device__ __forceinline__ double gradient_lift(double w, double tg, double nGM)
+{
+    return w * (tg - nGM);
+}
+__device__ __forceinline__ double contravariant(double M, double xa, double xb, double xc, double G1, double G2,
+                                                double G3)
+{
+    return M * (xa * G1 + xb * G2 + xc * G3);
+}
+template <int NQ>
+__device__ __forceinline__ double div_volume_h(double MI, const double *sD, const double *c1, const double *c2, int i,
+                                               int j, int k)
+{
+    double dh = 0.0;
+#pragma unroll
+    for (int n = 0; n < NQ; ++n) {
+        dh -= MI * sD[n + NQ * i] * c1[n + NQ * (j + NQ * k)];
+        dh -= MI * sD[n + NQ * j] * c2[i + NQ * (n + NQ * k)];
+    }
+    return dh;
+}
+__device__ __forceinline__ double central_divergence_flux(const double *gP, const double *gM, double nh0, double nh1,
+                                                          double nh2)
+{
+    return (gP[0] + gM[0]) * nh0 + (gP[1] + gM[1]) * nh1 + (gP[2] + gM[2]) * nh2;
+}
+
 template <class P, int NQ, int NQV = NQ, bool USE_GF = true, bool GARG_IN = false>
 __global__ void __launch_bounds__((KDims<NQ, NQV>::Np > 125 ? CMDG_GRAD_BOUND_LARGE : KDims<NQ, NQV>::NT),
                                    (NQ == 5 && NQV == 5 ? grad_min_waves<P>::value : 1)) k_gradients(const PassArgs<P> a)
@@ -730,18 +793,10 @@
 #pragma unroll
             for (int s = 0; s < NGRAD; ++s) {
                 if (!(GMASK >> s & 1)) continue;
-                double G1 = 0.0, G2 = 0.0;
-#pragma unroll
-                for (int n = 0; n < NQ; ++n) {
-                    G1 += sD[i + NQ * n] * sG[s * Np + n + NQ * (j + NQ * k)];
-                    G2 += sD[j + NQ * n] * sG[s * Np + i + NQ * (n + NQ * k)];
-                }
-                gh[3 * s + 0] += x11 * G1;
-                gh[3 * s + 1] += x12 * G1;
-                gh[3 * s + 2] += x13 * G1;
-                gh[3 * s + 0] += x21 * G2;
-                gh[3 * s + 1] += x22 * G2;
-                gh[3 * s + 2] += x23 * G2;
+                grad_volume_h<NQ>(
+                    sD, i, j, [&](int n) { return sG[s * Np + n + NQ * (j + NQ * k)]; },
+                    [&](int n) { return sG[s * Np + i + NQ * (n + NQ * k)]; }, x11, x12, x13, x21, x22, x23,
+                    &gh[3 * s]);
             }
         }
         if (vt) {
@@ -817,7 +872,7 @@
 #pragma unroll
                 for (int s = 0; s < NGRAD; ++s)
 #pragma unroll
-                    for (int d = 0; d < 3; ++d) tg[d + 3 * s] = fp.n[d] * (GP[s] + GM[s]) / 2;
+                    for (int d = 0; d < 3; ++d) tg[d + 3 * s] = central_gradient_flux(fp.n[d], GP[s], GM[s]);
             } else {
                 if constexpr (GARG_IN) {
                     load_state<NS, Np>(QM, a.Q, fp.vidM, e);
@@ -853,7 +908,7 @@
 #pragma unroll
                 for (int d = 0; d < 3; ++d) {
                     const int q = d + 3 * P::hv_indexmap(s);
-                    corr[NGF + 3 * s + d] = fp.w * (tg[q] - nGM[q]);
+                    corr[NGF + 3 * s + d] = gradient_lift(fp.w, tg[q], nGM[q]);
                 }
             if constexpr (NGF > 0) {
                 Vec<NGF> visc;
@@ -930,10 +985,10 @@
         for (int s = 0; s < NGL; ++s) {
             const double G1 = G[3 * s + 0], G2 = G[3 * s + 1], G3 = G[3 * s + 2];
             if (hz) {
-                sC[(0 * NG + s) * Np + tid] = M * (x11 * G1 + x12 * G2 + x13 * G3);
-                sC[(1 * NG + s) * Np + tid] = M * (x21 * G1 + x22 * G2 + x23 * G3);
-            }
-            if (vt) sC[(2 * NG + s) * Np + tid] = M * (x31 * G1 + x32 * G2 + x33 * G3);
+                sC[(0 * NG + s) * Np + tid] = contravariant(M, x11, x12, x13, G1, G2, G3);
+                sC[(1 * NG + s) * Np + tid] = contravariant(M, x21, x22, x23, G1, G2, G3);
+            }
+            if (vt) sC[(2 * NG + s) * Np + tid] = contravariant(M, x31, x32, x33, G1, G2, G3);
             const int sidx = surf_index<NQ, NQV>(tid);
             if (sidx >= 0) {
                 sM[(3 * s + 0) * NSURF + sidx] = G1;
@@ -948,13 +1003,7 @@
 #pragma unroll
         for (int s = 0; s < NGL; ++s) {
             double dh = 0.0, dv = 0.0;
-            if (hz) {
-#pragma unroll
-                for (int n = 0; n < NQ; ++n) {
-                    dh -= MI * sD[n + NQ * i] * sC[(0 * NG + s) * Np + n + NQ * (j + NQ * k)];
-                    dh -= MI * sD[n + NQ * j] * sC[(1 * NG + s) * Np + i + NQ * (n + NQ * k)];
-                }
-            }
+            if (hz) dh = div_volume_h<NQ>(MI, sD, sC + (0 * NG + s) * Np, sC + (1 * NG + s) * Np, i, j, k);
             if (vt) {
 #pragma unroll
                 for (int kk = 0; kk < NQV; ++kk)
@@ -988,9 +1037,7 @@
             const double nh0 = fp.n[0] / 2, nh1 = fp.n[1] / 2, nh2 = fp.n[2] / 2;
 #pragma unroll
             for (int s = 0; s < NGL; ++s) {
-                const double ldiv = (gP[3 * s] + gM[3 * s]) * nh0 +
-                                    (gP[3 * s + 1] + gM[3 * s + 1]) * nh1 +
-                                    (gP[3 * s + 2] + gM[3 * s + 2]) * nh2;
+                const double ldiv = central_divergence_flux(&gP[3 * s], &gM[3 * s], nh0, nh1, nh2);
                 corr[s] = fp.w * ldiv;
             }
             vidM = fp.vidM;
@@ -1015,6 +1062,193 @@
     }
     if constexpr (NGL > 0)
         send_nodes<NGL, NGL>(a.h, 0, e, tid, (int)blockDim.x, [&](int s, int n) { return sA[s * Np + n]; });
+}
+
+template <class P, int NQ, int NQV = NQ>
+__global__ void __launch_bounds__((KDims<NQ, NQV>::NT), CMDG_LAPFUSED_MINW) k_lapfused(const PassArgs<P> a)
+{
+    using KD = KDims<NQ, NQV>;
+    constexpr int Np = KD::Np, NGL = P::NGL, NHG = 3 * NGL, NHYP = P::NHYP, NG = NGL > 0 ? NGL : 1,
+                  NFT = KD::NFT, NL = 4 * KD::Nfph, NT = KD::NT;
+    static_assert(NT >= NL && NGL > 0, "one lane per lateral face task");
+    __shared__ double sD[NQ * NQ];
+    __shared__ double sG[NG * Np];
+    __shared__ double sA[3 * NG * Np];
+    __shared__ double sC[2 * NG * Np];
+    __shared__ double sL[NG * Np];
+    const int tid = threadIdx.x;
+    const int64_t e = a.elems[xcd_remap(blockIdx.x, gridDim.x)] - 1;
+    const int ft = tid - (NT - NL);
+    if (tid < NQ * NQ) sD[tid] = a.g.D[tid];
+    if (tid < Np) {
+        const double *rec = a.garg + garg_at<NGL, Np>(tid, e);
+        Vec<NGL> r;
+#pragma unroll
+        for (int s = 0; s < NGL; ++s) r[s] = rec[s];
+#pragma unroll
+        for (int s = 0; s < NGL; ++s) sG[s * Np + tid] = r[s];
+    }
+    FacePt fp;
+    int tP = 0, tE = -1, iP = 0, jP = 0, kP = 0;
+    int32_t idE = 0;
+    const double *gN = a.garg;
+    if (ft >= 0) {
+        int f, n;
+        KD::face_task(ft, f, n);
+        face_setup<NQ, NQV, true>(a.g, e, ft, f, n, fp);
+        tP = a.g.facePr[((int64_t)2 * e + 0) * NL + ft];
+        tE = a.g.facePr[((int64_t)2 * e + 1) * NL + ft];
+        gN = a.garg + garg_at<NGL, Np>(0, fp.eP);
+        iP = fp.vidP % NQ, jP = (fp.vidP / NQ) % NQ, kP = fp.vidP / (NQ * NQ);
+        if (tE >= 0) idE = a.g.faceP[(int64_t)NFT * fp.eP + tE];
+    }
+    double M = 0, MI = 0, x11 = 0, x12 = 0, x13 = 0, x21 = 0, x22 = 0, x23 = 0;
+    if (tid < Np) {
+        const double *vg = a.g.vgeo + (int64_t)Np * a.g.nvgeo * e + tid;
+        M = vg[VM * Np];
+        MI = vg[VMI * Np];
+        x11 = vg[XI1X1 * Np], x12 = vg[XI1X2 * Np], x13 = vg[XI1X3 * Np];
+        x21 = vg[XI2X1 * Np], x22 = vg[XI2X2 * Np], x23 = vg[XI2X3 * Np];
+    }
+    __syncthreads();
+    if (tid < Np) {
+        const int i = tid % NQ, j = (tid / NQ) % NQ, k = tid / (NQ * NQ);
+        Vec<NHG> gh;
+        gh.negzero();
+#pragma unroll
+        for (int s = 0; s < NGL; ++s)
+            grad_volume_h<NQ>(
+                sD, i, j, [&](int n) { return sG[s * Np + n + NQ * (j + NQ * k)]; },
+                [&](int n) { return sG[s * Np + i + NQ * (n + NQ * k)]; }, x11, x12, x13, x21, x22, x23, &gh[3 * s]);
+#pragma unroll
+        for (int q = 0; q < NHG; ++q) sA[q * Np + tid] = gh[q];
+    }
+    Vec<NHG> corr, gP;
+    int fpair = -1;
+    if (ft >= 0) {
+        fpair = ft / (2 * KD::Nfph);
+        const double *lapT = a.derived + (int64_t)10 * NL * e + ft;
+        Vec<NGL> GY, G1, G2;
+        double r1[NQ][NG];
+#pragma unroll
+        for (int s = 0; s < NGL; ++s) GY[s] = gN[NGL * fp.vidP + s];
+#pragma unroll
+        for (int n = 0; n < NQ; ++n)
+#pragma unroll
+            for (int s = 0; s < NGL; ++s) r1[n][s] = gN[NGL * (n + NQ * (jP + NQ * kP)) + s];
+#pragma unroll
+        for (int s = 0; s < NGL; ++s) G1[s] = line_derivative<NQ>(sD, iP, [&](int n) { return r1[n][s]; });
+#pragma unroll
+        for (int s = 0; s < NGL; ++s) CMDG_LAPFUSED_STAGE(kP, G1[s]);
+        double r2[NQ][NG];
+#pragma unroll
+        for (int n = 0; n < NQ; ++n)
+#pragma unroll
+            for (int s = 0; s < NGL; ++s) r2[n][s] = gN[NGL * (iP + NQ * (n + NQ * kP)) + s];
+        double T[6];
+#pragma unroll
+        for (int c = 0; c < 6; ++c) T[c] = lapT[c * NL];
+#pragma unroll
+        for (int s = 0; s < NGL; ++s) G2[s] = line_derivative<NQ>(sD, jP, [&](int n) { return r2[n][s]; });
+        gP.negzero();
+#pragma unroll
+        for (int s = 0; s < NGL; ++s) metric_gradient(T[0], T[1], T[2], T[3], T[4], T[5], G1[s], G2[s], &gP[3 * s]);
+#pragma unroll
+        for (int q = 0; q < NHG; ++q) CMDG_LAPFUSED_STAGE(idE, gP[q]);
+        double nS[3], wS, nE[3] = {0, 0, 0}, wE = 0;
+#pragma unroll
+        for (int d = 0; d < 3; ++d) nS[d] = lapT[(6 + d) * NL];
+        wS = lapT[9 * NL];
+        Vec<NGL> GE;
+        int pairE = 2;
+        if (tE >= 0) {
+            const double *sg = a.g.faceG + (int64_t)4 * NFT * fp.eP + tE;
+            nE[0] = sg[0], nE[1] = sg[NFT], nE[2] = sg[2 * NFT];
+            wE = a.g.faceW[(int64_t)NFT * fp.eP + tE];
+            const double *rec = a.garg + (int64_t)NGL * idE;
+#pragma unroll
+            for (int s = 0; s < NGL; ++s) GE[s] = rec[s];
+            int fE, nn;
+            KD::face_task(tE, fE, nn);
+            pairE = fE / 2;
+        }
+        int fS, nn;
+        KD::face_task(tP, fS, nn);
+        const bool edge_first = pairE < fS / 2;
+        Vec<NGL> GM;
+#pragma unroll
+        for (int s = 0; s < NGL; ++s) GM[s] = sG[s * Np + fp.vidM];
+#pragma unroll
+        for (int s = 0; s < NGL; ++s)
+#pragma unroll
+            for (int d = 0; d < 3; ++d) {
+                const double lS = gradient_lift(wS, central_gradient_flux(nS[d], GM[s], GY[s]), nS[d] * GY[s]);
+                if (tE >= 0) {
+                    const double lE = gradient_lift(wE, central_gradient_flux(nE[d], GE[s], GY[s]), nE[d] * GY[s]);
+                    gP[3 * s + d] += edge_first ? lE : lS;
+                    gP[3 * s + d] += edge_first ? lS : lE;
+                } else {
+                    gP[3 * s + d] += lS;
+                }
+            }
+#pragma unroll
+        for (int s = 0; s < NGL; ++s)
+#pragma unroll
+            for (int d = 0; d < 3; ++d)
+                corr[3 * s + d] =
+                    gradient_lift(fp.w, central_gradient_flux(fp.n[d], GY[s], GM[s]), fp.n[d] * GM[s]);
+    }
+    __syncthreads();
+#pragma unroll
+    for (int p = 0; p < 2; ++p) {
+        if (fpair == p) {
+#pragma unroll
+            for (int q = 0; q < NHG; ++q) sA[q * Np + fp.vidM] += corr[q];
+        }
+        __syncthreads();
+    }
+    if (tid < Np) {
+#pragma unroll
+        for (int s = 0; s < NGL; ++s) {
+            const double G1 = sA[(3 * s + 0) * Np + tid], G2 = sA[(3 * s + 1) * Np + tid],
+                         G3 = sA[(3 * s + 2) * Np + tid];
+            sC[(0 * NG + s) * Np + tid] = contravariant(M, x11, x12, x13, G1, G2, G3);
+            sC[(1 * NG + s) * Np + tid] = contravariant(M, x21, x22, x23, G1, G2, G3);
+        }
+    }
+    __syncthreads();
+    if (tid < Np) {
+        const int i = tid % NQ, j = (tid / NQ) % NQ, k = tid / (NQ * NQ);
+#pragma unroll
+        for (int s = 0; s < NGL; ++s)
+            sL[s * Np + tid] = div_volume_h<NQ>(MI, sD, sC + (0 * NG + s) * Np, sC + (1 * NG + s) * Np, i, j, k);
+    }
+    Vec<NGL> corrL;
+    if (ft >= 0) {
+        Vec<NHG> gM;
+#pragma unroll
+        for (int q = 0; q < NHG; ++q) gM[q] = sA[q * Np + fp.vidM];
+        const double nh0 = fp.n[0] / 2, nh1 = fp.n[1] / 2, nh2 = fp.n[2] / 2;
+#pragma unroll
+        for (int s = 0; s < NGL; ++s) {
+            const double ldiv = central_divergence_flux(&gP[3 * s], &gM[3 * s], nh0, nh1, nh2);
+            corrL[s] = fp.w * ldiv;
+        }
+    }
+    __syncthreads();
+#pragma unroll
+    for (int p = 0; p < 2; ++p) {
+        if (fpair == p) {
+#pragma unroll
+            for (int s = 0; s < NGL; ++s) sL[s * Np + fp.vidM] += corrL[s];
+        }
+        __syncthreads();
+    }
+    store_ring_major<NG, NQ, NQV>(a.lapr, e, tid, (int)blockDim.x, sL);
+    if (tid < Np && a.hypdiv_out) {
+#pragma unroll
+        for (int s = 0; s < NGL; ++s) a.hypdiv[tid + (int64_t)Np * (s + (int64_t)NHYP * e)] = sL[s * Np + tid];
+    }
 }
 
 template <class P, int NQ, int NQV = NQ, bool RING = false>
diff --git a/climatemachine.jl_amd/csrc/lapfused_tables.h b/climatemachine.jl_amd/csrc/lapfused_tables.h
--- /dev/null
+++ b/climatemachine.jl_amd/csrc/lapfused_tables.h
@@ -0,0 +1,84 @@
+#pragma once
+#include <stdint.h>
+
+#include <string>
+#include <vector>
+
+namespace cmdg {
+
+struct LapFusedTables {
+    int NQ = 0, NQV = 0;
+    int64_t nreal = 0;
+    bool eligible = false;
+    std::string why;
+    std::vector<int32_t> tP, tE;
+};
+
+inline int lapfused_face_vid(int NQ, int NQV, int t)
+{
+    const int Nfph = NQ * NQV, f = t / Nfph, n = t % Nfph, a = n % NQ, b = n / NQ;
+    switch (f) {
+    case 0: return NQ * (a + NQ * b);
+    case 1: return (NQ - 1) + NQ * (a + NQ * b);
+    case 2: return a + NQ * NQ * b;
+    default: return a + NQ * ((NQ - 1) + NQ * b);
+    }
+}
+
+inline void lapfused_tasks_of(int NQ, int NQV, int vid, int out[2])
+{
+    const int Nfph = NQ * NQV, i = vid % NQ, j = (vid / NQ) % NQ, k = vid / (NQ * NQ);
+    out[0] = i == 0 ? j + NQ * k : (i == NQ - 1 ? Nfph + j + NQ * k : -1);
+    out[1] = j == 0 ? 2 * Nfph + i + NQ * k : (j == NQ - 1 ? 3 * Nfph + i + NQ * k : -1);
+}
+
+inline void lapfused_build(int NQ, int NQV, int64_t nreal, const int32_t *faceP, const int64_t *elemtobndy,
+                           LapFusedTables &out)
+{
+    out = LapFusedTables();
+    out.NQ = NQ;
+    out.NQV = NQV;
+    out.nreal = nreal;
+    auto no = [&](const std::string &m) {
+        out.eligible = false;
+        out.why = m;
+        out.tP.clear();
+        out.tE.clear();
+    };
+    if (NQ < 2 || NQV < 1 || nreal < 1 || !faceP || !elemtobndy) return no("empty grid");
+    const int Np = NQ * NQ * NQV, Nfph = NQ * NQV, NL = 4 * Nfph, NFT = NL + 2 * NQ * NQ;
+    auto str = [](int64_t v) { return std::to_string(v); };
+    for (int64_t e = 0; e < nreal; ++e)
+        for (int f = 0; f < 4; ++f)
+            if (elemtobndy[f + 6 * e] != 0)
+                return no("lateral face " + str(f + 1) + " of element " + str(e + 1) + " is a boundary face");
+    out.tP.assign((size_t)(NL * nreal), -1);
+    out.tE.assign((size_t)(NL * nreal), -1);
+    for (int64_t e = 0; e < nreal; ++e)
+        for (int t = 0; t < NL; ++t) {
+            const int64_t idP = faceP[NFT * e + t];
+            const int64_t me = e * Np + lapfused_face_vid(NQ, NQV, t);
+            if (idP < 0 || idP >= nreal * Np)
+                return no("face task " + str(t) + " of element " + str(e + 1) + " has no real element on its plus side");
+            const int64_t N = idP / Np;
+            int cand[2];
+            lapfused_tasks_of(NQ, NQV, (int)(idP - N * Np), cand);
+            int found = -1, other = -1, matches = 0;
+            for (int c = 0; c < 2; ++c) {
+                if (cand[c] < 0) continue;
+                if (faceP[NFT * N + cand[c]] == me) {
+                    if (matches++ == 0) found = cand[c];
+                } else {
+                    other = cand[c];
+                }
+            }
+            if (matches != 1)
+                return no("face task " + str(t) + " of element " + str(e + 1) + (matches == 0 ? " is not seen" : " is seen twice") +
+                          " from its neighbour " + str(N + 1));
+            out.tP[(size_t)(NL * e + t)] = found;
+            out.tE[(size_t)(NL * e + t)] = other;
+        }
+    out.eligible = true;
+}
+
+}
diff --git a/climatemachine.jl_amd/csrc/lsrk_run.hip b/climatemachine.jl_amd/csrc/lsrk_run.hip
--- a/climatemachine.jl_amd/csrc/lsrk_run.hip
+++ b/climatemachine.jl_amd/csrc/lsrk_run.hip
@@ -82,6 +82,8 @@
             x.garg_out = h.out;
             x.hypdiv_out = !h.garg_in || h.last_eval;
             if (h.out == GargOut::records_refresh) g[i]->handoff_refreshes += 1;
+            x.lap_fused = h.garg_in && g[i]->lapfused_eligible();
+            if (x.lap_fused) g[i]->fused_launches += 1;
         }
         if (int r = group_rhs(g, c, s > 0 || continued)) return r;
     }
@@ -189,6 +191,7 @@
     int64_t i = 0;
     handoff_used = false;
     handoff_refreshes = 0;
+    fused_launches = 0;
     if (nsteps >= 2 && nstages <= 16 && graph_eligible()) {
         if (int r = lsrk_step(Q, dQ, t, dt, nstages, rka, rkb, rkc, false)) return r;
         t += dt;
diff --git a/include/cmdg.h b/include/cmdg.h
--- a/include/cmdg.h
+++ b/include/cmdg.h
@@ -123,7 +123,8 @@
     CMDG_OPT_KEEP_GRADFLUX = 1, CMDG_OPT_STACK_HEIGHT = 2, CMDG_OPT_REFERENCE_HALO = 3,
     CMDG_OPT_HALO_PIPELINE = 4, CMDG_OPT_STEP_GRAPH = 5, CMDG_OPT_STREAM_PRIORITY = 6,
     CMDG_OPT_TENDENCY_PAIRS = 7 , CMDG_OPT_ASYNC_RUN = 8,
-    CMDG_OPT_TENDENCY_FOUR_WAVES = 9 , CMDG_OPT_GRADARG_HANDOFF = 10
+    CMDG_OPT_TENDENCY_FOUR_WAVES = 9 , CMDG_OPT_GRADARG_HANDOFF = 10,
+    CMDG_OPT_FUSED_LAPLACIAN = 11
 };
 int cmdg_set_option(cmdg_handle h, int32_t option, int32_t value);
 
@@ -138,7 +139,8 @@
     CMDG_Q_TENDENCY_PAIRS = 13,
     CMDG_Q_GRADARG_HANDOFF = 14,
     CMDG_Q_GRADARG_REFRESHES = 15,
-    CMDG_Q_STATE_READ = 16, CMDG_Q_AUX_READ = 20
+    CMDG_Q_STATE_READ = 16, CMDG_Q_AUX_READ = 20,
+    CMDG_Q_FUSED_LAPLACIAN = 24
 };
 int cmdg_query(cmdg_handle h, int32_t what, int64_t *out);
 
```
